# mjevans26/Satellite_ComputerVision

Measured on AMD Instinct MI355X. Metric: tiles/sec (train) 256x256x4 U-Net, higher is better.
Workload: dtype bf16; 1 GPU; U-Net 256x256x4 bfloat16 training, batch 64 per GPU (BASELINE configs[1]); global_batch=64, parallelism=dp1, loss=weighted_categorical_crossentropy, optimizer=adam(9e-4)

## Files before the change

include/satcv.h:

```cpp
#ifndef SATCV_H
#define SATCV_H
#include <stdint.h>
#ifdef __cplusplus
extern "C" {
#endif

typedef double satcv_stat_t;

enum { SATCV_OK = 0, SATCV_ERR_INVALID = -1, SATCV_ERR_HIP = -2, SATCV_ERR_UNSUPPORTED = -3 };
enum { SATCV_F32 = 0, SATCV_BF16 = 1,
       SATCV_FP8 = 2 ,
       SATCV_FP8X = 3 ,
       SATCV_F64 = 4  };
#define SATCV_STAT_ROWS 32

const char* satcv_version(void);
const char* satcv_last_error(void);
int satcv_device_info(int32_t* out4);

int satcv_ingest_nhwc(const float* src, void* dst, int64_t npix, int32_t c, int32_t cpad,
                      int32_t dtype, void* stream);
int satcv_ingest_nhwc_scaled(const float* src, void* dst, int64_t npix, int32_t c, int32_t cpad, float mul, int32_t dtype, void* stream);
int satcv_ingest_chw(const void* src, int32_t src_kind, float scale, void* dst, int32_t n,
                     int32_t c, int32_t h, int32_t w, int32_t cpad, int32_t dtype, void* stream);

int satcv_pack_weights(const float* src, void* dst_fwd, void* dst_dgrad, int32_t kh, int32_t kw,
                       int32_t cin, int32_t cout, int32_t cin_pad, int32_t transposed,
                       int32_t dtype, void* stream);
typedef struct { const float* src; void* dst; int32_t mode, taps, cin, cout, kpad, npad; } satcv_pack_job;
int64_t satcv_pack_job_items(const satcv_pack_job* job);
int satcv_pack_weights_batched(const satcv_pack_job* jobs_dev, const int64_t* prefix_dev, int32_t njobs, int64_t total_items, int32_t dtype,
                               void* stream);

typedef struct satcv_conv_desc {
  const void* x0;
  const void* x1;
  int32_t c0, c1;
  const float* in_scale;
  const float* in_shift;
  int32_t in_relu;
  const void* w;
  const float* bias;
  void* y;
  int32_t ldy;
  satcv_stat_t* stats;
  int32_t stats_ld;
  int32_t n, h, w_;
  int32_t cout;
  int32_t cout_pad;
  int32_t kh, kw, dil;
  int32_t mode_in;
  int32_t mode_out;
  int32_t f;
  int32_t cstat;
  int32_t out_relu;
  int32_t dtype;
  int32_t accumulate;
  int32_t stride, hin, win;
  const float* out_scale;
  void* pool_y; int32_t pool_ld, pool_f;
  const void* bst_y; const void* bst_y1; int32_t bst_ld, bst_ld1, bst_split;
  const float* bst_scale; const float* bst_shift; const float* bst_mean; const float* bst_rstd; int32_t bst_relu;
  int32_t tile_policy;
  int32_t pair_n, pair_c0, pair_c1;
} satcv_conv_desc;
int satcv_conv2d_igemm(const satcv_conv_desc* d, void* stream);
int satcv_conv2d_igemm_pipelined(const satcv_conv_desc* d);

typedef struct satcv_wgrad_desc {
  const void* x0; const void* x1; int32_t c0, c1;
  const float* in_scale; const float* in_shift; int32_t in_relu;
  const void* dy; int32_t lddy;
  float* dw;
  int32_t cin, cout;
  int32_t n, h, w_;
  int32_t kh, kw, dil;
  int32_t mode_dy;
  int32_t f;
  int32_t transposed;
  float* workspace; int64_t workspace_bytes;
  int32_t dtype;
  int32_t accumulate;
  int32_t whole_chip;
  int32_t defer_reduce;
} satcv_wgrad_desc;
int64_t satcv_conv2d_wgrad_workspace(const satcv_wgrad_desc* d);
int satcv_conv2d_wgrad(const satcv_wgrad_desc* d, void* stream);

typedef struct satcv_reduce_job {
  const float* ws; float* dw;
  int32_t nslab, taps, kpad, npad, cin, nvalid, transposed, accumulate, lanes, pad_;
} satcv_reduce_job;
int satcv_conv2d_wgrad_reduce_job(const satcv_wgrad_desc* d, satcv_reduce_job* job);
int64_t satcv_reduce_job_items(const satcv_reduce_job* job);
int satcv_reduce_slabs_batched(const satcv_reduce_job* jobs_dev, const int64_t* prefix_dev, int32_t njobs, int64_t total_items, void* stream);

typedef struct satcv_bwdf_desc {
  const void* g; const void* yraw; int32_t ldg;
  const float* bn_scale; const float* bn_shift; const float* bn_mean; const float* bn_rstd;
  const float* bn_coef;
  int32_t linear;
  const void* x0; const void* x1; int32_t c0, c1;
  const float* in_scale; const float* in_shift; int32_t in_relu;
  const void* w_dgrad;
  void* dx; int32_t lddx;
  float* dw; int32_t cin, cout;
  int32_t n, h, w_;
  int32_t kh, kw, dil;
  float* workspace; int64_t workspace_bytes;
  int32_t dtype;
  int32_t accumulate;
  satcv_stat_t* bst_sums; int32_t bst_sums_ld;
  const float* bst_mean; const float* bst_rstd;
  int32_t bst_act_form;
  const void* dpool; int32_t lddp; const void* amax;
// ... 243 lines not shown
```

satellite_computervision_amd/_lib.py:

```python
import ctypes as C
import os

import torch

_HERE = os.path.dirname(os.path.abspath(__file__))
LIB_PATH = os.environ.get('SATCV_LIB') or os.path.join(_HERE, 'libsatcv.so')

F32, BF16, FP8, FP8X, F64 = 0, 1, 2, 3, 4
STAT_ROWS = 32
COMPOSITE_MAX_T = 256

c_i32, c_i64, c_f32, c_vp = C.c_int32, C.c_int64, C.c_float, C.c_void_p


class ConvDesc(C.Structure):
    _fields_ = [('x0', c_vp), ('x1', c_vp), ('c0', c_i32), ('c1', c_i32),
                ('in_scale', c_vp), ('in_shift', c_vp), ('in_relu', c_i32),
                ('w', c_vp), ('bias', c_vp), ('y', c_vp), ('ldy', c_i32),
                ('stats', c_vp), ('stats_ld', c_i32),
                ('n', c_i32), ('h', c_i32), ('w_', c_i32),
                ('cout', c_i32), ('cout_pad', c_i32),
                ('kh', c_i32), ('kw', c_i32), ('dil', c_i32),
                ('mode_in', c_i32), ('mode_out', c_i32), ('f', c_i32),
                ('cstat', c_i32), ('out_relu', c_i32), ('dtype', c_i32), ('accumulate', c_i32),
                ('stride', c_i32), ('hin', c_i32), ('win', c_i32), ('out_scale', c_vp), ('pool_y', c_vp), ('pool_ld', c_i32), ('pool_f', c_i32),
                ('bst_y', c_vp), ('bst_y1', c_vp), ('bst_ld', c_i32), ('bst_ld1', c_i32), ('bst_split', c_i32),
                ('bst_scale', c_vp), ('bst_shift', c_vp), ('bst_mean', c_vp), ('bst_rstd', c_vp), ('bst_relu', c_i32), ('tile_policy', c_i32),
                ('pair_n', c_i32), ('pair_c0', c_i32), ('pair_c1', c_i32)]


class PackJob(C.Structure):
    _fields_ = [('src', c_vp), ('dst', c_vp), ('mode', c_i32), ('taps', c_i32), ('cin', c_i32), ('cout', c_i32), ('kpad', c_i32), ('npad', c_i32)]


class TileDesc(C.Structure):
    _fields_ = [('src', c_vp), ('src_kind', c_i32), ('n', c_i32), ('c', c_i32), ('hin', c_i32), ('win', c_i32), ('h', c_i32), ('w_', c_i32),
                ('rescale', C.c_double), ('nan_mask', c_i32), ('replace', c_i32), ('seed', C.c_uint64), ('ch_mean', c_vp),
                ('contra_mul', C.c_double), ('bright_mul', C.c_double), ('flip_v', c_i32), ('flip_h', c_i32), ('rot', c_i32),
                ('dst', c_vp), ('ldc', c_i32), ('coff', c_i32)]


class SceneGatherDesc(C.Structure):
    _fields_ = [('src', c_vp), ('src_kind', c_i32), ('h', c_i32), ('w_', c_i32), ('c', c_i32), ('rescale', C.c_double),
                ('origins', c_vp), ('total', c_i32), ('first', c_i32), ('n', c_i32), ('off', c_i32), ('side', c_i32),
                ('dst', c_vp), ('ldc', c_i32), ('coff', c_i32)]


class SceneScatterDesc(C.Structure):
    _fields_ = [('src', c_vp), ('src_kind', c_i32), ('n', c_i32), ('sh', c_i32), ('sw', c_i32), ('lds', c_i32), ('c0', c_i32), ('nc', c_i32),
                ('crop_y', c_i32), ('crop_x', c_i32), ('crop_h', c_i32), ('crop_w', c_i32),
                ('origins', c_vp), ('total', c_i32), ('first', c_i32), ('dst', c_vp), ('dst_kind', c_i32),
                ('h', c_i32), ('w_', c_i32), ('ldd', c_i32), ('doff', c_i32), ('accumulate', c_i32)]


class CompositeDesc(C.Structure):
    _fields_ = [('src', c_vp), ('src_kind', c_i32), ('t', c_i32), ('c', c_i32), ('h', c_i32), ('w_', c_i32), ('offsets', c_vp),
                ('median', c_vp), ('ld_med', c_i32), ('coff_med', c_i32), ('norm', c_vp), ('ld_norm', c_i32), ('coff_norm', c_i32),
                ('use_fill', c_i32), ('fill', c_f32)]


class WgradDesc(C.Structure):
    _fields_ = [('x0', c_vp), ('x1', c_vp), ('c0', c_i32), ('c1', c_i32),
                ('in_scale', c_vp), ('in_shift', c_vp), ('in_relu', c_i32),
                ('dy', c_vp), ('lddy', c_i32), ('dw', c_vp),
                ('cin', c_i32), ('cout', c_i32),
                ('n', c_i32), ('h', c_i32), ('w_', c_i32),
                ('kh', c_i32), ('kw', c_i32), ('dil', c_i32),
                ('mode_dy', c_i32), ('f', c_i32), ('transposed', c_i32),
                ('workspace', c_vp), ('workspace_bytes', c_i64), ('dtype', c_i32), ('accumulate', c_i32), ('whole_chip', c_i32), ('defer_reduce', c_i32)]


class BwdfDesc(C.Structure):
    _fields_ = [('g', c_vp), ('yraw', c_vp), ('ldg', c_i32),
                ('bn_scale', c_vp), ('bn_shift', c_vp), ('bn_mean', c_vp), ('bn_rstd', c_vp), ('bn_coef', c_vp), ('linear', c_i32),
                ('x0', c_vp), ('x1', c_vp), ('c0', c_i32), ('c1', c_i32),
                ('in_scale', c_vp), ('in_shift', c_vp), ('in_relu', c_i32),
                ('w_dgrad', c_vp), ('dx', c_vp), ('lddx', c_i32),
                ('dw', c_vp), ('cin', c_i32), ('cout', c_i32),
                ('n', c_i32), ('h', c_i32), ('w_', c_i32), ('kh', c_i32), ('kw', c_i32), ('dil', c_i32),
                ('workspace', c_vp), ('workspace_bytes', c_i64), ('dtype', c_i32), ('accumulate', c_i32),
                ('bst_sums', c_vp), ('bst_sums_ld', c_i32), ('bst_mean', c_vp), ('bst_rstd', c_vp), ('bst_act_form', c_i32),
# ... 179 lines not shown
```

satellite_computervision_amd/csrc/common.hpp:

```cpp
#pragma once
#include <hip/hip_runtime.h>
#include <hip/hip_fp8.h>
#include <stdint.h>
#include <type_traits>
#include "../../include/satcv.h"

typedef __bf16 bf16;
typedef __hip_fp8_e4m3 fp8;
struct fp8s : public __hip_fp8_e4m3 { using __hip_fp8_e4m3::__hip_fp8_e4m3; };
using i32x8 = __attribute__((ext_vector_type(8))) int;
using i32x4 = __attribute__((ext_vector_type(4))) int;

template <typename T> struct KTraits { static constexpr int EL = 8, SUB = 1; };
template <> struct KTraits<fp8s> { static constexpr int EL = 16, SUB = 2; };
using bf16x8 = __attribute__((ext_vector_type(8))) __bf16;
using bf16x4 = __attribute__((ext_vector_type(4))) __bf16;
using short4v = __attribute__((ext_vector_type(4))) short;
using f32x16 = __attribute__((ext_vector_type(16))) float;
using f32x4 = __attribute__((ext_vector_type(4))) float;

void satcv_set_error(const char* fmt, ...);
#define SATCV_CHECK(cond, ...)                        \
  do {                                                \
    if (!(cond)) {                                    \
// ... 199 lines not shown
  } else if constexpr (std::is_same<T, float>::value) {
    const float* f = reinterpret_cast<const float*>(&r.q[0]);
#pragma unroll
    for (int i = 0; i < 8; ++i) out[i] = f[i];
  } else {
    const fp8* b = reinterpret_cast<const fp8*>(&r.q);
#pragma unroll
    for (int i = 0; i < 8; ++i) out[i] = (float)b[i];
  }
}
template <typename T>
__device__ __forceinline__ void keep8(const Raw8<T>& r) {
  if constexpr (std::is_same<T, fp8>::value) { asm volatile("" :: "v"(r.q.x), "v"(r.q.y)); }
  else {
#pragma unroll
    for (int i = 0; i < Raw8<T>::NQ; ++i) asm volatile("" :: "v"(r.q[i].x), "v"(r.q[i].y), "v"(r.q[i].z), "v"(r.q[i].w));
  }
}
template <typename T>
__device__ __forceinline__ Raw8<T> select8(bool keep, const Raw8<T>& r) {
  Raw8<T> o;
  if constexpr (std::is_same<T, fp8>::value) {
    o.q = make_uint2(keep ? r.q.x : 0u, keep ? r.q.y : 0u);
  } else {
#pragma unroll
    for (int i = 0; i < Raw8<T>::NQ; ++i) o.q[i] = make_uint4(keep ? r.q[i].x : 0u, keep ? r.q[i].y : 0u, keep ? r.q[i].z : 0u, keep ? r.q[i].w : 0u);
  }
  return o;
}

template <typename T>
__device__ __forceinline__ float round_to(float x) {
  if constexpr (std::is_same<T, bf16>::value) return (float)(bf16)x;
  else if constexpr (std::is_same<T, fp8>::value) return (float)(fp8)x;
  else return x;
}

__device__ __forceinline__ float wave_sum(float v) {
#pragma unroll
  for (int o = 32; o > 0; o >>= 1) v += __shfl_xor(v, o, 64);
  return v;
}

typedef __attribute__((address_space(3))) char satcv_lds_char;
__device__ __forceinline__ unsigned lds_addr_of(const void* p) { return (unsigned)(uintptr_t)(satcv_lds_char*)p; }
__device__ __forceinline__ void lds_dma16(const void* gbase, unsigned voff, unsigned lds_dst) {
  unsigned keep;
  asm volatile("s_mov_b32 %0, m0\n\ts_mov_b32 m0, %3\n\ts_nop 0\n\tglobal_load_lds_dwordx4 %2, %1\n\ts_mov_b32 m0, %0"
               : "=&s"(keep) : "s"(gbase), "v"(voff), "s"(lds_dst) : "memory");
}
__device__ __forceinline__ void dma_wait_all() { asm volatile("s_waitcnt vmcnt(0)" ::: "memory"); }

#define SATCV_STAT_REPL 32
```

satellite_computervision_amd/csrc/conv_igemm.hip:

```cpp
#include "igemm_common.hpp"
#include <cstdlib>

template <typename T, int TW, int WM, int WN, int MT, int NT, int KS>
__global__ __launch_bounds__(WM* WN * 64) void igemm_kernel(const IgemmArgs a) {
  constexpr int NTHREADS = WM * WN * 64;
  constexpr int BM = WM * MT * 32;
  constexpr int BN = WN * NT * 32;
  constexpr int TH = BM / TW;
  constexpr int KC = KS * 16;
  constexpr int SLOTS = KC / 8;
  extern __shared__ __attribute__((aligned(16))) unsigned char smem_raw[];
  T* ldsA = reinterpret_cast<T*>(smem_raw);
  const int a_elems = SLOTS * a.rl * a.pitch * 8;
  T* ldsB = ldsA + a_elems;

  const int tid = threadIdx.x;
  const int lane = tid & 63;
  const int wave = tid >> 6;
  const int wm = wave / WN, wn = wave % WN;
  const int r = lane & 31, hh = lane >> 5;

  int bid = blockIdx.x;
  const int nt = bid % a.n_tiles;
  int mt = bid / a.n_tiles;
// ... 226 lines not shown

template <typename T>
static int launch_t(IgemmArgs& a, hipStream_t st) {
  switch (igemm_pick_tw(a.w_)) {
    case 32: return launch_tw<T, 32>(a, st);
    case 16: return launch_tw<T, 16>(a, st);
    default: return launch_tw<T, 8>(a, st);
  }
}

void satcv_prof_begin(int kind, double flops, hipStream_t st);
void satcv_prof_end(int kind, hipStream_t st);

static int igemm_fill_args(const satcv_conv_desc* d, IgemmArgs& a) {
  SATCV_CHECK(d && d->x0 && d->w && d->y, "igemm: null pointer");
  SATCV_CHECK(d->c0 > 0 && d->c0 % 16 == 0 && d->c1 % 16 == 0, "igemm: channels must be multiples of 16 (c0=%d c1=%d)", d->c0, d->c1);
  SATCV_CHECK(d->dtype != SATCV_FP8X || (d->c0 % 64 == 0 && d->c1 % 64 == 0 && !d->in_scale), "igemm: the scaled fp8 path needs channels %% 64 == 0 and no input transform");
  SATCV_CHECK((d->c1 == 0) == (d->x1 == nullptr), "igemm: x1/c1 mismatch");
  SATCV_CHECK(d->kh >= 1 && d->kw >= 1 && (d->kh & 1) && (d->kw & 1) && d->dil >= 1, "igemm: bad taps");
  SATCV_CHECK(d->n > 0 && d->h > 0 && d->w_ > 0 && d->cout > 0, "igemm: bad dims");
  SATCV_CHECK(satcv_pixels_ok(d->n, d->h, d->w_, d->f) && d->cout <= (1 << 20) && d->c0 <= (1 << 20) && d->c1 <= (1 << 20) &&
              d->kh <= 15 && d->kw <= 15 && d->dil <= (1 << 15) && d->f <= 16 && d->stride <= 16,
              "igemm: extents out of range (n*h*w must stay below 2^31 pixels, channels below 2^20)");
  SATCV_CHECK(d->cstat > 0, "igemm: cstat");
  SATCV_CHECK((!d->mode_in && !d->mode_out) || (d->f >= 2 && d->kh == 1 && d->kw == 1), "igemm: s2d/d2s need 1x1 taps and f>=2");
  SATCV_CHECK(!(d->accumulate && d->stats), "igemm: accumulate with statistics");
  SATCV_CHECK(!(d->mode_in && d->in_scale), "igemm: s2d source cannot carry an input transform");
  a.x0 = d->x0; a.x1 = d->x1; a.c0 = d->c0; a.c1 = d->c1;
  a.in_scale = d->in_scale; a.in_shift = d->in_shift; a.in_relu = d->in_relu;
  a.w = d->w; a.bias = d->bias; a.out_scale = d->out_scale; a.y = d->y; a.ldy = d->ldy;
  a.pool_y = d->pool_y; a.pool_ld = d->pool_ld; a.pool_f = d->pool_f;
  SATCV_CHECK(!d->pool_y || (d->pool_f >= 2 && !d->mode_out && !d->accumulate && d->h % d->pool_f == 0 && d->w_ % d->pool_f == 0 && d->pool_ld >= d->cout &&
                             d->cout % (d->dtype == SATCV_F32 ? 4 : (d->dtype == SATCV_BF16 ? 8 : 16)) == 0),
              "igemm: fused max-pool needs pool_f >= 2 dividing h and w_, plain output mode, whole 16-byte channel vectors");
  a.stats = d->stats; a.stats_ld = d->stats_ld;
  a.n = d->n; a.h = d->h; a.w_ = d->w_;
  a.hs = d->mode_in ? d->h * d->f : d->h; a.ws = d->mode_in ? d->w_ * d->f : d->w_;
  a.cout = d->cout; a.cout_pad = d->cout_pad;
  a.kh = d->kh; a.kw = d->kw; a.dil = d->dil;
  a.mode_in = d->mode_in; a.mode_out = d->mode_out; a.f = d->f;
  a.cstat = d->cstat; a.out_relu = d->out_relu; a.accumulate = d->accumulate;
  a.stride = d->stride > 1 ? d->stride : 1;
  if (a.stride > 1) {
    SATCV_CHECK(!d->mode_in && !d->mode_out && d->hin > 0 && d->win > 0 && d->h == (d->hin - 1) / a.stride + 1 && d->w_ == (d->win - 1) / a.stride + 1,
                "igemm: strided conv needs hin/win with h=(hin-1)/stride+1");
    a.hs = d->hin; a.ws = d->win;
  }
  a.dbg = 0;
  a.ksplit = 1; a.kslab = nullptr;
  a.bst_y = d->bst_y; a.bst_y1 = d->bst_y1; a.bst_ld = d->bst_ld; a.bst_ld1 = d->bst_ld1; a.bst_split = d->bst_y1 ? d->bst_split : 0;
  a.bst_scale = d->bst_scale; a.bst_shift = d->bst_shift; a.bst_mean = d->bst_mean; a.bst_rstd = d->bst_rstd; a.bst_relu = d->bst_relu;
  a.tile_policy = d->tile_policy;
  a.pair_n = d->pair_n; a.pair_c0 = d->pair_c0; a.pair_c1 = d->pair_c1;
  if (d->pair_n || d->pair_c0 || d->pair_c1) {
    const int epv = d->dtype == SATCV_F32 ? 4 : (d->dtype == SATCV_BF16 ? 8 : 16);
    SATCV_CHECK(d->pair_n > 0 && d->n == 2 * d->pair_n, "igemm: pair store needs n == 2 * pair_n (n=%d pair_n=%d)", d->n, d->pair_n);
    SATCV_CHECK(!d->mode_out && !d->accumulate && !d->stats && !d->bst_y, "igemm: pair store needs a plain store (no mode_out / accumulate / stats / bst_y)");
    SATCV_CHECK(d->pair_c0 >= 0 && d->pair_c1 >= 0 && d->pair_c0 + d->cout <= d->ldy && d->pair_c1 + d->cout <= d->ldy,
                "igemm: pair channel offsets %d / %d + cout %d exceed ldy %d", d->pair_c0, d->pair_c1, d->cout, d->ldy);
    SATCV_CHECK(d->pair_c0 % epv == 0 && d->pair_c1 % epv == 0, "igemm: pair channel offsets must be multiples of %d", epv);
  }
  if (d->bst_y) {
    SATCV_CHECK(d->stats && d->bst_scale && d->bst_shift && d->bst_mean && d->bst_rstd, "igemm: bst_y needs stats and the four BatchNorm vectors");
    SATCV_CHECK(!d->accumulate && !d->mode_out && !d->out_relu && !d->pool_y && d->cstat == d->cout, "igemm: bst_y needs a plain, non-accumulating store");
    SATCV_CHECK(d->bst_ld >= (d->bst_y1 ? d->bst_split : d->cout) && (!d->bst_y1 || (d->bst_split > 0 && d->bst_split < d->cout && d->bst_ld1 >= d->cout - d->bst_split)),
                "igemm: bst_y channel strides");
  }
  if (a.mode_in == 1) {
    SATCV_CHECK(!d->x1, "igemm: s2d with dual source");
    a.c1 = a.c0 * (d->f * d->f - 1);
  }
  return SATCV_OK;
}

static bool igemm_force_generic() {
  static const bool v = [] { const char* e = getenv("SATCV_IGEMM"); return e && e[0] == 'g'; }();
  return v;
}

extern "C" int satcv_conv2d_igemm_pipelined(const satcv_conv_desc* d) {
  IgemmArgs a;
  if (!d || igemm_fill_args(d, a) != SATCV_OK || igemm_force_generic()) return 0;
  if (a.kh == 3 && a.kw == 3 && a.stride == 1 && a.dil >= a.h && a.dil >= a.w_) { a.kh = a.kw = 1; a.dil = 1; }
  if (d->bst_y && a.dil == 3) {
    IgemmArgs b = a;
    b.bst_y = nullptr; b.bst_y1 = nullptr;
    if (igemm_ws_launch(b, d->dtype, nullptr, true) == SATCV_OK) return 0;
  }
  return igemm_fast_launch(a, d->dtype, nullptr, true) == SATCV_OK ? 1 : 0;
}

extern "C" int satcv_conv2d_igemm(const satcv_conv_desc* d, void* stream) {
  IgemmArgs a;
  int rc = igemm_fill_args(d, a);
  if (rc) return rc;
  hipStream_t st = reinterpret_cast<hipStream_t>(stream);
  const double flops = 2.0 * d->n * d->h * d->w_ * (double)d->cout * (double)(a.c0 + a.c1) * d->kh * d->kw;
  if (a.kh == 3 && a.kw == 3 && a.stride == 1 && a.dil >= a.h && a.dil >= a.w_) {
    const size_t esz = d->dtype == SATCV_BF16 ? 2 : 4;
    a.w = reinterpret_cast<const unsigned char*>(a.w) + (size_t)4 * ((a.c0 + a.c1) / 8) * a.cout_pad * 8 * esz;
    a.kh = a.kw = 1; a.dil = 1;
  }
  satcv_prof_begin(d->kh * d->kw > 1 ? 0 : 1, flops, st);
  rc = SATCV_ERR_UNSUPPORTED;
  if (!igemm_force_generic()) {
    rc = convt_thin_launch(a, d->dtype, st);
    if (rc == SATCV_ERR_UNSUPPORTED) rc = convt_thin_dgrad_launch(a, d->dtype, st);
    if (rc == SATCV_ERR_UNSUPPORTED) rc = igemm_tr_launch(a, d->dtype, st, false);
    if (rc == SATCV_ERR_UNSUPPORTED) rc = igemm_ws_launch(a, d->dtype, st, false);
    if (rc == SATCV_ERR_UNSUPPORTED) rc = igemm_fast_launch(a, d->dtype, st);
  }
  if (rc != SATCV_ERR_UNSUPPORTED) {  }
  else if (d->dtype == SATCV_FP8 || d->dtype == SATCV_FP8X) { satcv_set_error("igemm: this fp8 shape is outside the pipelined kernel's limits"); rc = SATCV_ERR_UNSUPPORTED; }
  else if (d->out_scale || d->pool_y || d->bst_y || d->pair_n) { satcv_set_error("igemm: out_scale / pool_y / bst_y / pair store need the pipelined kernel"); rc = SATCV_ERR_UNSUPPORTED; }
  else if (d->dtype == SATCV_BF16) rc = launch_t<bf16>(a, st);
  else if (d->dtype == SATCV_F32) rc = launch_t<float>(a, st);
  else { satcv_set_error("igemm: bad dtype %d", d->dtype); rc = SATCV_ERR_INVALID; }
  satcv_prof_end(d->kh * d->kw > 1 ? 0 : 1, st);
  return rc;
}
```

satellite_computervision_amd/csrc/conv_igemm_fast.hip:

```cpp
#include "igemm_common.hpp"
#include <cstdlib>
extern int g_opt_igemm_db, g_opt_igemm_thin, g_opt_igemm_sched, g_opt_splitk, g_opt_igemm_m16;

#ifndef SATCV_ABLATE
#define SATCV_ABLATE 0
#endif
#define ABL(bit) ((SATCV_ABLATE & (bit)) != 0)
#ifdef SATCV_STAMP
__device__ unsigned long long g_stamp[8][8][8];
#define STAMP(t) do { __builtin_amdgcn_sched_barrier(0); asm volatile("s_memtime %0\n\ts_waitcnt lgkmcnt(0)" : "=s"(t) :: "memory"); __builtin_amdgcn_sched_barrier(0); } while (0)
extern "C" int satcv_debug_read_stamps(unsigned long long* out) {
  return hipMemcpyFromSymbol(out, HIP_SYMBOL(g_stamp), sizeof(g_stamp)) == hipSuccess ? 0 : -1;
}
#endif
template <typename T, int TW, int WM, int WN, int MT, int NT, int KS, int TAPS, bool DYN, bool TL = false, bool DB = false, int WPS = 0, bool WDMA = false, bool SK = false, bool M16 = false>
__global__ __launch_bounds__(WM* WN * 64, (WPS ? WPS : (MT * NT <= 2 ? (KTraits<T>::SUB == 2 ? 2 : 4) : 1))) void igemm_fast_kernel(const IgemmArgs a) {
  constexpr int NTHREADS = WM * WN * 64;
  constexpr int BM = WM * MT * 32;
  constexpr int BN = WN * NT * 32;
  constexpr int TH = BM / TW;
  constexpr int EL = KTraits<T>::EL, SUB = KTraits<T>::SUB;
  constexpr int CLc = TW + (TAPS == 9 ? 2 : 0);
  constexpr int PITCHc = igemm_pitch(TW, CLc, M16);
  static_assert(!M16 || (std::is_same<T, bf16>::value && DB && !SK && !DYN && KS % 2 == 0 && TW >= 16), "16x16x32 form: double-buffered bf16 tiles, chunks of 32 k channels, tiles at least 16 pixels wide");
// ... 440 lines not shown
#ifdef SATCV_STAMP
      STAMP(t2);
#endif
      __syncthreads();
#ifdef SATCV_STAMP
      STAMP(t3);
#endif
      if (more) {
        store_lds(chunk + 1);
#ifdef SATCV_STAMP
        STAMP(t4);
#endif
        __syncthreads();
      }
#ifdef SATCV_STAMP
      else { STAMP(t4); }
      STAMP(t5);
      s_issue += t1 - t0; s_comp += t2 - t1; s_bar1 += t3 - t2; s_store += t4 - t3; s_bar2 += t5 - t4;
#endif
    }
#ifdef SATCV_STAMP
    if (blockIdx.x < 8 && lane == 0) {
      g_stamp[blockIdx.x][wave][0] = s_issue; g_stamp[blockIdx.x][wave][1] = s_comp; g_stamp[blockIdx.x][wave][2] = s_bar1;
      g_stamp[blockIdx.x][wave][3] = s_store; g_stamp[blockIdx.x][wave][7] = s_bar2;
    }
#endif
    }
#ifdef SATCV_STAMP
    STAMP(k3);
#endif

    if constexpr (SK) {
      const size_t mtot = (size_t)a.n * a.h * a.w_;
      float* slab = a.kslab + (size_t)split * mtot * a.cout;
#pragma unroll
      for (int m = 0; m < MT; ++m)
#pragma unroll
        for (int i = 0; i < 16; ++i) {
          const int q = (wm * MT + m) * 32 + (i & 3) + 8 * (i >> 2) + 4 * hh;
          const int t = q / TW, cx = q % TW;
          const int k = (a.imgs == 1) ? 0 : t / a.rpi;
          const int nimg = n0 + k, y = y0 + (t - k * a.rpi), x = x0 + cx;
          if (!((k < a.imgs) && (nimg < a.n) && (y < a.h) && (x < a.w_))) continue;
          float* row = slab + ((size_t)(nimg * a.h + y) * a.w_ + x) * a.cout;
#pragma unroll
          for (int n = 0; n < NT; ++n) {
            const int cn = nbase + (wn * NT + n) * 32 + r;
            if (cn < a.cout) row[cn] = acc[m][n][i];
          }
        }
      return;
    } else
    igemm_epilogue<T, TW, WM, WN, MT, NT, ABL(1), !DYN, true, M16, !DYN && !std::is_same<T, float>::value>(a, acc, n0, y0, x0, nbase, smem_raw);
#ifdef SATCV_STAMP
    {
      unsigned long long k4;
      STAMP(k4);
      if (blockIdx.x < 8 && lane == 0) {
        g_stamp[blockIdx.x][wave][4] = k1 - k0; g_stamp[blockIdx.x][wave][5] = k2 - k1; g_stamp[blockIdx.x][wave][6] = k4 - k3;
      }
    }
#endif
  }
}


#include <mutex>
static float* igemm_splitk_workspace(hipStream_t st, size_t bytes) {
  struct Slot { hipStream_t st; int dev; void* p; size_t n; bool captured; };
  static Slot slots[16];
  static int nslots = 0;
  static std::mutex mu;
  std::lock_guard<std::mutex> lk(mu);
  int dev = 0;
  (void)hipGetDevice(&dev);
  Slot* s = nullptr;
  for (int i = 0; i < nslots; ++i) if (slots[i].st == st && slots[i].dev == dev) s = &slots[i];
  if (!s) {
    if (nslots == 16) return nullptr;
    s = &slots[nslots++];
    *s = Slot{st, dev, nullptr, 0, false};
  }
  hipStreamCaptureStatus cs = hipStreamCaptureStatusNone;
  const bool capturing = hipStreamIsCapturing(st, &cs) == hipSuccess && cs != hipStreamCaptureStatusNone;
  if (s->n < bytes) {
    if (capturing) return nullptr;
    if (s->p && !s->captured) { (void)hipStreamSynchronize(st); (void)hipFree(s->p); }
    s->p = nullptr; s->n = 0; s->captured = false;
    const size_t want = bytes + (bytes >> 2);
    if (hipMalloc(&s->p, want) != hipSuccess) { (void)hipGetLastError(); s->p = nullptr; return nullptr; }
    s->n = want;
  }
  if (capturing) s->captured = true;
  return reinterpret_cast<float*>(s->p);
}

template <typename T>
__global__ __launch_bounds__(256) void igemm_splitk_finish_kernel(const IgemmArgs a, long long mtot) {
  __shared__ float ssum[2][1024];
  const int G = a.cout / 8;
  const long long total = mtot * G;
  const bool st = a.stats != nullptr && a.cout <= 1024 && 256 % G == 0;
  if (st) { for (int i = threadIdx.x; i < 2 * 1024; i += blockDim.x) (&ssum[0][0])[i] = 0.f; __syncthreads(); }
  float s1[8], s2[8];
#pragma unroll
  for (int e = 0; e < 8; ++e) { s1[e] = 0.f; s2[e] = 0.f; }
// ... 84 lines not shown
  if (M16) {
    const size_t plane_b = (((size_t)a.rl * a.pitch * EL * sizeof(T) + 255) / 256) * 256;
    const size_t a_st = (size_t)(KC / EL) * plane_b, b_sl = (size_t)TAPS * KC * BN * sizeof(T);
    lds_stage = WDMA ? 2 * a_st + 3 * b_sl : 2 * (a_st + b_sl);
  }
  if (WDMA && (((uintptr_t)a.w % 16) != 0 || a.cout_pad % 64 != 0)) return SATCV_ERR_UNSUPPORTED;
  if (DB && ((TL && TAPS != 1) || a.mode_in != 0)) return SATCV_ERR_UNSUPPORTED;
  size_t lds_out = (size_t)BM * (BN + 16 / sizeof(T)) * sizeof(T) + (size_t)(WM + 1) * 2 * BN * sizeof(float);
  if (a.bst_y) {
    if (sizeof(T) != 2 || (TAPS == 9 && a.dil != 1 && !TL) || a.imgs != 1 || a.h % TH != 0 || a.w_ % TW != 0 || a.cout % BN != 0 || a.cout % 8 != 0 || a.bst_ld % 8 != 0 ||
        ((uintptr_t)a.bst_y % 16) != 0 || (a.bst_y1 && (a.bst_split % 8 != 0 || a.bst_ld1 % 8 != 0 || ((uintptr_t)a.bst_y1 % 16) != 0)))
      return SATCV_ERR_UNSUPPORTED;
    lds_out += (size_t)BM * (BN + 16 / sizeof(T)) * sizeof(T);
  }
  const size_t lds_tab = a.in_scale ? (size_t)2 * cin * sizeof(float) : 0;
  const size_t lds = lds_stage + lds_tab > lds_out ? lds_stage + lds_tab : lds_out;
  if (lds > 160 * 1024) return SATCV_ERR_UNSUPPORTED;
  const bool dyn = TAPS == 9 && a.dil != 1;
  if (a.pair_n && (dyn || std::is_same<T, float>::value)) return SATCV_ERR_UNSUPPORTED;
  long long blocks = (long long)a.ngroups * a.tiles_y * a.tiles_x * a.n_tiles;
  if (blocks <= 0 || blocks > 0x7fffffffLL) return SATCV_ERR_UNSUPPORTED;
  a.ksplit = 1; a.kslab = nullptr;
  int ks = 1;
  if constexpr (SK) {
    const int splitk = g_opt_splitk;
    static const int splitk_tl = [] { const char* e = getenv("SATCV_SPLITK_TL"); return e ? atoi(e) : 1; }();
    if ((TL ? splitk_tl : splitk) && !dyn && sizeof(T) == 2 && a.mode_out == 0 && !a.pool_y && !a.accumulate && !a.bst_y && !a.pair_n && a.cout % 8 == 0 && a.ldy % 8 == 0 &&
        a.stride == 1 && (!a.stats || (a.cout <= 1024 && 256 % (a.cout / 8) == 0))) {
      constexpr bool DEEP1X1 = TAPS == 1 && !TL && KS == 4;
      const bool small_only = !TL && (DEEP1X1 || splitk == 2);
      while (ks < (TL ? 16 : 4) && blocks * ks * 2 <= 256 && a.nchunks / (ks * 2) >= (DEEP1X1 ? 4 : 8) && !(small_only && blocks >= 64)) ks *= 2;
    }
    if (ks == 1) return SATCV_ERR_UNSUPPORTED;
  }
  if (dry) return SATCV_OK;
  if (!dyn) {
    constexpr int CLc = TW + (TAPS == 9 ? 2 : 0);
    constexpr int PITCHc = igemm_pitch(TW, CLc, M16);
    if (a.cl != CLc || a.pitch != PITCHc) { satcv_set_error("igemm_fast: internal pitch mismatch (%d/%d vs %d/%d)", a.cl, a.pitch, CLc, PITCHc); return SATCV_ERR_INVALID; }
  }
  auto kern = igemm_fast_kernel<T, TW, WM, WN, MT, NT, KS, TAPS, false, TL, DB, WPS, WDMA, SK, M16>;
  if constexpr (TAPS == 9 && !DB && WPS == 0 && !SK) { if (dyn) kern = igemm_fast_kernel<T, TW, WM, WN, MT, NT, KS, TAPS, true>; }
  if ((DB || WPS || SK) && dyn) return SATCV_ERR_UNSUPPORTED;
  { const int rc = satcv_ensure_dynamic_lds(reinterpret_cast<const void*>(kern), lds); if (rc) return rc; }
  if constexpr (SK) {
    float* ws = igemm_splitk_workspace(st, (size_t)ks * a.n * a.h * a.w_ * a.cout * sizeof(float));
    if (!ws) return SATCV_ERR_UNSUPPORTED;
    a.ksplit = ks; a.kslab = ws; blocks *= ks;
  }
  hipLaunchKernelGGL(kern, dim3((unsigned)blocks), dim3(NTHREADS), lds, st, a);
  hipError_t e = hipGetLastError();
  if (e != hipSuccess) { satcv_set_error("igemm_fast launch: %s", hipGetErrorString(e)); return SATCV_ERR_HIP; }
  if (a.ksplit > 1) return igemm_splitk_finish<T>(a, st);
  return SATCV_OK;
}

template <typename T, int TW, int TAPS>
static int fast_tw(IgemmArgs& a, hipStream_t st, bool dry) {
  const int cin = a.c0 + a.c1;
  static const bool convt_wide = !(getenv("SATCV_CONVT_WIDE") && atoi(getenv("SATCV_CONVT_WIDE")) == 0);
  const int nspace = (a.mode_out && !convt_wide) ? a.cstat : a.cout;
  if constexpr (TAPS == 9 && std::is_same<T, bf16>::value) {
    const int db_mode = g_opt_igemm_db;
    a.dbg = g_opt_igemm_sched;
    const int m16 = (g_opt_igemm_m16 > 0 && a.tile_policy > g_opt_igemm_m16) ? a.tile_policy : g_opt_igemm_m16;
    if (TW == 32 && a.dil == 1 && (m16 >= 2 || (m16 == 1 && (a.stats || a.bst_y)))) {
      const int rc = igemm_m16p_launch(a, SATCV_BF16, st, dry);
      if (rc != SATCV_ERR_UNSUPPORTED) return rc;
    }
    if (db_mode && a.dil == 1 && a.mode_in == 0 && a.mode_out == 0 && !a.pool_y && nspace % 128 == 0 && (cin >= 128 || db_mode >= 2)) {
      const long long tiles256 = (long long)cdiv(a.n * a.h * a.w_, 256) * (nspace / 128);
      if (db_mode >= 2 || tiles256 >= 192) {
        static const int wdma = [] { const char* e = getenv("SATCV_WDMA"); return e ? atoi(e) : 1; }();
        if (m16 >= 2 || (m16 == 1 && (a.stats || a.bst_y))) {
          const int rc = igemm_m16_launch(a, SATCV_BF16, st, dry);
          if (rc != SATCV_ERR_UNSUPPORTED) return rc;
        }
        if (wdma) {
          const int rc = fast_cfg<T, TW, 4, 2, 2, 2, 1, TAPS, false, true, 0, true>(a, st, dry);
          if (rc != SATCV_ERR_UNSUPPORTED) return rc;
        }
        const int rc = fast_cfg<T, TW, 4, 2, 2, 2, 1, TAPS, false, true>(a, st, dry);
        if (rc != SATCV_ERR_UNSUPPORTED) return rc;
      }
    }
    static const int db64 = [] { const char* e = getenv("SATCV_DB64"); return e ? atoi(e) : 1; }();
    if (db_mode && db64 && a.dil == 1 && a.mode_in == 0 && a.mode_out == 0 && !a.pool_y && nspace % 64 == 0 && (nspace == 64 || db64 >= 2) && (cin >= 128 || db64 >= 3) &&
        (long long)cdiv(a.n * a.h * a.w_, 512) * (nspace / 64) >= 192) {
      const int rc = fast_cfg<T, TW, 8, 1, 2, 2, 1, TAPS, false, true>(a, st, dry);
      if (rc != SATCV_ERR_UNSUPPORTED) return rc;
    }
  }
  if constexpr (KTraits<T>::SUB == 2) {
    if (nspace >= 64 && nspace % 64 == 0) return fast_cfg<T, TW, 2, 2, 2, 1, 1, TAPS>(a, st, dry);
    return fast_cfg<T, TW, 4, 1, 2, 1, 1, TAPS>(a, st, dry);
  }
  if constexpr (TAPS == 1 && KTraits<T>::SUB == 1) {
    const bool ks2 = (cin % 32 == 0) && (!a.x1 || a.c0 % 32 == 0) && (a.mode_in != 1 || a.c0 % 32 == 0);
    if (a.taploop) {
      if (!ks2) {
        if (nspace >= 64 && nspace % 64 == 0) return fast_cfg<T, TW, 2, 2, 2, 1, 1, TAPS, true>(a, st, dry);
        return fast_cfg<T, TW, 4, 1, 2, 1, 1, TAPS, true>(a, st, dry);
      }
      if (nspace >= 128 && nspace % 128 == 0) {
        if constexpr (std::is_same<T, bf16>::value) {
          const int rc = fast_cfg<T, TW, 2, 2, 2, 2, 2, TAPS, true, false, 0, false, true>(a, st, dry);
// ... 90 lines not shown
```

satellite_computervision_amd/csrc/conv_igemm_m16.hip:

```cpp
#include "igemm_common.hpp"
#include <cstdlib>

#ifndef SATCV_M16_ABL
#define SATCV_M16_ABL 0
#endif
#define MABL(bit) ((SATCV_M16_ABL & (bit)) != 0)

template <int TW>
struct M16Geom {
  static constexpr int BM = 256, BN = 128, TH = BM / TW, CL = TW + 2, RL = TH + 2;
  static constexpr int NPIX = ((RL * CL + 7) / 8) * 8;
  static constexpr int PLANE_E = (((NPIX * 16 + 255) / 256) * 256) / 2;
  static constexpr int A_STAGE_E = 4 * PLANE_E;
  static constexpr int UNIT_E = 3 * 4 * BN * 8;
  static constexpr int WBUF_E = 2 * UNIT_E;
  static constexpr int A_ITEMS = NPIX * 4;
  static constexpr int AI = (A_ITEMS + 511) / 512;
  static constexpr size_t LDS_OPERANDS = (size_t)(2 * A_STAGE_E + 2 * WBUF_E) * 2;
};

template <int TW>
__global__ __launch_bounds__(512, 1) void igemm_m16sym_kernel(const IgemmArgs a) {
  using T = bf16;
  using G = M16Geom<TW>;
// ... 128 lines not shown
#pragma unroll
        for (int j = 0; j < AI; ++j) {
          if (MABL(128)) { asm volatile("" :: "v"(ra[j].q[0].x), "v"(ra[j].q[0].y), "v"(ra[j].q[0].z), "v"(ra[j].q[0].w)); continue; }
          if (P == 0) store_a(1, j);
          if (P == 2) { if (c + 2 < nch) store_a(0, j); }
        }
      }
      if (t >= 0 && t < 3) {
        if (t < AI && !MABL(64)) {
          if (P == 1) load_a(c + 2 < nch ? c + 2 : nch - 1, t);
          if (P == 2) load_a(c + 3 < nch ? c + 3 : nch - 1, t);
        }
        if (more && !MABL(32)) {
          dma_piece(2 * (k + 1) + (2 * t) / 3, (2 * t) % 3, (k + 1) & 1, (2 * t) / 3);
          dma_piece(2 * (k + 1) + (2 * t + 1) / 3, (2 * t + 1) % 3, (k + 1) & 1, (2 * t + 1) / 3);
        }
      }
      __builtin_amdgcn_sched_barrier(0);
      if (!MABL(8)) mma16_step<MT, NT>(acc, af[MABL(1) ? 0 : (s & 1)], bf[MABL(1) ? 0 : (s & 1)]);
      else { for (int m = 0; m < 2 * MT; ++m) asm volatile("" :: "v"(af[s & 1][m].v)); for (int n = 0; n < 2 * NT; ++n) asm volatile("" :: "v"(bf[s & 1][n].v)); }
    }
#pragma unroll
    for (int m = 0; m < MT; ++m)
#pragma unroll
      for (int n = 0; n < NT; ++n) asm volatile("" : "+v"(acc[m][n]));
    if (!MABL(4)) {
      dma_wait_all();
      __syncthreads();
    }
  };
  static_assert(AI <= 3, "one activation load per staging slot");
  auto k_loop = [&](auto LATEC) {
    for (int k = 0, c = 0; k < nint; k += 3, c += 2) {
      interval(std::integral_constant<int, 0>{}, LATEC, k, c);
      interval(std::integral_constant<int, 1>{}, LATEC, k + 1, c);
      interval(std::integral_constant<int, 2>{}, LATEC, k + 2, c);
    }
  };
#ifdef SATCV_M16_NOSTAGGER
  k_loop(std::false_type{});
#else
  if (wave >= 4) k_loop(std::true_type{});
  else k_loop(std::false_type{});
#endif
  if (MABL(4)) { dma_wait_all(); __syncthreads(); }
  if (MABL(16)) {
#pragma unroll
    for (int m = 0; m < MT; ++m)
#pragma unroll
      for (int n = 0; n < NT; ++n) asm volatile("" :: "v"(acc[m][n]));
    return;
  }
  igemm_epilogue<T, TW, WM, WN, MT, NT, false, true, true, true>(a, acc, n0, y0, x0, nbase, smem_raw);
}

template <int TW>
__global__ __launch_bounds__(768, 1) void igemm_m16_kernel(const IgemmArgs a) {
  using T = bf16;
  using G = M16Geom<TW>;
  constexpr int WM = 4, WN = 2, MT = 2, NT = 2, BN = G::BN, TH = G::TH, CL = G::CL;
  extern __shared__ __attribute__((aligned(16))) unsigned char smem_raw[];
  T* ldsA = reinterpret_cast<T*>(smem_raw);
  T* ldsW = ldsA + 2 * G::A_STAGE_E;
  float* ldsT = reinterpret_cast<float*>(ldsW + 2 * G::WBUF_E);
  const int tid = threadIdx.x, lane = tid & 63;
  const int wave = __builtin_amdgcn_readfirstlane(tid >> 6);
  const int cin = a.c0 + a.c1, nch = cin / 32, nint = (3 * nch) / 2;
  int bid;
  {
    const int G_ = gridDim.x, orig = blockIdx.x;
    const int xcd = orig & 7, q = G_ >> 3, rem = G_ & 7;
    bid = (xcd < rem ? xcd * (q + 1) : rem * (q + 1) + (xcd - rem) * q) + (orig >> 3);
  }
  const int nbase = (bid % a.n_tiles) * BN;
  int n0, y0, x0;
  {
    int mt = bid / a.n_tiles;
    const int tx = mt % a.tiles_x; mt /= a.tiles_x;
    const int ty = mt % a.tiles_y;
    n0 = mt / a.tiles_y; y0 = ty * TH; x0 = tx * TW;
  }
  if (a.in_scale) {
    for (int i = tid; i < cin; i += 768) { ldsT[i] = a.in_scale[i]; ldsT[cin + i] = a.in_shift[i]; }
  }

  if (wave >= 8) {
    constexpr int NS = 256, AI = (G::A_ITEMS + NS - 1) / NS;
    const int sid = tid - 512, ws = wave - 8;
#ifndef SATCV_M16_PRIO
#define SATCV_M16_PRIO 2
#endif
    if (SATCV_M16_PRIO) __builtin_amdgcn_s_setprio(SATCV_M16_PRIO);
    const int slot_t = ((sid >> 3) + sid) & 3;
    int a_l[AI], a_p[AI];
#pragma unroll
    for (int j = 0; j < AI; ++j) {
      const int it = sid + j * NS;
      const int pix = ((it >> 5) << 3) | (it & 7);
      const int L = pix / CL, c = pix - L * CL;
      const int y = y0 + L - 1, x = x0 + c - 1;
      a_l[j] = (it < G::A_ITEMS) ? slot_t * G::PLANE_E + pix * 8 : -1;
      a_p[j] = (it < G::A_ITEMS && L < G::RL && y >= 0 && y < a.h && x >= 0 && x < a.w_) ? (n0 * a.h + y) * a.w_ + x : -1;
    }
    auto chunk_ptr = [&](int x, int& cs) -> const T* {
      const int cg0 = x * 32;
      if (cg0 < a.c0) { cs = a.c0; return reinterpret_cast<const T*>(a.x0) + cg0 + slot_t * 8; }
// ... 72 lines not shown
  }

  const int wm = wave / WN, wn = wave % WN, g4 = lane >> 4, l16 = lane & 15;
  int a_off[2 * MT];
#pragma unroll
  for (int m = 0; m < 2 * MT; ++m) {
    const int q = wm * MT * 32 + m * 16 + l16;
    a_off[m] = g4 * G::PLANE_E + ((q / TW) * CL + q % TW) * 8;
  }
  const int b_lane = (g4 * BN + wn * NT * 32 + l16) * 8;
  f32x16 acc[MT][NT];
#pragma unroll
  for (int m = 0; m < MT; ++m)
#pragma unroll
    for (int n = 0; n < NT; ++n)
#pragma unroll
      for (int i = 0; i < 16; ++i) acc[m][n][i] = 0.f;
  __syncthreads();
  __syncthreads();
  auto interval = [&](auto PC, int k) {
    constexpr int P = decltype(PC)::value;
    const int wb = (k & 1) * G::WBUF_E;
    FragT<T> af[2][2 * MT], bf[2][2 * NT];
    auto read_step = [&](int s, int buf) {
      const int ub = s / 3, kx = s % 3;
      const int ky = P == 0 ? ub : (P == 1 ? (ub == 0 ? 2 : 0) : ub + 1);
      const int stage = P == 0 ? 0 : (P == 1 ? ub : 1);
      const int aoff = stage * G::A_STAGE_E + (ky * CL + kx) * 8;
#pragma unroll
      for (int m = 0; m < 2 * MT; ++m) af[buf][m] = lds_frag<T>(ldsA + a_off[m] + aoff);
#pragma unroll
      for (int n = 0; n < 2 * NT; ++n) bf[buf][n] = lds_frag<T>(ldsW + wb + b_lane + ub * G::UNIT_E + (kx * 4 * BN + n * 16) * 8);
    };
    read_step(0, 0);
#pragma unroll
    for (int s = 0; s < 6; ++s) {
      asm volatile("" ::: "memory");
      if (s + 1 < 6) read_step(s + 1, (s + 1) & 1);
      __builtin_amdgcn_sched_barrier(0);
      mma16_step<MT, NT>(acc, af[s & 1], bf[s & 1]);
    }
#pragma unroll
    for (int m = 0; m < MT; ++m)
#pragma unroll
      for (int n = 0; n < NT; ++n) asm volatile("" : "+v"(acc[m][n]));
    __syncthreads();
  };
  for (int k = 0; k < nint; k += 3) {
    interval(std::integral_constant<int, 0>{}, k);
    interval(std::integral_constant<int, 1>{}, k + 1);
    interval(std::integral_constant<int, 2>{}, k + 2);
  }
  igemm_epilogue<T, TW, WM, WN, MT, NT, false, true, true, true>(a, acc, n0, y0, x0, nbase, smem_raw);
}

template <int TW>
static int m16_cfg(IgemmArgs& a, hipStream_t st, bool dry) {
  using G = M16Geom<TW>;
  const int cin = a.c0 + a.c1;
  if (a.h < G::TH) return SATCV_ERR_UNSUPPORTED;
  if (cin % 64 != 0 || (a.x1 && a.c0 % 32 != 0) || a.cout % 128 != 0 || a.cout_pad % 64 != 0 || a.cout_pad < a.cout) return SATCV_ERR_UNSUPPORTED;
  if (((uintptr_t)a.w % 16) != 0 || a.ldy % 8 != 0 || ((uintptr_t)a.y % 16) != 0) return SATCV_ERR_UNSUPPORTED;
  a.halh = a.halw = 1;
  a.tiles_x = cdiv(a.w_, TW); a.tiles_y = cdiv(a.h, G::TH);
  a.rpi = G::TH; a.imgs = 1; a.ngroups = a.n;
  a.seg = G::RL; a.rl = G::RL; a.cl = G::CL; a.pitch = G::CL;
  a.n_tiles = a.cout / 128;
  a.cpt = cin / 32; a.nchunks = a.cpt; a.taploop = 0; a.halh_tl = a.halw_tl = 1;
  a.ksplit = 1; a.kslab = nullptr;
  size_t lds_out = (size_t)G::BM * (G::BN + 8) * 2 + (size_t)(4 + 1) * 2 * G::BN * sizeof(float);
  if (a.bst_y) {
    if (a.h % G::TH != 0 || a.w_ % TW != 0 || a.cout % 8 != 0 || a.bst_ld % 8 != 0 || ((uintptr_t)a.bst_y % 16) != 0 ||
        (a.bst_y1 && (a.bst_split % 8 != 0 || a.bst_ld1 % 8 != 0 || ((uintptr_t)a.bst_y1 % 16) != 0)))
      return SATCV_ERR_UNSUPPORTED;
    lds_out += (size_t)G::BM * (G::BN + 8) * 2;
  }
  const size_t lds_op = G::LDS_OPERANDS + (a.in_scale ? (size_t)2 * cin * sizeof(float) : 0);
  const size_t lds = lds_op > lds_out ? lds_op : lds_out;
  if (lds > 160 * 1024) return SATCV_ERR_UNSUPPORTED;
  const long long blocks = (long long)a.n * a.tiles_y * a.tiles_x * a.n_tiles;
  if (blocks <= 0 || blocks > 0x7fffffffLL) return SATCV_ERR_UNSUPPORTED;
  if (dry) return SATCV_OK;
  static const int roles_opt = [] { const char* e = getenv("SATCV_M16_WS"); return e ? atoi(e) : 1; }();
  const bool roles = roles_opt >= 2 || (roles_opt == 1 && cin >= 256);
  auto kern = roles ? igemm_m16_kernel<TW> : igemm_m16sym_kernel<TW>;
  { const int rc = satcv_ensure_dynamic_lds(reinterpret_cast<const void*>(kern), lds); if (rc) return rc; }
  hipLaunchKernelGGL(kern, dim3((unsigned)blocks), dim3(roles ? 768 : 512), lds, st, a);
  hipError_t e = hipGetLastError();
  if (e != hipSuccess) { satcv_set_error("igemm_m16 launch: %s", hipGetErrorString(e)); return SATCV_ERR_HIP; }
  return SATCV_OK;
}

int igemm_m16_launch(IgemmArgs& a, int dtype, hipStream_t st, bool dry) {
  if (dtype != SATCV_BF16) return SATCV_ERR_UNSUPPORTED;
  if (!(a.kh == 3 && a.kw == 3 && a.dil == 1 && a.stride == 1 && a.mode_in == 0 && a.mode_out == 0 && !a.pool_y && !a.out_scale)) return SATCV_ERR_UNSUPPORTED;
  switch (igemm_pick_tw(a.w_)) {
    case 32: return m16_cfg<32>(a, st, dry);
    case 16: return m16_cfg<16>(a, st, dry);
    default: return SATCV_ERR_UNSUPPORTED;
  }
}
```

satellite_computervision_amd/csrc/conv_igemm_m16p.hip:

```cpp
#include "igemm_common.hpp"
#include <cstdlib>

#ifndef SATCV_M16P_ABL
#define SATCV_M16P_ABL 0
#endif
#define PABL(bit) ((SATCV_M16P_ABL & (bit)) != 0)

#ifdef SATCV_STAMP_M16P
__device__ unsigned long long g_stamp_m16p[8][12][4];
extern "C" int satcv_debug_read_stamps_m16p(unsigned long long* out) { return hipMemcpyFromSymbol(out, HIP_SYMBOL(g_stamp_m16p), sizeof(g_stamp_m16p)) == hipSuccess ? 0 : -1; }
#define PSTAMP(t) do { __builtin_amdgcn_sched_barrier(0); asm volatile("s_memtime %0\n\ts_waitcnt lgkmcnt(0)" : "=s"(t) :: "memory"); __builtin_amdgcn_sched_barrier(0); } while (0)
#else
#define PSTAMP(t) do { } while (0)
#endif

__device__ __forceinline__ bf16x4 m16p_tr_read(const bf16* p) {
  typedef short short4v_ __attribute__((ext_vector_type(4)));
  short4v_ v = __builtin_amdgcn_ds_read_tr16_b64_v4i16((__attribute__((address_space(3))) short4v_*)(p));
  return __builtin_bit_cast(bf16x4, v);
}

extern int g_opt_m16p_prio;
extern int g_opt_m16p;
int g_m16p_launches = 0;

template <int BN_>
struct M16PGeom {
  static constexpr int TW = 32, TH = 8, BM = 256, BN = BN_, CL = TW + 2, RL = TH + 2;
  static constexpr int NPIX = ((RL * CL + 7) / 8) * 8;
  static constexpr int PLANE_E = (((NPIX * 16 + 255) / 256) * 256) / 2;
  static constexpr int A_STAGE_E = 4 * PLANE_E;
  static constexpr int UNIT_E = 3 * 4 * BN * 8;
  static constexpr int A_ITEMS = NPIX * 4;
  static constexpr int NS = 256, AI = (A_ITEMS + NS - 1) / NS;
  static constexpr int VPR = BN / 8, PPR = NS / VPR;
  static constexpr int ROUNDS = BM * (BN / 8) / NS;
  static constexpr int NBW = BN / 32;
  static constexpr int SWM = BN == 128 ? 15 : 7;
  static constexpr size_t FIXED_BYTES = (size_t)(2 * A_STAGE_E + 2 * UNIT_E + BM * BN) * 2 + BN * sizeof(float);
};

template <bool BST, int BN_ = 128>
__global__ __launch_bounds__(768, 1) void igemm_m16p_kernel(const IgemmArgs a, const int m_total) {
  using T = bf16;
  using G = M16PGeom<BN_>;
  constexpr int BN = G::BN, CL = G::CL, TH = G::TH, TW = G::TW;
  extern __shared__ __attribute__((aligned(16))) unsigned char smem_raw[];
  T* ldsA = reinterpret_cast<T*>(smem_raw);
  T* ldsW = ldsA + 2 * G::A_STAGE_E;
  T* ldsO = ldsW + 2 * G::UNIT_E;
  float* ldsB = reinterpret_cast<float*>(ldsO + G::BM * BN);
  float* ldsT = ldsB + BN;
  const int tid = threadIdx.x, lane = tid & 63;
  const int wave = __builtin_amdgcn_readfirstlane(tid >> 6);
  const int cin = a.c0 + a.c1, nch = cin / 32, upt = 3 * nch;

  int bid;
  {
    const int G_ = gridDim.x, orig = blockIdx.x;
    const int xcd = orig & 7, q = G_ >> 3, rem = G_ & 7;
    bid = (xcd < rem ? xcd * (q + 1) : rem * (q + 1) + (xcd - rem) * q) + (orig >> 3);
  }
  const int nbase = (bid % a.n_tiles) * BN;
  int m_lo, ntl;
  {
    const int rr = bid / a.n_tiles, R = gridDim.x / a.n_tiles;
    const int per = m_total / R, extra = m_total % R;
    m_lo = rr * per + (rr < extra ? rr : extra);
    ntl = per + (rr < extra ? 1 : 0);
  }
  if (ntl <= 0) return;
  for (int i = tid; i < BN; i += 768) ldsB[i] = a.bias ? a.bias[nbase + i] : 0.f;
  const bool xaff = !BST && a.in_scale != nullptr;
  if (xaff) {
    for (int i = tid; i < cin; i += 768) { ldsT[i] = a.in_scale[i]; ldsT[cin + i] = a.in_shift[i]; }
  }
  if constexpr (BST) {
    for (int i = tid; i < BN; i += 768) { ldsT[i] = a.bst_scale[nbase + i]; ldsT[BN + i] = a.bst_shift[nbase + i]; }
  }
  auto tile_origin = [&](int v, int& n0, int& y0, int& x0) __attribute__((always_inline)) {
    const int tx = v % a.tiles_x; v /= a.tiles_x;
    const int ty = v % a.tiles_y;
    n0 = v / a.tiles_y; y0 = ty * TH; x0 = tx * TW;
  };

  if (wave >= 8) {
    constexpr int NS = G::NS, AI = G::AI;
    const int sid = tid - 512;
    if (a.dbg == 1) __builtin_amdgcn_s_setprio(1);
    else if (a.dbg == 2) __builtin_amdgcn_s_setprio(2);
    else if (a.dbg == 3) __builtin_amdgcn_s_setprio(3);
    const int nc = ntl * nch;
    const int slot_t = ((sid >> 3) + sid) & 3;
    auto item_lc = [&](int j, int& L, int& c) __attribute__((always_inline)) -> bool {
      int it = sid + j * NS;
      asm volatile("" : "+v"(it));
      const int pix = ((it >> 5) << 3) | (it & 7);
      L = pix / CL; c = pix - L * CL;
      return it < G::A_ITEMS && L < G::RL;
    };
    Raw8<T> ra[2][AI];
    unsigned vmask[2] = {0u, 0u};
    int l_v = m_lo, l_x = 0;
    unsigned l_pix[AI], l_vm = 0;
    long long l_pb = 0;
    auto load_setup = [&]() __attribute__((always_inline)) {
      int n0, y0, x0; tile_origin(l_v, n0, y0, x0);
      const int ylo = 1 - y0, yhi = a.h - y0 + 1, xlo = 1 - x0, xhi = a.w_ - x0 + 1;
      l_pb = (long long)(n0 * a.h + y0 - 1) * a.w_ + (x0 - 1);
      unsigned vm = 0;
#pragma unroll
      for (int j = 0; j < AI; ++j) {
        int L, c;
        const bool ok = item_lc(j, L, c) && L >= ylo && L < yhi && c >= xlo && c < xhi;
        vm |= (ok ? 1u : 0u) << j;
        l_pix[j] = ok ? (unsigned)(__mul24(L, a.w_) + c) : (unsigned)(a.w_ + 1);
      }
      l_vm = vm;
    };
    auto load_items = [&](auto SET, auto J0C, auto NJC) __attribute__((always_inline)) {
      constexpr int S = decltype(SET)::value, J0 = decltype(J0C)::value, NJ = decltype(NJC)::value;
      const int cg0 = l_x * 32;
      const bool second = cg0 >= a.c0;
      const int cs = second ? a.c1 : a.c0;
// ... 305 lines not shown
            asm volatile("" ::: "memory");
            if (kx + 1 < 3 && (!PABL(2) || gu == 0)) read_step(kx + 1, (kx + 1) & 1);
            __builtin_amdgcn_sched_barrier(0);
#pragma unroll
            for (int m = 0; m < 4; ++m)
#pragma unroll
              for (int n = 0; n < NBW; ++n) {
                if constexpr (!PABL(1)) acc[m][n] = __builtin_amdgcn_mfma_f32_16x16x32_bf16(bf[kx & 1][n].v, af[kx & 1][m].v, acc[m][n], 0, 0, 0);
                else asm volatile("" : "+v"(acc[m][n]) : "v"(bf[kx & 1][n].v), "v"(af[kx & 1][m].v));
              }
          }
        }
        if (ky == 2 && x + 1 == nch && !PABL(32)) {
#pragma unroll
          for (int m = 0; m < 4; ++m) {
            const int px = wm * 64 + m * 16 + l16;
#pragma unroll
            for (int n = 0; n < NBW; ++n) {
              const int gr = (wn * (BN / 8) + n * 4 + g4) ^ (2 * (l16 & G::SWM));
              bf16x4 o;
#pragma unroll
              for (int j = 0; j < 4; ++j) o[j] = (bf16)acc[m][n][j];
              *reinterpret_cast<bf16x4*>(ldsO + px * BN + gr * 4) = o;
            }
          }
          acc_init();
        }
        PSTAMP(y1);
        if (!PABL(128)) dma_wait_all();
        PSTAMP(y2);
        __syncthreads();
        PSTAMP(y3);
#ifdef SATCV_STAMP_M16P
        ys[0] += y1 - y0; ys[1] += y2 - y1; ys[2] += y3 - y2; ys[3] += 1; y0 = y3;
#endif
        ++gu;
      }
    }
  }
#ifdef SATCV_STAMP_M16P
  if (blockIdx.x < 8 && lane == 0) for (int i = 0; i < 4; ++i) g_stamp_m16p[blockIdx.x][wave][i] = ys[i];
#endif
  if (mstats) {
    stats_mfma();
    if ((l16 >> 2) == g4) {
      const int r = l16 & 3;
      const float s2 = r == 0 ? g_sq[0] : r == 1 ? g_sq[1] : r == 2 ? g_sq[2] : g_sq[3];
      const float s1 = r == 0 ? g_sm[0] : r == 1 ? g_sm[1] : r == 2 ? g_sm[2] : g_sm[3];
      satcv_stat_t* rowp = a.stats + (size_t)(blockIdx.x % SATCV_STAT_ROWS) * 2 * a.stats_ld;
      atomicAdd(rowp + nbase + wave * 16 + l16, (satcv_stat_t)s1);
      atomicAdd(rowp + a.stats_ld + nbase + wave * 16 + l16, (satcv_stat_t)s2);
    }
  }
}

template <int BN>
static int m16p_launch_bn(IgemmArgs& a, hipStream_t st, bool dry) {
  using G = M16PGeom<BN>;
  if (!(a.kh == 3 && a.kw == 3 && a.dil == 1 && a.stride == 1 && a.mode_in == 0 && a.mode_out == 0 && !a.pool_y && !a.out_scale && !a.out_relu && !a.accumulate))
    return SATCV_ERR_UNSUPPORTED;
  const int cin = a.c0 + a.c1;
  if (a.h % G::TH != 0 || a.w_ % G::TW != 0) return SATCV_ERR_UNSUPPORTED;
  if (cin % 64 != 0 || (a.x1 && a.c0 % 32 != 0) || a.cout % BN != 0 || a.cout_pad % 64 != 0 || a.cout_pad < a.cout || a.cstat != a.cout) return SATCV_ERR_UNSUPPORTED;
  if (((uintptr_t)a.w % 16) != 0 || a.ldy % 8 != 0 || ((uintptr_t)a.y % 16) != 0 || ((uintptr_t)a.x0 % 16) != 0 || (a.x1 && ((uintptr_t)a.x1 % 16) != 0)) return SATCV_ERR_UNSUPPORTED;
  if (a.c0 % 8 != 0 || a.c1 % 8 != 0) return SATCV_ERR_UNSUPPORTED;
  if (a.bst_y) {
    if (a.bst_ld % 8 != 0 || ((uintptr_t)a.bst_y % 16) != 0 || (a.bst_y1 && (a.bst_split % 8 != 0 || a.bst_ld1 % 8 != 0 || ((uintptr_t)a.bst_y1 % 16) != 0))) return SATCV_ERR_UNSUPPORTED;
    if ((long long)G::TH * a.w_ * (a.bst_ld > a.bst_ld1 ? a.bst_ld : a.bst_ld1) >= (1LL << 31)) return SATCV_ERR_UNSUPPORTED;
  }
  if ((long long)(G::TH + 2) * a.w_ * (a.c0 > a.c1 ? a.c0 : a.c1) >= (1LL << 23)) return SATCV_ERR_UNSUPPORTED;
  if ((long long)G::TH * a.w_ * a.ldy >= (1LL << 31)) return SATCV_ERR_UNSUPPORTED;
  if (a.bst_y && a.in_scale) return SATCV_ERR_UNSUPPORTED;
  const size_t lds = G::FIXED_BYTES + (a.bst_y ? (size_t)2 * G::BN * sizeof(float) : a.in_scale ? (size_t)2 * cin * sizeof(float) : 0);
  if (lds > 160 * 1024) return SATCV_ERR_UNSUPPORTED;
  static int ncu = 0;
  if (!ncu) {
    int dev = 0; hipDeviceProp_t p;
    if (hipGetDevice(&dev) != hipSuccess || hipGetDeviceProperties(&p, dev) != hipSuccess) { satcv_set_error("igemm_m16p: device query failed"); return SATCV_ERR_HIP; }
    ncu = p.multiProcessorCount;
  }
  a.halh = a.halw = 1;
  a.tiles_x = a.w_ / G::TW; a.tiles_y = a.h / G::TH;
  a.rpi = G::TH; a.imgs = 1; a.ngroups = a.n;
  a.seg = G::RL; a.rl = G::RL; a.cl = G::CL; a.pitch = G::CL;
  a.n_tiles = a.cout / BN;
  a.cpt = cin / 32; a.nchunks = a.cpt; a.taploop = 0; a.halh_tl = a.halw_tl = 1;
  a.ksplit = 1; a.kslab = nullptr;
  a.dbg = a.bst_y ? g_opt_m16p_prio % 10 : a.in_scale ? (g_opt_m16p_prio / 10) % 10 : (g_opt_m16p_prio / 100) % 10;
  if (BN == 64) {
    static const int p64 = [] { const char* e = getenv("SATCV_M16P_PRIO64"); return e ? atoi(e) : -1; }();
    if (p64 >= 0) a.dbg = a.bst_y ? p64 % 10 : a.in_scale ? (p64 / 10) % 10 : (p64 / 100) % 10;
  }
  const long long m_total = (long long)a.n * a.tiles_y * a.tiles_x;
  if (m_total <= 0 || m_total > 0x7fffffffLL || a.n_tiles > ncu) return SATCV_ERR_UNSUPPORTED;
  long long ranges = ncu / a.n_tiles;
  if (ranges > m_total) ranges = m_total;
  if (g_opt_m16p < 2 && m_total < 2 * ranges) return SATCV_ERR_UNSUPPORTED;
  if (dry) return SATCV_OK;
  auto kern = a.bst_y ? igemm_m16p_kernel<true, BN> : igemm_m16p_kernel<false, BN>;
  { const int rc = satcv_ensure_dynamic_lds(reinterpret_cast<const void*>(kern), lds); if (rc) return rc; }
  hipLaunchKernelGGL(kern, dim3((unsigned)(ranges * a.n_tiles)), dim3(768), lds, st, a, (int)m_total);
  ++g_m16p_launches;
  hipError_t e = hipGetLastError();
  if (e != hipSuccess) { satcv_set_error("igemm_m16p launch: %s", hipGetErrorString(e)); return SATCV_ERR_HIP; }
  return SATCV_OK;
}

int igemm_m16p_launch(IgemmArgs& a, int dtype, hipStream_t st, bool dry) {
  if (dtype != SATCV_BF16 || a.pair_n) return SATCV_ERR_UNSUPPORTED;
  if (!g_opt_m16p) return SATCV_ERR_UNSUPPORTED;
  if (a.cout % 128 == 0) return m16p_launch_bn<128>(a, st, dry);
  static const int bn64 = [] { const char* e = getenv("SATCV_M16P_BN64"); return e ? atoi(e) : 1; }();
  if (bn64 && a.cout % 64 == 0) return m16p_launch_bn<64>(a, st, dry);
  return SATCV_ERR_UNSUPPORTED;
}
```

satellite_computervision_amd/csrc/conv_igemm_ws.hip:

```cpp
#include "igemm_common.hpp"
#include <cstdlib>
extern int g_opt_igemm_thin;
int g_ws_launches = 0;

#ifndef SATCV_ABLATE
#define SATCV_ABLATE 0
#endif
#define WABL(bit) ((SATCV_ABLATE & (bit)) != 0)
#ifdef SATCV_STAMP
__device__ unsigned long long g_stamp_ws[8][8][8];
extern "C" int satcv_debug_read_stamps_ws(unsigned long long* out) { return hipMemcpyFromSymbol(out, HIP_SYMBOL(g_stamp_ws), sizeof(g_stamp_ws)) == hipSuccess ? 0 : -1; }
#define STAMP(t) do { __builtin_amdgcn_sched_barrier(0); asm volatile("s_memtime %0\n\ts_waitcnt lgkmcnt(0)" : "=s"(t) :: "memory"); __builtin_amdgcn_sched_barrier(0); } while (0)
#define STAMP_V(t) do { __builtin_amdgcn_sched_barrier(0); asm volatile("s_waitcnt vmcnt(0)\n\ts_memtime %0\n\ts_waitcnt lgkmcnt(0)" : "=s"(t) :: "memory"); __builtin_amdgcn_sched_barrier(0); } while (0)
#endif

template <typename T, int CIN, int NT, int WPS, int WN = 1, int DIL = 1>
__global__ __launch_bounds__(256 * WN, WPS) void igemm_ws_kernel(const IgemmArgs a, const int total_tiles) {
  constexpr int TW = 32, TH = 8, WM = 4, MT = 2, BM = 256, BN = WN * NT * 32, NTHREADS = 256 * WN, EL = 8;
  constexpr int SLOTS = CIN / EL, CL = TW + 2 * DIL, PITCH = CL, RL = TH + 2 * DIL;
  constexpr int PLANE = RL * PITCH * EL;
  constexpr int WANT = (SLOTS >= 8 ? 16 : 128 / SLOTS) / (int)sizeof(T), BANKSPAN = 128 / (int)sizeof(T);
  constexpr int SPAD = ((WANT - PLANE % BANKSPAN) % BANKSPAN + BANKSPAN) % BANKSPAN;
  constexpr int SLOT_STRIDE = PLANE + SPAD;
  constexpr int A_ITEMS = RL * CL * SLOTS, AI = (A_ITEMS + NTHREADS - 1) / NTHREADS;
  constexpr int W_ITEMS = 9 * SLOTS * BN;
  constexpr int OPITCH = BN + 16 / (int)sizeof(T);
  constexpr size_t A_BYTES = (size_t)SLOTS * SLOT_STRIDE * sizeof(T);
  constexpr size_t O_BYTES = (size_t)BM * OPITCH * sizeof(T) + (size_t)(WM + 1) * 2 * BN * sizeof(float);
  constexpr size_t R0_BYTES = ((A_BYTES > O_BYTES ? A_BYTES : O_BYTES) + 127) / 128 * 128;
  extern __shared__ __attribute__((aligned(16))) unsigned char smem_raw[];
  T* ldsA = reinterpret_cast<T*>(smem_raw);
  T* ldsW = reinterpret_cast<T*>(smem_raw + R0_BYTES);

  const int tid = threadIdx.x, lane = tid & 63, wave = tid >> 6;
  const int wm = wave / WN, wn = wave % WN;
  const int r = lane & 31, hh = lane >> 5;
  const int slot_t = tid % SLOTS;
  const T* wp = reinterpret_cast<const T*>(a.w);

  for (int it = tid; it < W_ITEMS; it += NTHREADS) {
    const int co = it % BN, run = it / BN;
    const Raw8<T> v = gload8<T>(wp + ((size_t)run * a.cout_pad + co) * EL);
    lstore8<T>(ldsW + (size_t)it * EL, v);
  }
  const int ch0 = slot_t * EL;
  const bool second = ch0 >= a.c0;
  const T* src = second ? reinterpret_cast<const T*>(a.x1) + (ch0 - a.c0) : reinterpret_cast<const T*>(a.x0) + ch0;
  const int cs = second ? a.c1 : a.c0;
  float sc[8], sh[8];
#pragma unroll
  for (int e = 0; e < 8; ++e) { sc[e] = a.in_scale ? a.in_scale[ch0 + e] : 1.f; sh[e] = a.in_scale ? a.in_shift[ch0 + e] : 0.f; }
  const bool aff = a.in_scale != nullptr;
  const unsigned relu_lim = a.in_relu != 0 ? 0u : 0x80008000u;

  int a_l[AI], a_yx[AI], a_eoff[AI];
#pragma unroll
  for (int j = 0; j < AI; ++j) {
    const int it = tid + j * NTHREADS;
    const int pix = it / SLOTS, c = pix % CL, L = pix / CL;
    a_l[j] = it < A_ITEMS ? slot_t * SLOT_STRIDE + (L * PITCH + c) * EL : -1;
    a_yx[j] = ((L - DIL) << 16) | ((c - DIL) & 0xffff);
    a_eoff[j] = ((L - DIL) * a.w_ + (c - DIL)) * cs;
  }
  int a_off[MT];
#pragma unroll
  for (int m = 0; m < MT; ++m) {
    const int q = (wm * MT + m) * 32 + r;
// ... 68 lines not shown
    f32x16 acc[MT][NT];
#pragma unroll
    for (int m = 0; m < MT; ++m)
#pragma unroll
      for (int n = 0; n < NT; ++n)
#pragma unroll
        for (int i = 0; i < 16; ++i) acc[m][n][i] = 0.f;
    {
      constexpr int KS = CIN / 16, STEPS = 9 * KS;
      FragT<T> af[2][MT], bf[2][NT];
      auto read_step = [&](int st, int buf) {
        const int tap = st / KS, ks = st % KS;
        const int tap_off = ((tap / 3) * DIL * PITCH + (tap % 3) * DIL) * EL;
        const int slot = ks * 2 + hh;
#pragma unroll
        for (int m = 0; m < MT; ++m) af[buf][m] = lds_frag<T>(ldsA + slot * SLOT_STRIDE + a_off[m] + tap_off);
#pragma unroll
        for (int n = 0; n < NT; ++n) bf[buf][n] = lds_frag<T>(ldsW + ((tap * SLOTS + slot) * BN + (wn * NT + n) * 32 + r) * EL);
      };
      read_step(0, 0);
#pragma unroll
      for (int st = 0; st < STEPS; ++st) {
        asm volatile("" ::: "memory");
        if (st + 1 < STEPS) read_step(st + 1, (st + 1) & 1);
        __builtin_amdgcn_sched_barrier(0);
#pragma unroll
        for (int m = 0; m < MT; ++m)
#pragma unroll
          for (int n = 0; n < NT; ++n) { if (!WABL(2)) mma32<T>(acc[m][n], af[st & 1][m], bf[st & 1][n]); }
      }
    }
#ifdef SATCV_STAMP
    STAMP(q5);
#endif
    __syncthreads();
#ifdef SATCV_STAMP
    STAMP(q6);
#endif
    igemm_epilogue<T, TW, WM, WN, MT, NT, WABL(1), true, false, false, DIL == 1>(a, acc, tn0, ty0, tx0, 0, smem_raw, carry);
#ifdef SATCV_STAMP
    STAMP(q7);
#endif
    __syncthreads();
#ifdef SATCV_STAMP
    STAMP(q8);
    z[0] += q1 - q0; z[1] += q2 - q1; z[2] += q3 - q2; z[3] += q4 - q3; z[4] += q5 - q4; z[5] += q6 - q5; z[6] += q7 - q6; z[7] += q8 - q7;
#endif
  }
  if (a.stats && tid < BN && tid < a.cout && t_lo < t_hi) {
    satcv_stat_t* rowp = a.stats + (size_t)(blockIdx.x % SATCV_STAT_ROWS) * 2 * a.stats_ld;
    atomicAdd(rowp + tid, (satcv_stat_t)carry[0]);
    atomicAdd(rowp + a.stats_ld + tid, (satcv_stat_t)carry[1]);
  }
#ifdef SATCV_STAMP
  if (blockIdx.x < 8 && lane == 0)
    for (int i = 0; i < 8; ++i) g_stamp_ws[blockIdx.x][wave][i] = z[i] / (unsigned long long)max(t_hi - t_lo, 1);
#endif
}

template <typename T, int CIN, int NT, int WPS, int WN = 1, int DIL = 1>
static int ws_cfg(IgemmArgs& a, hipStream_t st, bool dry) {
  constexpr int TW = 32, TH = 8, BN = WN * NT * 32, SLOTS = CIN / 8, RL = TH + 2 * DIL, PITCH = TW + 2 * DIL;
  constexpr int ES = (int)sizeof(T);
  constexpr int PLANE = RL * PITCH * 8;
  constexpr int WANT = (SLOTS >= 8 ? 16 : 128 / SLOTS) / ES, BANKSPAN = 128 / ES;
  constexpr int SPAD = ((WANT - PLANE % BANKSPAN) % BANKSPAN + BANKSPAN) % BANKSPAN;
  constexpr size_t A_BYTES = (size_t)SLOTS * (PLANE + SPAD) * ES;
  constexpr size_t O_BYTES = (size_t)256 * (BN + 16 / ES) * ES + (size_t)5 * 2 * BN * 4;
  constexpr size_t R0 = ((A_BYTES > O_BYTES ? A_BYTES : O_BYTES) + 127) / 128 * 128;
  constexpr size_t LDS = R0 + (size_t)9 * SLOTS * BN * 8 * ES;
  static_assert(LDS <= 160 * 1024, "weights + tile exceed the LDS");
  a.halh = a.halw = DIL;
  a.tiles_x = cdiv(a.w_, TW); a.tiles_y = cdiv(a.h, TH);
  a.rpi = TH; a.imgs = 1; a.ngroups = a.n; a.seg = RL; a.rl = RL; a.cl = PITCH; a.pitch = PITCH; a.n_tiles = 1;
  const long long total = (long long)a.n * a.tiles_y * a.tiles_x;
  if (total <= 0 || total > 0x7fffffffLL) return SATCV_ERR_UNSUPPORTED;
  if (dry) return SATCV_OK;
  auto kern = igemm_ws_kernel<T, CIN, NT, WPS, WN, DIL>;
  { const int rc = satcv_ensure_dynamic_lds(reinterpret_cast<const void*>(kern), LDS); if (rc) return rc; }
  static int ncu = 0;
  if (!ncu) {
    int dev = 0; hipDeviceProp_t p;
    if (hipGetDevice(&dev) != hipSuccess || hipGetDeviceProperties(&p, dev) != hipSuccess) { satcv_set_error("ws: device query failed"); return SATCV_ERR_HIP; }
    ncu = p.multiProcessorCount;
  }
  int per_cu = (int)((160 * 1024) / LDS);
  if (per_cu > WPS) per_cu = WPS;
  if (per_cu < 1) per_cu = 1;
  long long grid = (long long)ncu * per_cu;
  if (grid > total) grid = total;
  hipLaunchKernelGGL(kern, dim3((unsigned)grid), dim3(256 * WN), LDS, st, a, (int)total);
  ++g_ws_launches;
  hipError_t e = hipGetLastError();
  if (e != hipSuccess) { satcv_set_error("igemm_ws launch: %s", hipGetErrorString(e)); return SATCV_ERR_HIP; }
  return SATCV_OK;
}

int igemm_ws_launch(IgemmArgs& a, int dtype, hipStream_t st, bool dry) {
  if (!g_opt_igemm_thin || (dtype != SATCV_BF16 && dtype != SATCV_FP8)) return SATCV_ERR_UNSUPPORTED;
  const int cin = a.c0 + a.c1;
  if (a.kh != 3 || a.kw != 3 || (a.dil != 1 && a.dil != 3) || a.stride != 1 || a.mode_in || a.mode_out || a.bst_y) return SATCV_ERR_UNSUPPORTED;
  if (a.accumulate && (a.accumulate != 1 || dtype != SATCV_BF16 || a.stats || a.pool_y || a.out_relu || a.out_scale)) return SATCV_ERR_UNSUPPORTED;
  if (a.pool_y && (8 % a.pool_f != 0 || 32 % a.pool_f != 0)) return SATCV_ERR_UNSUPPORTED;
  if (a.dil == 3) {
    if (dtype != SATCV_BF16 || a.pool_y || a.pair_n || !(cin == 16 || cin == 32) || !(a.cout == 16 || a.cout == 32) || a.cout_pad != 32 || a.cstat != a.cout) return SATCV_ERR_UNSUPPORTED;
    if (a.x1 && (a.c0 % 8 != 0)) return SATCV_ERR_UNSUPPORTED;
    if (a.h % 8 != 0 || a.w_ % 32 != 0 || a.ldy % 8 != 0 || ((uintptr_t)a.y % 16) != 0) return SATCV_ERR_UNSUPPORTED;
    return cin == 16 ? ws_cfg<bf16, 16, 1, 2, 1, 3>(a, st, dry) : ws_cfg<bf16, 32, 1, 2, 1, 3>(a, st, dry);
  }
  if (a.cout == 16 && dtype == SATCV_BF16 && !a.pool_y && (cin == 16 || cin == 32) && a.cout_pad == 32 && a.cstat == 16 && !(a.x1 && (a.c0 % 8 != 0)) &&
      a.h % 8 == 0 && a.w_ % 32 == 0 && a.ldy % 8 == 0 && ((uintptr_t)a.y % 16) == 0) {
    return cin == 16 ? ws_cfg<bf16, 16, 1, 3>(a, st, dry) : ws_cfg<bf16, 32, 1, 3>(a, st, dry);
  }
  if (!(cin == 16 || cin == 32 || cin == 64) || !(a.cout == 32 || a.cout == 64) || a.cout_pad != a.cout || a.cstat != a.cout) return SATCV_ERR_UNSUPPORTED;
  if (a.x1 && (a.c0 % 8 != 0)) return SATCV_ERR_UNSUPPORTED;
  const int epv = dtype == SATCV_FP8 ? 16 : 8;
  if (a.h % 8 != 0 || a.w_ % 32 != 0 || a.ldy % epv != 0 || ((uintptr_t)a.y % 16) != 0) return SATCV_ERR_UNSUPPORTED;
  if (dtype == SATCV_FP8) {
    if (a.stats || cin == 16 || (a.pool_y && a.pool_ld % 16 != 0)) return SATCV_ERR_UNSUPPORTED;
    if (a.cout == 32) return cin == 32 ? ws_cfg<fp8, 32, 1, 3>(a, st, dry) : ws_cfg<fp8, 64, 1, 2>(a, st, dry);
    return cin == 32 ? ws_cfg<fp8, 32, 2, 2>(a, st, dry) : ws_cfg<fp8, 64, 1, 1, 2>(a, st, dry);
  }
  if (a.cout == 32) {
    if (cin == 16) return ws_cfg<bf16, 16, 1, 3>(a, st, dry);
    if (cin == 32) return ws_cfg<bf16, 32, 1, 3>(a, st, dry);
    return ws_cfg<bf16, 64, 1, 2>(a, st, dry);
  }
  if (cin == 16) return ws_cfg<bf16, 16, 2, 2>(a, st, dry);
  if (cin == 32) return ws_cfg<bf16, 32, 2, 2>(a, st, dry);
  return ws_cfg<bf16, 64, 1, 1, 2>(a, st, dry);
}
```

satellite_computervision_amd/csrc/conv_thin_roles.hip:

```cpp
#include "igemm_common.hpp"
#include <cstdlib>
extern int g_opt_igemm_thin, g_opt_thin_roles;
extern int g_ws_launches, g_tr_launches;

template <int CINS, int COUT, int TH>
struct TrGeom {
  static constexpr int CINP = CINS < 32 ? 32 : CINS;
  static constexpr int SX = CINP / 8, SXR = CINS / 8, PX = TH * 32, RL = TH + 2, CL = 34, NPIX = RL * CL, NPIXP = (NPIX + 7) / 8 * 8;
  static constexpr int PLANE_E = ((NPIXP * 16 + 255) / 256 * 256) / 2;
  static constexpr int ABUF_E = SX * PLANE_E;
  static constexpr int W_E = 9 * CINP * COUT;
  static constexpr int OPITCH = COUT + 8, O_E = PX * OPITCH;
  static constexpr size_t LDS = (size_t)(2 * ABUF_E + W_E + 2 * O_E) * 2;
  static constexpr int A_ITEMS = NPIXP * SXR, AI = (A_ITEMS + 255) / 256;
  static_assert(LDS >= 16 * 256 * sizeof(float), "end-of-kernel reduction of the statistics");
};

template <int CINS, int COUT, int TH>
__global__ __launch_bounds__(768, 1) void igemm_tr_kernel(const IgemmArgs a, const int total_tiles) {
  typedef bf16 T;
  using G = TrGeom<CINS, COUT, TH>;
  constexpr int CINP = G::CINP, SX = G::SX, SXR = G::SXR, PX = G::PX, CL = G::CL, OPITCH = G::OPITCH, AI = G::AI;
  constexpr int NS = 256, VQ = COUT / 8, OI = PX * VQ / NS, OQS = NS / VQ;
  static_assert((PX * VQ) % NS == 0 && NS % VQ == 0 && NS % (8 * SXR) == 0, "item -> thread mapping");
// ... 116 lines not shown
          for (int e = 0; e < 8; ++e) mx[e] = -INFINITY;
          for (int i = 0; i < f; ++i)
            for (int jj = 0; jj < f; ++jj) {
              const bf16x8 s8 = *reinterpret_cast<const bf16x8*>(so + ((t0 + i) * 32 + c0 + jj) * OPITCH);
#pragma unroll
              for (int e = 0; e < 8; ++e) mx[e] = fmaxf(mx[e], (float)s8[e]);
            }
          bf16x8 o;
#pragma unroll
          for (int e = 0; e < 8; ++e) o[e] = (bf16)mx[e];
          *reinterpret_cast<bf16x8*>(pp + ((size_t)(n0 * hp + (y0 + t0) / f) * wp + (x0 + c0) / f) * a.pool_ld) = o;
        }
      }
    };
    const std::integral_constant<int, 0> S0{};
    const std::integral_constant<int, 1> S1{};
    if (t_lo < t_hi) issue(t_lo, S0);
    if (t_lo + 1 < t_hi) issue(t_lo + 1, S1);
    __syncthreads();
    if (t_lo < t_hi) {
      store_tile(0, S0);
      if (t_lo + 2 < t_hi) issue(t_lo + 2, S0);
    }
    __syncthreads();
    auto iteration = [&](int t, auto KC) __attribute__((always_inline)) {
      constexpr int K = decltype(KC)::value;
      if (t > t_lo) epilogue(t - 1, K ^ 1);
      if (t + 1 < t_hi) {
        store_tile(K ^ 1, std::integral_constant<int, K ^ 1>{});
        if (t + 3 < t_hi) issue(t + 3, std::integral_constant<int, K ^ 1>{});
      }
      __syncthreads();
    };
    for (int t = t_lo; t < t_hi; t += 2) {
      iteration(t, S0);
      if (t + 1 < t_hi) iteration(t + 1, S1);
    }
    if (t_lo < t_hi) epilogue(t_hi - 1, (t_hi - 1 - t_lo) & 1);
    __syncthreads();
    if (a.stats && t_lo < t_hi) {
      float* r2 = reinterpret_cast<float*>(smem_raw);
#pragma unroll
      for (int e = 0; e < 8; ++e) { r2[e * NS + sid] = st1[e]; r2[(8 + e) * NS + sid] = st2[e]; }
      __syncthreads();
      if (sid < COUT) {
        const int gq = sid >> 3, e = sid & 7;
        double t1 = 0.0, t2 = 0.0;
        for (int k = 0; k < NS / VQ; ++k) { t1 += (double)r2[e * NS + k * VQ + gq]; t2 += (double)r2[(8 + e) * NS + k * VQ + gq]; }
        satcv_stat_t* rowp = a.stats + (size_t)(blockIdx.x % SATCV_STAT_ROWS) * 2 * a.stats_ld;
        atomicAdd(rowp + sid, (satcv_stat_t)t1);
        atomicAdd(rowp + a.stats_ld + sid, (satcv_stat_t)t2);
      }
    }
    return;
  }

  const int g4 = lane >> 4, l16 = lane & 15;
  constexpr int NPB = PX / 16, PBW = NPB / 8, NB = COUT / 16, KS = CINP / 32;
  static_assert(PBW * 8 == NPB, "pixel blocks per wave");
  int a_off[PBW];
#pragma unroll
  for (int p = 0; p < PBW; ++p) {
    const int q = (wave * PBW + p) * 16 + l16;
    a_off[p] = g4 * G::PLANE_E + ((q >> 5) * CL + (q & 31)) * 8;
  }
  const int b_off = (g4 * COUT + l16) * 8;
  float bia[NB], osc[NB];
#pragma unroll
  for (int n = 0; n < NB; ++n) { bia[n] = a.bias ? a.bias[n * 16 + l16] : 0.f; osc[n] = a.out_scale ? a.out_scale[n * 16 + l16] : 1.f; }
  const bool orelu = a.out_relu != 0;
  __syncthreads();
  __syncthreads();
  for (int t = t_lo; t < t_hi; ++t) {
    const int b = (t - t_lo) & 1;
    const T* A = ldsA + b * G::ABUF_E;
    f32x4 acc[PBW][NB];
#pragma unroll
    for (int p = 0; p < PBW; ++p)
#pragma unroll
      for (int n = 0; n < NB; ++n) acc[p][n] = f32x4{0.f, 0.f, 0.f, 0.f};
    {
      constexpr int STEPS = 9 * KS;
      FragT<T> af[2][PBW], bf[2][NB];
      auto read_step = [&](int st, int buf) __attribute__((always_inline)) {
        const int tap = st / KS, ks = st % KS;
        const int toff = ((tap / 3) * CL + (tap % 3)) * 8 + ks * 4 * G::PLANE_E;
#pragma unroll
        for (int p = 0; p < PBW; ++p) af[buf][p] = lds_frag<T>(A + a_off[p] + toff);
#pragma unroll
        for (int n = 0; n < NB; ++n) bf[buf][n] = lds_frag<T>(ldsW + ((tap * SX + ks * 4) * COUT + n * 16) * 8 + b_off);
      };
      read_step(0, 0);
      auto tap_row = [&](auto GC) __attribute__((always_inline)) {
        constexpr int S0_ = decltype(GC)::value * 3 * KS;
#pragma unroll
        for (int s_ = 0; s_ < 3 * KS; ++s_) {
          const int st = S0_ + s_;
          asm volatile("" ::: "memory");
          if (st + 1 < STEPS) read_step(st + 1, (st + 1) & 1);
          __builtin_amdgcn_sched_barrier(0);
#pragma unroll
          for (int p = 0; p < PBW; ++p)
#pragma unroll
            for (int n = 0; n < NB; ++n) acc[p][n] = __builtin_amdgcn_mfma_f32_16x16x32_bf16(af[st & 1][p].v, bf[st & 1][n].v, acc[p][n], 0, 0, 0);
        }
      };
      tap_row(std::integral_constant<int, 0>{});
      tap_row(std::integral_constant<int, 1>{});
      tap_row(std::integral_constant<int, 2>{});
    }
#pragma unroll
    for (int p = 0; p < PBW; ++p) {
      T* op = ldsO + b * G::O_E + ((wave * PBW + p) * 16 + 4 * g4) * OPITCH + l16;
#pragma unroll
      for (int n = 0; n < NB; ++n)
#pragma unroll
        for (int j = 0; j < 4; ++j) {
          float v = acc[p][n][j] * osc[n] + bia[n];
          if (orelu) v = fmaxf(v, 0.f);
          op[j * OPITCH + n * 16] = (T)v;
        }
    }
    __syncthreads();
  }
  __syncthreads();
}

template <int CINS, int COUT, int TH>
static int tr_cfg(IgemmArgs& a, hipStream_t st, bool dry) {
  using G = TrGeom<CINS, COUT, TH>;
  static_assert(G::LDS <= 160 * 1024, "buffers + weights exceed the LDS");
  if (a.h % TH != 0) return SATCV_ERR_UNSUPPORTED;
  if (a.pool_y && (TH % a.pool_f != 0 || 32 % a.pool_f != 0)) return SATCV_ERR_UNSUPPORTED;
  a.halh = a.halw = 1;
  a.tiles_x = a.w_ / 32; a.tiles_y = a.h / TH;
  a.rpi = TH; a.imgs = 1; a.ngroups = a.n; a.seg = TH + 2; a.rl = TH + 2; a.cl = 34; a.pitch = 34; a.n_tiles = 1;
  const long long total = (long long)a.n * a.tiles_y * a.tiles_x;
  if (total <= 0 || total > 0x7fffffffLL) return SATCV_ERR_UNSUPPORTED;
  if ((long long)(TH + 2) * a.w_ * (a.c0 > a.c1 ? a.c0 : a.c1) >= (1LL << 23)) return SATCV_ERR_UNSUPPORTED;
  if (dry) return SATCV_OK;
  auto kern = igemm_tr_kernel<CINS, COUT, TH>;
  { const int rc = satcv_ensure_dynamic_lds(reinterpret_cast<const void*>(kern), G::LDS); if (rc) return rc; }
  static int ncu = 0;
  if (!ncu) {
    int dev = 0; hipDeviceProp_t p;
    if (hipGetDevice(&dev) != hipSuccess || hipGetDeviceProperties(&p, dev) != hipSuccess) { satcv_set_error("igemm_tr: device query failed"); return SATCV_ERR_HIP; }
    ncu = p.multiProcessorCount;
  }
  long long grid = ncu;
  if (grid > total) grid = total;
  hipLaunchKernelGGL(kern, dim3((unsigned)grid), dim3(768), G::LDS, st, a, (int)total);
  ++g_ws_launches; ++g_tr_launches;
  hipError_t e = hipGetLastError();
  if (e != hipSuccess) { satcv_set_error("igemm_tr launch: %s", hipGetErrorString(e)); return SATCV_ERR_HIP; }
  return SATCV_OK;
}

int igemm_tr_launch(IgemmArgs& a, int dtype, hipStream_t st, bool dry) {
  const int on = g_opt_thin_roles;
  if (!on || !g_opt_igemm_thin || dtype != SATCV_BF16) return SATCV_ERR_UNSUPPORTED;
  const int cin = a.c0 + a.c1;
  if (a.kh != 3 || a.kw != 3 || a.dil != 1 || a.stride != 1 || a.mode_in || a.mode_out || a.accumulate || a.bst_y || a.pair_n) return SATCV_ERR_UNSUPPORTED;
  if (!(cin == 16 || cin == 32 || cin == 64) || !(a.cout == 32 || a.cout == 64) || a.cout_pad != a.cout || a.cstat != a.cout) return SATCV_ERR_UNSUPPORTED;
  if (a.x1 && (a.c0 % 8 != 0)) return SATCV_ERR_UNSUPPORTED;
  if (a.w_ % 32 != 0 || a.ldy % 8 != 0 || ((uintptr_t)a.y % 16) != 0 || ((uintptr_t)a.w % 16) != 0) return SATCV_ERR_UNSUPPORTED;
  if (a.pool_y && (a.pool_ld % 8 != 0 || ((uintptr_t)a.pool_y % 16) != 0)) return SATCV_ERR_UNSUPPORTED;
  if (on < 2 && cin != 32) return SATCV_ERR_UNSUPPORTED;
  if (a.cout == 32) {
    if (cin == 16) return tr_cfg<16, 32, 8>(a, st, dry);
    if (cin == 32) return tr_cfg<32, 32, 8>(a, st, dry);
    return tr_cfg<64, 32, 4>(a, st, dry);
  }
  if (cin == 16) return tr_cfg<16, 64, 8>(a, st, dry);
  if (cin == 32) return tr_cfg<32, 64, 8>(a, st, dry);
  return SATCV_ERR_UNSUPPORTED;
}
```

satellite_computervision_amd/csrc/conv_transpose_thin.hip:

```cpp
#include "igemm_common.hpp"
#include <cstdlib>

struct ConvtArgs {
  const void* x; const float* in_scale; const float* in_shift; int in_relu;
  const void* w; const float* bias;
  const float* out_scale; int out_relu;
  void* y; int ldy;
  satcv_stat_t* stats; int stats_ld;
  int h, w_;
  int total_strips;
};

__device__ __forceinline__ unsigned pk_bf16(float a, float b) {
  typedef __bf16 bf16x2 __attribute__((ext_vector_type(2)));
  bf16x2 v;
  v[0] = (bf16)a; v[1] = (bf16)b;
  return __builtin_bit_cast(unsigned, v);
}

template <int CIN, int COUT, int NW, int WPS, int NSPLIT = 1>
__global__ __launch_bounds__(NW * 64, WPS) void convt_thin_kernel(const ConvtArgs a) {
  typedef bf16 T;
  constexpr int KS = CIN / 16, NCOL = 4 * COUT, NTW = NCOL / 32 / NSPLIT, NT = NTW, NCOLW = NTW * 32, NTHREADS = NW * 64;
  static_assert(NTW % 2 == 0 && (NTW * 32) % 64 == 0 && (NSPLIT == 1 || (NTW * 32) % COUT == 0 || COUT % (NTW * 32) == 0), "column blocks of whole 64-channel pairs");
  constexpr size_t W_BYTES = (size_t)CIN * NCOLW * sizeof(T);
  extern __shared__ __attribute__((aligned(16))) unsigned char smem_raw[];
  T* ldsW = reinterpret_cast<T*>(smem_raw);
  float* tab = reinterpret_cast<float*>(smem_raw + W_BYTES);
  constexpr int OPITCH = 144, TAB_FLOATS = (2 * CIN + 2 * COUT > 2 * NW * COUT ? 2 * CIN + 2 * COUT : 2 * NW * COUT);
  unsigned char* ldsO = smem_raw + W_BYTES + (size_t)TAB_FLOATS * sizeof(float) + (size_t)(threadIdx.x >> 6) * (32 * OPITCH);
  const int tid = threadIdx.x, lane = tid & 63, wave = tid >> 6;
  const int r = lane & 31, hh = lane >> 5;

  {
    const T* wp = reinterpret_cast<const T*>(a.w);
    const int col0 = (int)((blockIdx.x >> 3) % NSPLIT) * NCOLW;
    for (int it = tid; it < (CIN / 8) * NCOLW; it += NTHREADS) lstore8<T>(ldsW + (size_t)it * 8, gload8<T>(wp + ((size_t)(it / NCOLW) * NCOL + col0 + it % NCOLW) * 8));
    for (int ch = tid; ch < CIN; ch += NTHREADS) {
      tab[ch] = a.in_scale ? a.in_scale[ch] : 1.f;
      tab[CIN + ch] = a.in_scale ? a.in_shift[ch] : 0.f;
    }
    for (int ch = tid; ch < COUT; ch += NTHREADS) { tab[2 * CIN + ch] = a.bias ? a.bias[ch] : 0.f; tab[2 * CIN + COUT + ch] = a.out_scale ? a.out_scale[ch] : 1.f; }
  }
  __syncthreads();
  const bool xaff = a.in_scale != nullptr;
  const unsigned relu_lim = a.in_relu != 0 ? 0u : 0x80008000u;
  const unsigned orelu_lim = a.out_relu != 0 ? 0u : 0x80008000u;
  const bool want_stats = a.stats != nullptr;

  const int G = gridDim.x / NSPLIT;
  const int xcd = blockIdx.x & 7, jx = blockIdx.x >> 3, by = jx % NSPLIT, gj = jx / NSPLIT;
  const int gnt0 = __builtin_amdgcn_readfirstlane(by * NTW);
  const int nx = G >> 3, remx = G & 7;
  const int bid = (xcd < remx ? xcd * (nx + 1) : remx * (nx + 1) + (xcd - remx) * nx) + gj;
  const int gw = __builtin_amdgcn_readfirstlane(bid * NW + wave), GW = G * NW;
  const int per = a.total_strips / GW, extra = a.total_strips % GW;
  const int t_lo = gw * per + (gw < extra ? gw : extra), t_hi = t_lo + per + (gw < extra ? 1 : 0);

  const T* xlane = reinterpret_cast<const T*>(a.x) + (size_t)r * CIN + hh * 8;
  const T* wlane = ldsW + (size_t)(hh * NCOLW + r) * 8;
  const int wo = 2 * a.w_;
  float st1[NT], st2[NT];
#pragma unroll
// ... 66 lines not shown
      {
        const int ij = ((gnt0 + 2 * np) * 32) / COUT, cbp = ((gnt0 + 2 * np) * 32) % COUT;
        T* yrow = reinterpret_cast<T*>(a.y) + ((size_t)(2 * row + (ij >> 1)) * wo + 2 * x0 + (COUT == 32 ? 0 : (ij & 1))) * a.ldy + (COUT == 32 ? 0 : cbp);
#pragma unroll
        for (int m = 0; m < 4; ++m) {
          const int c = lane + 64 * m, q = c >> 3, piece = c & 7;
          const uint4 v = *reinterpret_cast<const uint4*>(ldsO + q * OPITCH + piece * 16);
          const int eoff = COUT == 32 ? (2 * q + (piece >> 2)) * a.ldy + (piece & 3) * 8 : 2 * q * a.ldy + piece * 8;
          *reinterpret_cast<uint4*>(yrow + eoff) = v;
        }
      }
      if (want_stats) {
#pragma unroll
        for (int u = 0; u < 2; ++u) {
          const int cb = ((gnt0 + 2 * np + u) * 32) % COUT;
          const float bv = tab[2 * CIN + cb + r];
          float s1 = 0.f, s2 = 0.f;
#pragma unroll
          for (int i = 0; i < 16; ++i) {
            const float fv = (float)(T)(accD[u][i] + bv);
            s1 += fv; s2 += fv * fv;
          }
          st1[2 * np + u] += s1; st2[2 * np + u] += s2;
        }
      }
    }
  }
  if (want_stats) {
    float c1[COUT / 32], c2[COUT / 32];
#pragma unroll
    for (int u = 0; u < COUT / 32; ++u) { c1[u] = 0.f; c2[u] = 0.f; }
#pragma unroll
    for (int nt = 0; nt < NT; ++nt) {
      const int grp = (gnt0 + nt) % (COUT / 32);
#pragma unroll
      for (int u = 0; u < COUT / 32; ++u) { c1[u] += u == grp ? st1[nt] : 0.f; c2[u] += u == grp ? st2[nt] : 0.f; }
    }
    __syncthreads();
    float* red = tab;
#pragma unroll
    for (int u = 0; u < COUT / 32; ++u) {
      const float s1 = c1[u] + __shfl_xor(c1[u], 32, 64), s2 = c2[u] + __shfl_xor(c2[u], 32, 64);
      if (hh == 0) { red[(wave * 2 + 0) * COUT + u * 32 + r] = s1; red[(wave * 2 + 1) * COUT + u * 32 + r] = s2; }
    }
    __syncthreads();
    if (tid < COUT) {
      float t1 = 0.f, t2 = 0.f;
#pragma unroll
      for (int w = 0; w < NW; ++w) { t1 += red[(w * 2 + 0) * COUT + tid]; t2 += red[(w * 2 + 1) * COUT + tid]; }
      satcv_stat_t* rowp = a.stats + (size_t)(blockIdx.x % SATCV_STAT_ROWS) * 2 * a.stats_ld;
      atomicAdd(rowp + tid, (satcv_stat_t)t1);
      atomicAdd(rowp + a.stats_ld + tid, (satcv_stat_t)t2);
    }
  }
}

template <int CIN, int COUT, int NW, int WPS, int NSPLIT = 1>
static int convt_thin_cfg(const ConvtArgs& ca, hipStream_t st) {
  constexpr size_t lds = (size_t)CIN * 4 * COUT / NSPLIT * sizeof(bf16) + (size_t)(2 * CIN + 2 * COUT > 2 * NW * COUT ? 2 * CIN + 2 * COUT : 2 * NW * COUT) * sizeof(float) + (size_t)NW * 32 * 144;
  auto kern = convt_thin_kernel<CIN, COUT, NW, WPS, NSPLIT>;
  { const int rc = satcv_ensure_dynamic_lds(reinterpret_cast<const void*>(kern), lds); if (rc) return rc; }
  static const int cus = [] {
    int dev = 0, v = 256;
    hipDeviceProp_t p;
    if (hipGetDevice(&dev) == hipSuccess && hipGetDeviceProperties(&p, dev) == hipSuccess && p.multiProcessorCount > 0) v = p.multiProcessorCount;
    return v;
  }();
  int per_cu = WPS * 4 / NW;
  while (per_cu > 1 && (size_t)per_cu * lds > 150 * 1024) --per_cu;
  if (per_cu < 1) per_cu = 1;
  long long grid = (long long)cus * per_cu;
  const long long need = (ca.total_strips + NW - 1) / NW * NSPLIT;
  if (grid > need) grid = need;
  if (NSPLIT > 1) { grid -= grid % (8 * NSPLIT); if (grid < 8 * NSPLIT) grid = 8 * NSPLIT; }
  if (grid < 1) grid = 1;
  hipLaunchKernelGGL(kern, dim3((unsigned)grid), dim3(NW * 64), lds, st, ca);
  hipError_t e = hipGetLastError();
  if (e != hipSuccess) { satcv_set_error("convt_thin launch: %s", hipGetErrorString(e)); return SATCV_ERR_HIP; }
  return SATCV_OK;
}

struct ConvtDgradArgs {
  const void* dy; int lddy;
  const void* w;
  void* dx; int lddx;
  satcv_stat_t* stats; int stats_ld;
  const void* bst_y; int bst_ld;
  const float* bst_scale; const float* bst_shift; const float* bst_mean; const float* bst_rstd; int bst_relu;
  int h, w_, total_strips;
};

template <int CIN, int COUT, int NW, int WPS>
__global__ __launch_bounds__(NW * 64, WPS) void convt_thin_dgrad_kernel(const ConvtDgradArgs a) {
  typedef bf16 T;
  constexpr int K = 4 * COUT, KS = K / 16, NT = CIN / 32, NP = NT / 2, NTHREADS = NW * 64, KPP = COUT / 16;
  constexpr size_t W_BYTES = (size_t)K * CIN * sizeof(T);
  constexpr int OPITCH = 144, TAB_FLOATS = (4 * CIN > 2 * NW * CIN ? 4 * CIN : 2 * NW * CIN);
  extern __shared__ __attribute__((aligned(16))) unsigned char smem_raw[];
  T* ldsW = reinterpret_cast<T*>(smem_raw);
  float* tab = reinterpret_cast<float*>(smem_raw + W_BYTES);
  unsigned char* ldsO = smem_raw + W_BYTES + (size_t)TAB_FLOATS * sizeof(float) + (size_t)(threadIdx.x >> 6) * (32 * OPITCH);
  const int tid = threadIdx.x, lane = tid & 63, wave = tid >> 6;
  const int r = lane & 31, hh = lane >> 5;
  const bool bst = a.bst_y != nullptr;
  {
    const T* wp = reinterpret_cast<const T*>(a.w);
// ... 134 lines not shown
      atomicAdd(rowp + tid, (satcv_stat_t)t1);
      atomicAdd(rowp + a.stats_ld + tid, (satcv_stat_t)(((double)t2 - (double)a.bst_mean[tid] * (double)t1) * (double)a.bst_rstd[tid]));
    }
  }
}

template <int CIN, int COUT, int NW, int WPS>
static int convt_thin_dgrad_cfg(const ConvtDgradArgs& ca, hipStream_t st) {
  constexpr size_t lds = (size_t)4 * COUT * CIN * sizeof(bf16) + (size_t)(4 * CIN > 2 * NW * CIN ? 4 * CIN : 2 * NW * CIN) * sizeof(float) + (size_t)NW * 32 * 144;
  auto kern = convt_thin_dgrad_kernel<CIN, COUT, NW, WPS>;
  { const int rc = satcv_ensure_dynamic_lds(reinterpret_cast<const void*>(kern), lds); if (rc) return rc; }
  static const int cus = [] {
    int dev = 0, v = 256;
    hipDeviceProp_t p;
    if (hipGetDevice(&dev) == hipSuccess && hipGetDeviceProperties(&p, dev) == hipSuccess && p.multiProcessorCount > 0) v = p.multiProcessorCount;
    return v;
  }();
  int per_cu = WPS * 4 / NW;
  while (per_cu > 1 && (size_t)per_cu * lds > 150 * 1024) --per_cu;
  if (per_cu < 1) per_cu = 1;
  long long grid = (long long)cus * per_cu;
  const long long need = (ca.total_strips + NW - 1) / NW;
  if (grid > need) grid = need;
  if (grid < 1) grid = 1;
  hipLaunchKernelGGL(kern, dim3((unsigned)grid), dim3(NW * 64), lds, st, ca);
  hipError_t e = hipGetLastError();
  if (e != hipSuccess) { satcv_set_error("convt_thin_dgrad launch: %s", hipGetErrorString(e)); return SATCV_ERR_HIP; }
  return SATCV_OK;
}

int convt_thin_dgrad_launch(const IgemmArgs& a, int dtype, hipStream_t st) {
  static const bool on = [] { const char* e = getenv("SATCV_CONVT_THIN"); return !e || atoi(e) != 0; }();
  if (!on || dtype != SATCV_BF16 || a.pair_n) return SATCV_ERR_UNSUPPORTED;
  if (a.kh != 1 || a.kw != 1 || a.mode_in != 1 || a.mode_out != 0 || a.f != 2 || a.x1 || a.stride != 1) return SATCV_ERR_UNSUPPORTED;
  if (a.out_scale || a.pool_y || a.accumulate || a.out_relu || a.in_scale || a.bias || a.bst_y1) return SATCV_ERR_UNSUPPORTED;
  if ((a.stats != nullptr) != (a.bst_y != nullptr)) return SATCV_ERR_UNSUPPORTED;
  const int cout_t = a.c0, cin = a.cout;
  if (a.cout_pad != cin || a.w_ % 32 != 0 || a.ldy % 8 != 0 || a.ldy < cin) return SATCV_ERR_UNSUPPORTED;
  if (((uintptr_t)a.y % 16) != 0 || ((uintptr_t)a.x0 % 16) != 0 || ((uintptr_t)a.w % 16) != 0) return SATCV_ERR_UNSUPPORTED;
  if (a.bst_y && (a.bst_ld % 8 != 0 || a.bst_ld < cin || ((uintptr_t)a.bst_y % 16) != 0 || a.stats_ld < cin || a.cstat != cin)) return SATCV_ERR_UNSUPPORTED;
  const long long strips = (long long)a.n * a.h * a.w_ / 32;
  if (strips < 8 || strips > 0x3ffffff) return SATCV_ERR_UNSUPPORTED;
  ConvtDgradArgs ca;
  ca.dy = a.x0; ca.lddy = a.c0; ca.w = a.w; ca.dx = a.y; ca.lddx = a.ldy; ca.stats = a.stats; ca.stats_ld = a.stats_ld;
  ca.bst_y = a.bst_y; ca.bst_ld = a.bst_ld; ca.bst_scale = a.bst_scale; ca.bst_shift = a.bst_shift; ca.bst_mean = a.bst_mean; ca.bst_rstd = a.bst_rstd;
  ca.bst_relu = a.bst_relu;
  ca.h = a.h; ca.w_ = a.w_; ca.total_strips = (int)strips;
  static const bool all = [] { const char* e = getenv("SATCV_CONVT_THIN"); return e && atoi(e) >= 2; }();
  if (cin == 64 && cout_t == 32 && all) return convt_thin_dgrad_cfg<64, 32, 4, 3>(ca, st);
  if (cin == 128 && cout_t == 64) return convt_thin_dgrad_cfg<128, 64, 8, 2>(ca, st);
  return SATCV_ERR_UNSUPPORTED;
}

int convt_thin_launch(const IgemmArgs& a, int dtype, hipStream_t st) {
  static const bool on = [] { const char* e = getenv("SATCV_CONVT_THIN"); return !e || atoi(e) != 0; }();
  if (!on || dtype != SATCV_BF16 || a.pair_n) return SATCV_ERR_UNSUPPORTED;
  if (a.kh != 1 || a.kw != 1 || a.mode_out != 1 || a.mode_in != 0 || a.f != 2 || a.x1 || a.stride != 1) return SATCV_ERR_UNSUPPORTED;
  if (a.pool_y || a.accumulate || a.bst_y || ((a.out_scale || a.out_relu) && a.stats)) return SATCV_ERR_UNSUPPORTED;
  const int cin = a.c0, cout_t = a.cstat;
  if (a.cout != 4 * cout_t || a.cout_pad != 4 * cout_t) return SATCV_ERR_UNSUPPORTED;
  if (a.w_ % 32 != 0 || a.ldy % 8 != 0 || a.ldy < cout_t || ((uintptr_t)a.y % 16) != 0 || ((uintptr_t)a.x0 % 16) != 0 || ((uintptr_t)a.w % 16) != 0) return SATCV_ERR_UNSUPPORTED;
  const long long strips = (long long)a.n * a.h * a.w_ / 32;
  if (strips < 8 || strips > 0x3ffffff) return SATCV_ERR_UNSUPPORTED;
  if (a.stats && a.stats_ld < cout_t) return SATCV_ERR_UNSUPPORTED;
  ConvtArgs ca;
  ca.x = a.x0; ca.in_scale = a.in_scale; ca.in_shift = a.in_shift; ca.in_relu = a.in_relu;
  ca.w = a.w; ca.bias = a.bias; ca.out_scale = a.out_scale; ca.out_relu = a.out_relu; ca.y = a.y; ca.ldy = a.ldy; ca.stats = a.stats; ca.stats_ld = a.stats_ld;
  ca.h = a.h; ca.w_ = a.w_; ca.total_strips = (int)strips;
  static const int wps = [] { const char* e = getenv("SATCV_CONVT_WPS"); return e ? atoi(e) : 3; }();
  if (cin == 64 && cout_t == 32) {
    if (wps == 2) return convt_thin_cfg<64, 32, 4, 2>(ca, st);
    return convt_thin_cfg<64, 32, 4, 3>(ca, st);
  }
  if (cin == 128 && cout_t == 64) return convt_thin_cfg<128, 64, 8, 2>(ca, st);
  static const bool mid = [] { const char* e = getenv("SATCV_CONVT_MID"); return !e || atoi(e) != 0; }();
  if (cin == 256 && cout_t == 128 && mid) return convt_thin_cfg<256, 128, 8, 2, 4>(ca, st);
  return SATCV_ERR_UNSUPPORTED;
}
```

satellite_computervision_amd/csrc/elementwise.hip:

```cpp
#include "common.hpp"
#include <cstdlib>

#define EW_BLOCK 256
static inline int ew_grid(long long items, int cap = 0) {
  static const int dflt = [] { const char* e = getenv("SATCV_EW_PER_CU"); const int v = e ? atoi(e) : 6; return 256 * (v >= 1 ? v : 6); }();
  if (cap <= 0) cap = dflt;
  long long b = (items + EW_BLOCK - 1) / EW_BLOCK;
  if (b < 1) b = 1;
  if (b > cap) b = cap;
  return (int)b;
}
#define LAUNCH_OK(name)                                                          \
  do {                                                                           \
    hipError_t e__ = hipGetLastError();                                          \
    if (e__ != hipSuccess) {                                                     \
      satcv_set_error(name " launch: %s", hipGetErrorString(e__));               \
      return SATCV_ERR_HIP;                                                      \
    }                                                                            \
  } while (0)
#define DISPATCH_T(dtype, ...)                                                   \
  do {                                                                           \
    if ((dtype) == SATCV_BF16) { using T = bf16; __VA_ARGS__; }                  \
    else if ((dtype) == SATCV_F32) { using T = float; __VA_ARGS__; }             \
    else { satcv_set_error("bad dtype %d", (int)(dtype)); return SATCV_ERR_INVALID; } \
// ... 126 lines not shown
      else { if (k < j.taps * j.cout && nn < j.cin) x = j.src[(size_t)k * j.cin + nn]; }
      v[e] = x;
    }
    store8<T>(reinterpret_cast<T*>(j.dst) + it * 8, v);
  }
}
extern "C" int64_t satcv_pack_job_items(const satcv_pack_job* j) {
  if (!j || j->kpad <= 0 || j->kpad % 8 || j->npad <= 0 || j->mode < 0 || j->mode > 3) return -1;
  const int64_t real = (int64_t)(j->mode >= 2 ? 1 : j->taps) * (j->kpad / 8) * j->npad;
  return (real + EW_BLOCK - 1) / EW_BLOCK * EW_BLOCK;
}
extern "C" int satcv_pack_weights_batched(const satcv_pack_job* jobs_dev, const int64_t* prefix_dev, int32_t njobs, int64_t total_items, int32_t dtype,
                                          void* stream) {
  SATCV_CHECK(jobs_dev && prefix_dev && njobs > 0 && total_items > 0, "pack_weights_batched: bad args");
  SATCV_CHECK(total_items % EW_BLOCK == 0, "pack_weights_batched: the prefix table must be built from satcv_pack_job_items (multiples of 256)");
  DISPATCH_T8(dtype, hipLaunchKernelGGL(pack_batched_kernel<T>, dim3(ew_grid(total_items)), dim3(EW_BLOCK), 0, (hipStream_t)stream, jobs_dev,
                                        (const long long*)prefix_dev, njobs, (long long)total_items));
  LAUNCH_OK("pack_weights_batched");
  return SATCV_OK;
}

extern "C" int satcv_pack_weights(const float* src, void* dst_fwd, void* dst_dgrad, int32_t kh, int32_t kw, int32_t cin, int32_t cout, int32_t cin_pad, int32_t transposed, int32_t dtype, void* stream) {
  SATCV_CHECK(src && cin > 0 && cout > 0 && cin_pad >= cin && cin_pad % 16 == 0, "pack_weights: bad args");
  const int taps = kh * kw;
  hipStream_t st = (hipStream_t)stream;
  if (dtype == SATCV_FP8X) {
    SATCV_CHECK(dst_fwd && !dst_dgrad && cin_pad % 16 == 0, "pack_weights: the scaled fp8 image is forward-only, cin_pad %% 16 == 0");
    const int kp = cin_pad, np = rup(transposed ? taps * cout : cout, 32);
    const long long items = (long long)(transposed ? 1 : taps) * (kp / 16) * np;
    hipLaunchKernelGGL((pack_kernel<fp8, 16>), dim3(ew_grid(items)), dim3(EW_BLOCK), 0, st, src, (fp8*)dst_fwd, transposed ? 2 : 0, taps, cin, cout, kp, np);
    LAUNCH_OK("pack_weights");
    return SATCV_OK;
  }
  DISPATCH_T8(dtype, {
    if (!transposed) {
      if (dst_fwd) { const int kp = cin_pad, np = rup(cout, 32);
        hipLaunchKernelGGL(pack_kernel<T>, dim3(ew_grid((long long)taps * (kp / 8) * np)), dim3(EW_BLOCK), 0, st, src, (T*)dst_fwd, 0, taps, cin, cout, kp, np); }
      if (dst_dgrad) { const int kp = rup(cout, 16), np = rup(cin, 32);
        hipLaunchKernelGGL(pack_kernel<T>, dim3(ew_grid((long long)taps * (kp / 8) * np)), dim3(EW_BLOCK), 0, st, src, (T*)dst_dgrad, 1, taps, cin, cout, kp, np); }
    } else {
      if (dst_fwd) { const int kp = cin_pad, np = rup(taps * cout, 32);
        hipLaunchKernelGGL(pack_kernel<T>, dim3(ew_grid((long long)(kp / 8) * np)), dim3(EW_BLOCK), 0, st, src, (T*)dst_fwd, 2, taps, cin, cout, kp, np); }
      if (dst_dgrad) { const int kp = rup(taps * cout, 16), np = rup(cin, 32);
        hipLaunchKernelGGL(pack_kernel<T>, dim3(ew_grid((long long)(kp / 8) * np)), dim3(EW_BLOCK), 0, st, src, (T*)dst_dgrad, 3, taps, cin, cout, kp, np); }
    }
  });
  LAUNCH_OK("pack_weights");
  return SATCV_OK;
}

__global__ void bn_finalize_train_kernel(satcv_stat_t* stats, int ld, int c, float count, const float* gamma, const float* beta,
                                         float eps, float momentum, int updates, int bessel, float* mm, float* mv,
                                         float* scale, float* shift, float* mean_o, float* rstd_o) {
  static_assert(SATCV_STAT_ROWS == 32, "one lane per replica row");
  const int ch = blockIdx.x * (blockDim.x / 32) + threadIdx.x / 32, r = threadIdx.x & 31;
  double s1 = 0.0, s2 = 0.0;
  float gam = 0.f, bet = 0.f, mm0 = 0.f, mv0 = 0.f;
  if (ch < c) {
    satcv_stat_t* row = stats + (size_t)r * 2 * ld;
    s1 = row[ch]; s2 = row[ld + ch];
    if (r == 0) { gam = gamma[ch]; bet = beta[ch]; if (mm) { mm0 = mm[ch]; mv0 = mv[ch]; } }
    row[ch] = 0.0; row[ld + ch] = 0.0;
  }
#pragma unroll
  for (int o = 16; o > 0; o >>= 1) { s1 += __shfl_xor(s1, o, 64); s2 += __shfl_xor(s2, o, 64); }
  if (ch >= c || r != 0) return;
  const double mean_d = s1 / (double)count;
  const float mean = (float)mean_d;
  float var = (float)(s2 / (double)count - mean_d * mean_d);
  var = fmaxf(var, 0.f);
  const float rstd = rsqrtf(var + eps);
  const float sc = gam * rstd;
  scale[ch] = sc; shift[ch] = bet - mean * sc;
  mean_o[ch] = mean; rstd_o[ch] = rstd;
  if (mm) {
    const float vv = bessel ? var * (count / fmaxf(count - 1.f, 1.f)) : var;
    float a = mm0, b = mv0;
    for (int u = 0; u < updates; ++u) { a = a * momentum + mean * (1.f - momentum); b = b * momentum + vv * (1.f - momentum); }
    mm[ch] = a; mv[ch] = b;
  }
}
extern "C" int satcv_bn_finalize_train(satcv_stat_t* stats, int32_t stats_ld, int32_t c, float count, const float* gamma, const float* beta,
                                       float eps, float momentum, int32_t updates, int32_t bessel, float* moving_mean, float* moving_var,
                                       float* scale, float* shift, float* mean, float* rstd, void* stream) {
  SATCV_CHECK(stats && gamma && beta && scale && shift && mean && rstd && c > 0 && stats_ld >= c && count > 0, "bn_finalize_train: bad args");
  hipLaunchKernelGGL(bn_finalize_train_kernel, dim3(cdiv(c, 8)), dim3(256), 0, (hipStream_t)stream, stats, stats_ld, c, count, gamma, beta,
                     eps, momentum, updates, bessel, moving_mean, moving_var, scale, shift, mean, rstd);
  LAUNCH_OK("bn_finalize_train");
  return SATCV_OK;
}
__global__ void bn_affine_infer_kernel(const float* gamma, const float* beta, const float* mm, const float* mv, float eps, int c, float* scale, float* shift) {
  const int ch = blockIdx.x * blockDim.x + threadIdx.x;
  if (ch >= c) return;
  const float sc = gamma[ch] / sqrtf(mv[ch] + eps);
  scale[ch] = sc; shift[ch] = beta[ch] - mm[ch] * sc;
}
extern "C" int satcv_bn_affine_infer(const float* gamma, const float* beta, const float* moving_mean, const float* moving_var, float eps, int32_t c, float* scale, float* shift, void* stream) {
  SATCV_CHECK(gamma && beta && moving_mean && moving_var && scale && shift && c > 0, "bn_affine_infer: bad args");
  hipLaunchKernelGGL(bn_affine_infer_kernel, dim3(cdiv(c, 128)), dim3(128), 0, (hipStream_t)stream, gamma, beta, moving_mean, moving_var, eps, c, scale, shift);
  LAUNCH_OK("bn_affine_infer");
  return SATCV_OK;
}

__global__ void bn_affine_infer_batched_kernel(const satcv_bn_affine_job* __restrict__ jobs, float eps) {
  const satcv_bn_affine_job j = jobs[blockIdx.x];
  for (int ch = threadIdx.x; ch < j.c; ch += blockDim.x) {
    const float sc = j.gamma[ch] / sqrtf(j.moving_var[ch] + eps);
    const float sh = j.beta[ch] - j.moving_mean[ch] * sc;
    j.scale[ch] = sc; j.shift[ch] = sh;
    if (j.bias_eff) j.bias_eff[ch] = sh + (j.conv_bias ? j.conv_bias[ch] * sc : 0.f);
  }
}
extern "C" int satcv_bn_affine_infer_batched(const satcv_bn_affine_job* jobs_device, int32_t njobs, float eps, void* stream) {
  SATCV_CHECK(jobs_device && njobs > 0, "bn_affine_infer_batched: bad args");
  hipLaunchKernelGGL(bn_affine_infer_batched_kernel, dim3(njobs), dim3(256), 0, (hipStream_t)stream, jobs_device, eps);
  LAUNCH_OK("bn_affine_infer_batched");
  return SATCV_OK;
}

__device__ __forceinline__ void block_channel_reduce(float* lds, const float (&a)[8], const float (&b)[8], int g, bool active,
                                                     int c, satcv_stat_t* out, int out_ld, int c_out = -1) {
  const int G = c / 8;
  if (c_out < 0) c_out = c;
  const int pitch = blockDim.x + 8;
#pragma unroll
  for (int e = 0; e < 8; ++e) { lds[e * pitch + threadIdx.x] = active ? a[e] : 0.f; lds[(8 + e) * pitch + threadIdx.x] = active ? b[e] : 0.f; }
  __syncthreads();
  const int g0 = (int)((blockIdx.x * (long long)blockDim.x) % G);
  satcv_stat_t* row = out + (size_t)(blockIdx.x % SATCV_STAT_ROWS) * 2 * out_ld;
  for (int i = threadIdx.x; i < 2 * c_out; i += blockDim.x) {
    const int which = i / c_out, ch = i - which * c_out, gg = ch / 8, e = ch % 8;
    float s = 0.f;
    for (int t = (gg - g0 + G) % G; t < (int)blockDim.x; t += G) s += lds[(which * 8 + e) * pitch + t];
// ... 392 lines not shown
}
static int bnbwd_check(const satcv_bnbwd_desc* d, bool apply) {
  SATCV_CHECK(d && d->yraw && d->scale && d->shift && d->mean && d->rstd, "bn_bwd: null pointer");
  SATCV_CHECK(d->da || d->dpool, "bn_bwd: no incoming gradient");
  SATCV_CHECK(d->c > 0 && d->c % 8 == 0 && d->c <= 2048 && d->n > 0 && d->h > 0 && d->w_ > 0, "bn_bwd: bad dims");
  SATCV_CHECK(!d->dpool || d->f >= 1, "bn_bwd: pool factor");
  SATCV_CHECK(!apply || !d->sk_sums || (d->c_split > 0 && !d->dbias && d->sk_sums_ld >= d->c_split), "bn_bwd_apply: sk_sums needs the two-source form");
  if (apply) SATCV_CHECK(d->coef && d->dy, "bn_bwd_apply: coef/dy missing");
  else SATCV_CHECK(d->sums && d->sums_ld >= d->c, "bn_bwd_reduce: sums missing");
  if (d->c_split > 0) {
    SATCV_CHECK(d->c_split % 8 == 0 && d->c_split < d->c && d->yraw1 && d->ldy1 >= d->c - d->c_split && !d->dpool && d->da && !d->dbias &&
                (long long)d->n * d->h * d->w_ < 0x7fffffffLL, "bn_bwd: second source needs the dense form (da, no dpool / dbias), c_split %% 8 == 0");
    if (apply) SATCV_CHECK(!d->dy1 || d->lddy1 >= d->c - d->c_split, "bn_bwd_apply: dy1 channel stride");
  }
  return SATCV_OK;
}
extern "C" int satcv_bn_bwd_reduce(const satcv_bnbwd_desc* d, void* stream) {
  int rc = bnbwd_check(d, false); if (rc) return rc;
  const int f = d->dpool ? d->f : 1;
  const long long items = (long long)d->n * cdiv(d->h, f) * cdiv(d->w_, f) * (d->c / 8);
  const int grid = ew_grid((items + 7) / 8);
  if (!d->dpool && d->da && (long long)d->n * d->h * d->w_ < 0x7fffffffLL) {
    DISPATCH_T(d->dtype, hipLaunchKernelGGL((bn_bwd_dense_kernel<T, false>), dim3(grid), dim3(EW_BLOCK), (EW_BLOCK + 8) * 16 * sizeof(float), (hipStream_t)stream, *d, 0, d->c));
  } else {
    DISPATCH_T(d->dtype, hipLaunchKernelGGL((bn_bwd_kernel<T, false>), dim3(grid), dim3(EW_BLOCK), (EW_BLOCK + 8) * 16 * sizeof(float), (hipStream_t)stream, *d));
  }
  LAUNCH_OK("bn_bwd_reduce");
  return SATCV_OK;
}
extern "C" int satcv_bn_bwd_apply(const satcv_bnbwd_desc* d, void* stream) {
  static const int rev = getenv("SATCV_BN_REV") ? atoi(getenv("SATCV_BN_REV")) : 1;
  int rc = bnbwd_check(d, true); if (rc) return rc;
  const int f = d->dpool ? d->f : 1;
  if (d->c_split > 0 && !d->dy1) {
    satcv_bnbwd_desc e = *d;
    e.c = d->c_split; e.c_split = 0; e.yraw1 = nullptr;
    const long long it1 = (long long)d->n * d->h * d->w_ * (e.c / 8);
    const size_t lds_1 = d->sk_sums ? (EW_BLOCK + 8) * 16 * sizeof(float) : e.c * sizeof(float);
    DISPATCH_T(d->dtype, bn_bwd_apply_dense_launch<T>(e, it1, lds_1, rev, d->c, (hipStream_t)stream));
    LAUNCH_OK("bn_bwd_apply");
    return SATCV_OK;
  }
  const long long items = (long long)d->n * cdiv(d->h, f) * cdiv(d->w_, f) * (d->c / 8);
  if (!d->dpool && d->da && (long long)d->n * d->h * d->w_ < 0x7fffffffLL) {
    const size_t lds_b = d->sk_sums ? (EW_BLOCK + 8) * 16 * sizeof(float) : d->c * sizeof(float);
    DISPATCH_T(d->dtype, bn_bwd_apply_dense_launch<T>(*d, items, lds_b, rev, d->c, (hipStream_t)stream));
  } else {
    DISPATCH_T(d->dtype, hipLaunchKernelGGL((bn_bwd_kernel<T, true>), dim3(ew_grid(items)), dim3(EW_BLOCK), d->c * sizeof(float), (hipStream_t)stream, *d));
  }
  LAUNCH_OK("bn_bwd_apply");
  return SATCV_OK;
}
__global__ void bn_bwd_finalize_kernel(satcv_stat_t* sums, int ld, int c, float count, float* dgamma, float* dbeta, float* coef, int accumulate) {
  const int ch = blockIdx.x * (blockDim.x / 32) + threadIdx.x / 32, r = threadIdx.x & 31;
  double d1 = 0.0, d2 = 0.0;
  if (ch < c) {
    satcv_stat_t* row = sums + (size_t)r * 2 * ld;
    d1 = row[ch]; d2 = row[ld + ch];
    row[ch] = 0.0; row[ld + ch] = 0.0;
  }
#pragma unroll
  for (int o = 16; o > 0; o >>= 1) { d1 += __shfl_xor(d1, o, 64); d2 += __shfl_xor(d2, o, 64); }
  if (ch >= c || r != 0) return;
  const float s1 = (float)d1, s2 = (float)d2;
  if (dbeta) dbeta[ch] = accumulate ? dbeta[ch] + s1 : s1;
  if (dgamma) dgamma[ch] = accumulate ? dgamma[ch] + s2 : s2;
  coef[ch] = s1 / count; coef[c + ch] = s2 / count;
}
__global__ void bn_bwd_finalize2_kernel(satcv_stat_t* sums, int ld, satcv_stat_t* asums, int ald, int c, float count, const float* scale, const float* shift,
                                        const float* mean, const float* rstd, float* dgamma, float* dbeta, float* coef, int accumulate) {
  const int ch = blockIdx.x * (blockDim.x / 32) + threadIdx.x / 32, r = threadIdx.x & 31;
  double d1 = 0.0, d2 = 0.0, a1 = 0.0, a2 = 0.0;
  if (ch < c) {
    if (sums) { satcv_stat_t* row = sums + (size_t)r * 2 * ld; d1 = row[ch]; d2 = row[ld + ch]; row[ch] = 0.0; row[ld + ch] = 0.0; }
    satcv_stat_t* arow = asums + (size_t)r * 2 * ald;
    a1 = arow[ch]; a2 = arow[ald + ch]; arow[ch] = 0.0; arow[ald + ch] = 0.0;
  }
#pragma unroll
  for (int o = 16; o > 0; o >>= 1) {
    d1 += __shfl_xor(d1, o, 64); d2 += __shfl_xor(d2, o, 64); a1 += __shfl_xor(a1, o, 64); a2 += __shfl_xor(a2, o, 64);
  }
  if (ch >= c || r != 0) return;
  const double sc = (double)scale[ch], sh = (double)shift[ch], mu = (double)mean[ch], rs = (double)rstd[ch];
  const double a2x = sc != 0.0 ? (a2 - (sh + sc * mu) * a1) * (rs / sc) : 0.0;
  const float s1 = (float)(d1 + a1), s2 = (float)(d2 + a2x);
  if (dbeta) dbeta[ch] = accumulate ? dbeta[ch] + s1 : s1;
  if (dgamma) dgamma[ch] = accumulate ? dgamma[ch] + s2 : s2;
  coef[ch] = s1 / count; coef[c + ch] = s2 / count;
}
extern "C" int satcv_bn_bwd_finalize2(satcv_stat_t* sums, int32_t sums_ld, satcv_stat_t* act_sums, int32_t act_sums_ld, int32_t c, float count,
                                      const float* scale, const float* shift, const float* mean, const float* rstd, float* dgamma, float* dbeta,
                                      float* coef, int32_t accumulate, void* stream) {
  SATCV_CHECK(act_sums && coef && scale && shift && mean && rstd && c > 0 && act_sums_ld >= c && (!sums || sums_ld >= c) && count > 0, "bn_bwd_finalize2: bad args");
  hipLaunchKernelGGL(bn_bwd_finalize2_kernel, dim3(cdiv(c, 8)), dim3(256), 0, (hipStream_t)stream, sums, sums_ld, act_sums, act_sums_ld, c, count, scale, shift,
                     mean, rstd, dgamma, dbeta, coef, accumulate);
  LAUNCH_OK("bn_bwd_finalize2");
  return SATCV_OK;
}
extern "C" int satcv_bn_bwd_finalize(satcv_stat_t* sums, int32_t sums_ld, int32_t c, float count, float* dgamma, float* dbeta, float* coef, int32_t accumulate,
                                     void* stream) {
  SATCV_CHECK(sums && coef && c > 0 && sums_ld >= c && count > 0, "bn_bwd_finalize: bad args");
  hipLaunchKernelGGL(bn_bwd_finalize_kernel, dim3(cdiv(c, 8)), dim3(256), 0, (hipStream_t)stream, sums, sums_ld, c, count, dgamma, dbeta, coef, accumulate);
  LAUNCH_OK("bn_bwd_finalize");
  return SATCV_OK;
}

#define HEAD_NCMAX 8
template <typename T>
__global__ void head_fwd_kernel(const satcv_head_desc d) {
  extern __shared__ float lds[];
  const int cin = d.cin, nc = d.ncls;
  float* lw = lds; float* lb = lw + cin * nc; float* lsc = lb + nc; float* lsh = lsc + cin;
  for (int i = threadIdx.x; i < cin * nc; i += blockDim.x) lw[i] = d.w[i];
  for (int i = threadIdx.x; i < nc; i += blockDim.x) lb[i] = d.b[i];
  for (int i = threadIdx.x; i < cin; i += blockDim.x) { lsc[i] = d.in_scale ? d.in_scale[i] : 1.f; lsh[i] = d.in_shift ? d.in_shift[i] : 0.f; }
  __syncthreads();
  const T* x = (const T*)d.x;
  const bool tr = d.in_scale != nullptr;
  for (long long p = blockIdx.x * (long long)blockDim.x + threadIdx.x; p < d.npix; p += (long long)gridDim.x * blockDim.x) {
    float z[HEAD_NCMAX];
#pragma unroll
    for (int k = 0; k < HEAD_NCMAX; ++k) z[k] = k < nc ? lb[k] : -INFINITY;
    for (int g = 0; g < cin / 8; ++g) {
      float v[8];
      load8<T>(x + p * d.ldx + g * 8, v);
#pragma unroll
      for (int e = 0; e < 8; ++e) {
        const int ch = g * 8 + e;
        const float a = tr ? fmaxf(v[e] * lsc[ch] + lsh[ch], 0.f) : v[e];
#pragma unroll
        for (int k = 0; k < HEAD_NCMAX; ++k) if (k < nc) z[k] += a * lw[ch * nc + k];
      }
    }
    if (d.activation == 2) {
#pragma unroll
      for (int k = 0; k < HEAD_NCMAX; ++k) if (k < nc) d.probs[p * nc + k] = z[k];
    } else if (d.activation == 0) {
      float mx = z[0]; int am = 0;
#pragma unroll
      for (int k = 1; k < HEAD_NCMAX; ++k) if (k < nc && z[k] > mx) { mx = z[k]; }
      float s = 0.f, ex[HEAD_NCMAX];
// ... 885 lines not shown
```

satellite_computervision_amd/csrc/igemm_common.hpp:

```cpp
#pragma once
#include "common.hpp"

struct IgemmArgs {
  const void* x0; const void* x1;
  int c0, c1;
  const float* in_scale; const float* in_shift; int in_relu;
  const void* w; const float* bias; const float* out_scale;
  void* pool_y; int pool_ld, pool_f;
  void* y; int ldy;
  satcv_stat_t* stats; int stats_ld;
  int n, h, w_;
  int hs, ws;
  int cout, cout_pad;
  int kh, kw, dil;
  int mode_in, mode_out, f;
  int cstat, out_relu, accumulate, stride;
  int tiles_x, tiles_y, ngroups;
  int rpi, imgs, seg, rl, cl, pitch, halh, halw;
  int n_tiles;
  int nchunks;
  int halh_tl, halw_tl;
  int taploop, cpt;
  const void* bst_y; const void* bst_y1; int bst_ld, bst_ld1, bst_split;
  const float* bst_scale; const float* bst_shift; const float* bst_mean; const float* bst_rstd; int bst_relu;
  int dbg;
  int ksplit; float* kslab;
  int tile_policy;
  int pair_n, pair_c0, pair_c1;
};

template <typename T>
struct FragT;
template <>
struct FragT<bf16> { bf16x8 v; };
template <>
struct FragT<float> { float4 lo, hi; };
template <>
struct FragT<fp8> { long v; };
template <>
struct FragT<fp8s> { i32x4 lo, hi; };

template <typename T>
__device__ __forceinline__ FragT<T> lds_frag(const T* p, int sub_stride = 0) {
  FragT<T> f;
  if constexpr (std::is_same<T, fp8s>::value) {
    f.lo = *reinterpret_cast<const i32x4*>(p);
    f.hi = *reinterpret_cast<const i32x4*>(p + sub_stride);
  } else if constexpr (std::is_same<T, bf16>::value) {
    f.v = *reinterpret_cast<const bf16x8*>(p);
  } else if constexpr (std::is_same<T, fp8>::value) {
    f.v = *reinterpret_cast<const long*>(p);
  } else {
    f.lo = reinterpret_cast<const float4*>(p)[0];
    f.hi = reinterpret_cast<const float4*>(p)[1];
  }
  return f;
}

template <typename T>
__device__ __forceinline__ void mma32(f32x16& acc, const FragT<T>& a, const FragT<T>& b) {
  if constexpr (std::is_same<T, bf16>::value) {
#ifdef SATCV_EXP_M16
    typedef float f32x4_ __attribute__((ext_vector_type(4)));
    f32x4_ c0 = {acc[0], acc[1], acc[2], acc[3]}, c1 = {acc[8], acc[9], acc[10], acc[11]};
    c0 = __builtin_amdgcn_mfma_f32_16x16x32_bf16(a.v, b.v, c0, 0, 0, 0);
    c1 = __builtin_amdgcn_mfma_f32_16x16x32_bf16(a.v, b.v, c1, 0, 0, 0);
    acc[0] = c0[0]; acc[1] = c0[1]; acc[2] = c0[2]; acc[3] = c0[3];
    acc[8] = c1[0]; acc[9] = c1[1]; acc[10] = c1[2]; acc[11] = c1[3];
#else
    acc = __builtin_amdgcn_mfma_f32_32x32x16_bf16(a.v, b.v, acc, 0, 0, 0);
#endif
  } else if constexpr (std::is_same<T, fp8>::value) {
    acc = __builtin_amdgcn_mfma_f32_32x32x16_fp8_fp8(a.v, b.v, acc, 0, 0, 0);
  } else if constexpr (std::is_same<T, fp8s>::value) {
    const i32x8 av = __builtin_shufflevector(a.lo, a.hi, 0, 1, 2, 3, 4, 5, 6, 7);
    const i32x8 bv = __builtin_shufflevector(b.lo, b.hi, 0, 1, 2, 3, 4, 5, 6, 7);
    acc = __builtin_amdgcn_mfma_scale_f32_32x32x64_f8f6f4(av, bv, acc, 0, 0, 0, 0x7f7f7f7f, 0, 0x7f7f7f7f);
  } else {
    acc = __builtin_amdgcn_mfma_f32_32x32x2f32(a.lo.x, b.lo.x, acc, 0, 0, 0);
    acc = __builtin_amdgcn_mfma_f32_32x32x2f32(a.lo.y, b.lo.y, acc, 0, 0, 0);
    acc = __builtin_amdgcn_mfma_f32_32x32x2f32(a.lo.z, b.lo.z, acc, 0, 0, 0);
// ... 357 lines not shown
    } else if (ncols - vq * EPV >= EPV) {
      *reinterpret_cast<uint4*>(yp + off) = *reinterpret_cast<const uint4*>(sp);
    } else {
      for (int e = 0; e < ncols - vq * EPV; ++e) yp[off + e] = sp[e];
    }
  }
  if (a.pool_y) {
    const int f = a.pool_f, pw = TW / f, ph = (BM / TW) / f;
    const int hp = a.h / f, wp = a.w_ / f;
    T* pp = reinterpret_cast<T*>(a.pool_y);
    for (int it = tid; it < ph * pw * VPR; it += NTHREADS) {
      const int vq = it % VPR, pq = it / VPR;
      if (vq * EPV + EPV > ncols) continue;
      const int t0 = (pq / pw) * f, c0 = (pq % pw) * f;
      const int k = (a.imgs == 1) ? 0 : t0 / a.rpi;
      const int nimg = n0 + k, y = y0 + (t0 - k * a.rpi), x = x0 + c0;
      if (!((k < a.imgs) && (nimg < a.n) && (y + f <= a.h) && (x + f <= a.w_))) continue;
      float mx[EPV];
#pragma unroll
      for (int e = 0; e < EPV; ++e) mx[e] = -INFINITY;
      for (int i = 0; i < f; ++i)
        for (int j = 0; j < f; ++j) {
          const T* sp = ldsO + ((t0 + i) * TW + c0 + j) * OPITCH + vq * EPV;
#pragma unroll
          for (int e = 0; e < EPV; ++e) mx[e] = fmaxf(mx[e], (float)sp[e]);
        }
      T o[EPV];
#pragma unroll
      for (int e = 0; e < EPV; ++e) o[e] = (T)mx[e];
      *reinterpret_cast<uint4*>(pp + ((size_t)(nimg * hp + y / f) * wp + x / f) * a.pool_ld + cbase + vq * EPV) = *reinterpret_cast<const uint4*>(o);
    }
  }
}

__host__ __device__ constexpr int igemm_pitch(int tw, int cl, bool m16) {
  return (tw == 32 || (m16 && tw == 16)) ? cl : (tw == 16 ? ((cl + 15) / 16) * 16 : (cl <= 8 ? 8 : ((cl - 8 + 15) / 16) * 16 + 8));
}

static inline int igemm_pick_tw(int w) {
  int best = 8, bestpad = cdiv(w, 8) * 8;
  const int cands[2] = {16, 32};
  for (int i = 0; i < 2; ++i) {
    int p = cdiv(w, cands[i]) * cands[i];
    if (p <= bestpad) { best = cands[i]; bestpad = p; }
  }
  return best;
}

int igemm_fast_launch(IgemmArgs& a, int dtype, hipStream_t st, bool dry_run = false);
int igemm_m16_launch(IgemmArgs& a, int dtype, hipStream_t st, bool dry);
int igemm_m16p_launch(IgemmArgs& a, int dtype, hipStream_t st, bool dry);
int igemm_ws_launch(IgemmArgs& a, int dtype, hipStream_t st, bool dry_run);
int igemm_tr_launch(IgemmArgs& a, int dtype, hipStream_t st, bool dry);
int convt_thin_launch(const IgemmArgs& a, int dtype, hipStream_t st);
int convt_thin_dgrad_launch(const IgemmArgs& a, int dtype, hipStream_t st);
```

satellite_computervision_amd/engine.py:

```python
import ctypes as C
import os
import itertools
from collections import defaultdict
from fractions import Fraction

import numpy as np
import torch

from . import ops, parallel
from ._lib import lib, check, F32, BF16, STAT_ROWS

_M16_DEFAULT = int(os.environ.get('SATCV_M16', '1'))

BN_EPS = 1e-3
BN_MOMENTUM = 0.99


class KTensor:
    _ids = itertools.count()

    def __init__(self, node, channels, down=Fraction(1), name=None):
        self.id = next(KTensor._ids)
        self.node, self.channels, self.down, self.name = node, channels, down, name

# ... 205 lines not shown
    def plan(self, n, h, w, training):
        frozen = tuple(sorted(l.name for l in self.model.layers if not l.trainable)) if training else ()
        raw_bn = tuple(sorted(self.zero_gamma)) if training else ()
        key = (n, h, w, bool(training), frozen, raw_bn)
        if key not in self.plans:
            self.plans[key] = Plan(self, n, h, w, training, frozen, raw_bn)
        return self.plans[key]


class Plan:

    def __init__(self, rt, n, h, w, training, frozen=(), raw_bn=()):
        self.rt, self.n, self.h, self.w, self.training = rt, n, h, w, training
        self.frozen = set(frozen)
        self.raw_bn = set(raw_bn)
        self.tile_policy = 2 if (training and _M16_DEFAULT == 1) else 0
        self.eo_lo, self.early_opt, self.eo_done = None, None, False
        self.fwd, self.bwd = [], []
        self.keep = []
        self.dropouts = []
        self.x_inputs = []
        self.x_by_tid = {}
        self.x_src = {}
        _sp = os.environ.get('SATCV_SIDE_PRIORITY')
        self.side = (torch.cuda.Stream(priority=int(_sp)) if _sp is not None else torch.cuda.Stream()) if (training and rt.model.wgrad_side_stream) else None
        self.step_count = 0
        self.outputs = {}
        self.sync_bn = bool(training and getattr(rt.model, 'sync_bn', False) and parallel.active())
        self.amax_of = {}
        self._bn_jobs = []
        self._build()
        if self._bn_jobs:
            tab = torch.tensor([[int(v or 0) for v in j] for j in self._bn_jobs], dtype=torch.int64).to(rt.dev)
            self.keep.append(tab)
            nj = len(self._bn_jobs)
            self.fwd.insert(0, lambda st: check(lib.satcv_bn_affine_infer_batched(tab.data_ptr(), nj, BN_EPS, st)))

    def _z(self, *shape, dtype=None):
        t = torch.zeros(*shape, dtype=dtype or self.rt.tdtype, device=self.rt.dev)
        self.keep.append(t)
        return t

    def _dims(self, t):
        hh, ww = self.h * t.down, self.w * t.down
        if hh.denominator != 1 or ww.denominator != 1:
            raise ValueError(f'input {self.h}x{self.w} is not divisible by the model downsampling ({1 / t.down})')
        return int(hh), int(ww)

    def _conv_step(self, role='fwd', **kw):
        kw.setdefault('tile_policy', self.tile_policy)
        d = ops.make_conv_desc(**kw)
        self.keep.append(d)
        fn = lambda st, d=d: check(lib.satcv_conv2d_igemm(C.byref(d), st))
        k, cin, cout = kw.get('kh', 1) * kw.get('kw', 1), kw.get('c0', 0) + (kw.get('c1', 0) or 0), kw['cout']
        px = kw['n'] * kw['h'] * kw['w_']
        fn.label = (f"conv_{role} k{kw.get('kh', 1)} d{kw.get('dil', 1)} n{kw['n']} {kw['h']}x{kw['w_']} {kw.get('c0', 0)}+{kw.get('c1', 0) or 0}->{cout}"
                    f"{' d2s' if kw.get('mode_out') else ''}{' s2d' if kw.get('mode_in') else ''}")
        fn.work = dict(kind='conv', role=role, taps=k, px=px, cin=cin, cout=cout, esize=self.rt.esize)
        return fn

    def _src_args(self, r):
        (x0, c0) = r.srcs[0]
        x1, c1 = (r.srcs[1] if len(r.srcs) > 1 else (None, 0))
        a = r.affine
        return dict(x0=x0.data_ptr(), c0=c0, x1=x1.data_ptr() if x1 is not None else None, c1=c1,
                    in_scale=_fp(a['scale']) if a else None, in_shift=_fp(a['shift']) if a else None,
                    in_relu=1 if (a and r.relu) else 0)

    def _bn_forward(self, bnname, stats, ld, off, c, count, updates, aff=None, aoff=0, conv_bias=None, bias_eff=None):
        rt = self.rt
        a = aff or dict(scale=self._z(c, dtype=torch.float32), shift=self._z(c, dtype=torch.float32),
                        mean=self._z(c, dtype=torch.float32), rstd=self._z(c, dtype=torch.float32))
        g, b = rt.pptr(bnname + '/gamma'), rt.pptr(bnname + '/beta')
        mm, mv = rt.sptr(bnname + '/moving_mean'), rt.sptr(bnname + '/moving_var')
        if self.training:
            bessel = 1 if rt.model.bn_bessel else 0
            if self.sync_bn:
                self.fwd.append(lambda st: parallel.allreduce_mean_(stats))
            if bnname in self.frozen:
                ts, tt = self._z(c, dtype=torch.float32), self._z(c, dtype=torch.float32)
                self.fwd.append(lambda st: check(lib.satcv_bn_finalize_train(
                    _fp(stats, off), ld, c, float(count), g, b, BN_EPS, BN_MOMENTUM, updates, bessel, None, None,
                    _fp(ts), _fp(tt), _fp(a['mean'], aoff), _fp(a['rstd'], aoff), st)))
                self.fwd.append(lambda st: check(lib.satcv_bn_affine_infer(g, b, mm, mv, BN_EPS, c, _fp(a['scale'], aoff), _fp(a['shift'], aoff), st)))
                return a
            self.fwd.append(lambda st: check(lib.satcv_bn_finalize_train(
                _fp(stats, off), ld, c, float(count), g, b, BN_EPS, BN_MOMENTUM, updates, bessel, mm, mv,
                _fp(a['scale'], aoff), _fp(a['shift'], aoff), _fp(a['mean'], aoff), _fp(a['rstd'], aoff), st)))
        else:
            self._bn_jobs.append((g, b, mm, mv, _fp(a['scale'], aoff), _fp(a['shift'], aoff), c, conv_bias, bias_eff))
        return a

    def _materialize(self, t, r, f=1, pooled=None, sink=None, actslot=None):
        if not r.relu:
            raise NotImplementedError('materialising a linear (no-ReLU) BatchNorm output')
        (y, c) = r.srcs[0]
        hh, ww = r.h, r.w
        if actslot is None:
            act = self._z(self.n, hh, ww, c)
            act_ptr, act_ld = act.data_ptr(), c
        else:
            act = actslot[0]
            act_ptr, act_ld = actslot[0].data_ptr() + actslot[1] * self.rt.esize, actslot[2]
        st_ptr, ld = (None, 0)
        if sink is not None and self.training:
            st_ptr, ld = _fp(sink[0], sink[1]), sink[2]
        a = r.affine
        dt = self.rt.dtype
        if (self.training and pooled is not None and f == 2 and dt == BF16 and getattr(self.rt.model, 'fuse_pool_bwd', True)
                and hh % 8 == 0 and ww % 32 == 0 and c in (32, 64)):
            amax = self._z(self.n, hh // 2, ww // 2, c, dtype=torch.uint8)
            self.amax_of[t.id] = amax
            self.fwd.append(lambda st: check(lib.satcv_bn_relu_pool_amax(
                y.data_ptr(), _fp(a['scale']), _fp(a['shift']), act_ptr, act_ld, pooled.data_ptr(), amax.data_ptr(),
                st_ptr, ld, self.n, hh, ww, c, f, dt, st)))
            return TRef([(act, c)], self.n, hh, ww) if actslot is None else None
        self.fwd.append(lambda st: check(lib.satcv_bn_relu_pool(
            y.data_ptr(), _fp(a['scale']), _fp(a['shift']), act_ptr, act_ld, pooled.data_ptr() if pooled is not None else None,
            st_ptr, ld, self.n, hh, ww, c, f, dt, st)))
        return TRef([(act, c)], self.n, hh, ww) if actslot is None else None

    def _build(self):
        rt, m, n = self.rt, self.rt.model, self.n
        T, dt, es = rt.tdtype, rt.dtype, rt.esize
        training = self.training
        consumers = defaultdict(list)
        for node in m.nodes:
            for t in node.inputs:
                consumers[t.id].append(node)
        vals, acts, ctx = {}, {}, {}
        sinks, cat_stats = {}, {}
        order = {id(nd): i for i, nd in enumerate(m.nodes)}
        fused_join = {}
        folded_plain = {}
        for node in m.nodes:
            if node.op == 'concat_bn_relu':
                a, b = node.inputs
# ... 1047 lines not shown
```

satellite_computervision_amd/model_tools.py:

```python
import ctypes as C
import json
import os
import time
from collections import defaultdict
from fractions import Fraction

import numpy as np
import torch

from . import engine as E
from . import ops
from ._lib import lib, check, F32, BF16

_DEFAULT_DTYPE = 'bfloat16'
_RNG = np.random.default_rng(0)
_UIDS = defaultdict(int)


def set_compute_dtype(name):
    global _DEFAULT_DTYPE
    assert name in ('bfloat16', 'float32')
    _DEFAULT_DTYPE = name


# ... 636 lines not shown
            s['done'] = torch.cuda.Event()
            s['done'].record(cs)
        s['multi'] = isinstance(b[0], (list, tuple))
        s['rest'] = tuple(b[2:])

    cur = 0
    upload(first, slots[0])
    while True:
        s = slots[cur]
        main.wait_event(s['done'])
        yield ((s['x'] if s['multi'] else s['x'][0]), s['y']) + s['rest']
        s['free'] = torch.cuda.Event()
        s['free'].record(main)
        try:
            nb = next(it)
        except StopIteration:
            return
        if not is_host_pair(nb):
            yield nb
            yield from it
            return
        cur ^= 1
        upload(nb, slots[cur])


class Model:

    def __init__(self, inputs, outputs, name='model', dtype=None):
        self.inputs = list(inputs) if isinstance(inputs, (list, tuple)) else [inputs]
        self.outputs = list(outputs) if isinstance(outputs, (list, tuple)) else [outputs]
        self._single_output = not isinstance(outputs, (list, tuple))
        self.name = name
        self.nodes = E.topo_nodes(self.outputs)
        seen, self.layers, self.param_specs = set(), [], []
        for node in self.nodes:
            lay = node.layer
            subs = [lay] if lay is not None else []
            if node.op == 'cba':
                subs = [l for l in (lay, node.attrs['owner'].bn_layer) if l is not None]
            for l in subs:
                if id(l) not in seen:
                    seen.add(id(l))
                    self.layers.append(l)
                    self.param_specs += l.specs
        self.compute_dtype = dtype or _DEFAULT_DTYPE
        self.bn_bessel = True
        self.fuse_head_bn_bwd = os.environ.get('SATCV_FUSE_HEAD_BN_BWD', '1') != '0'
        self.fuse_dgrad_bn_bwd = os.environ.get('SATCV_FUSE_DGRAD_BN_BWD', '1') != '0'
        self.wgrad_side_stream = os.environ.get('SATCV_WGRAD_STREAM', '1') != '0'
        self.fuse_pool_bn_sums = os.environ.get('SATCV_FUSE_POOL_BN_SUMS', '1') != '0'
        self.fuse_head_grad = os.environ.get('SATCV_FUSE_HEAD_GRAD', '1') != '0'
        self.fuse_pool_bwd = os.environ.get('SATCV_FUSE_POOL_BWD', '1') != '0'
        self.fuse_thin_bwd = os.environ.get('SATCV_FUSE_THIN_BWD', '1') != '0'
        self.sync_bn = os.environ.get('SATCV_SYNC_BN', '0') == '1'
        self._rt = None
        self.optimizer, self._loss, self._metrics = None, None, []
        self.metrics_names = []
        self.stop_training = False
        self._builder = None
        self.output_names = [t.name for t in self.outputs]

    @property
    def runtime(self):
        if self._rt is None:
            self._rt = E.Runtime(self, BF16 if self.compute_dtype == 'bfloat16' else F32)
            if self.optimizer is not None:
                self.optimizer._rt = self._rt
                self._rt.adam_state[0:1].fill_(self.optimizer._lr)
        return self._rt

    def count_params(self):
        return sum(p.size for p in self.param_specs)

    def get_layer(self, name):
        for l in self.layers:
            if l.name == name:
                return l
        raise ValueError(f'No such layer: {name}')

    def get_weights_dict(self):
        rt = self.runtime
        torch.cuda.synchronize()
        return {p.name: rt.get_param(p.name).detach().cpu().numpy().copy() for p in self.param_specs}

    def get_weights(self):
        w = self.get_weights_dict()
        return [w[ps.name] for ps in self.param_specs]

    def set_weights(self, weights):
        weights = list(weights)
        if len(weights) != len(self.param_specs):
            raise ValueError(f'You called `set_weights(weights)` with a weight list of length {len(weights)}, but the model was expecting '
                             f'{len(self.param_specs)} weights.')
        self.set_weights_dict({ps.name: np.asarray(v) for ps, v in zip(self.param_specs, weights)})

    def set_weights_dict(self, d, skip_mismatch=False):
        rt = self.runtime
        for k, v in d.items():
            if k.endswith('/moving_variance'):
                k = k[:-len('moving_variance')] + 'moving_var'
            if k not in rt.specs:
                if skip_mismatch:
                    continue
                raise KeyError(k)
            if tuple(np.shape(v)) != rt.specs[k].shape:
                if skip_mismatch:
# ... 668 lines not shown
```

satellite_computervision_amd/ops.py:

```python
import ctypes as C
import torch

from . import _lib
from ._lib import lib, check, ConvDesc, WgradDesc, BnBwdDesc, HeadDesc, F32, BF16, FP8, FP8X, STAT_ROWS

TORCH_DTYPE = {F32: torch.float32, BF16: torch.bfloat16, FP8: torch.float8_e4m3fn, FP8X: torch.float8_e4m3fn}
DTYPE_CODE = {torch.float32: F32, torch.bfloat16: BF16, torch.float8_e4m3fn: FP8}


def rup(a, b):
    return (a + b - 1) // b * b


def stream_ptr():
    return C.c_void_p(torch.cuda.current_stream().cuda_stream)


def ptr(t):
    if t is None:
        return None
    assert t.is_cuda, 'satcv ops need device tensors (no CPU fallback)'
    return C.c_void_p(t.data_ptr())


def new_stats(c, device):
    return torch.zeros(STAT_ROWS, 2, c, dtype=torch.float64, device=device)


def ingest_nhwc(x_f32, cpad, dtype):
    n, h, w, c = x_f32.shape
    x_f32 = x_f32.contiguous()
    out = torch.empty(n, h, w, cpad, dtype=TORCH_DTYPE[dtype], device=x_f32.device)
    check(lib.satcv_ingest_nhwc(ptr(x_f32), ptr(out), n * h * w, c, cpad, dtype, stream_ptr()))
    return out


def ingest_chw(planes, scale, cpad, dtype):
    n, c, h, w = planes.shape
    kind = {torch.uint8: 0, torch.int16: 1, torch.uint16: 1, torch.float32: 2}[planes.dtype]
    out = torch.empty(n, h, w, cpad, dtype=TORCH_DTYPE[dtype], device=planes.device)
    check(lib.satcv_ingest_chw(ptr(planes.contiguous()), kind, float(scale), ptr(out), n, c, h, w, cpad, dtype, stream_ptr()))
    return out


def packed_sizes(kh, kw, cin, cout, cin_pad, transposed):
    taps = kh * kw
    if not transposed:
        nf, nd = rup(cout, 32), rup(cin, 32)
        return taps * cin_pad * nf, taps * rup(cout, 16) * nd, nf, nd
    nf, nd = rup(taps * cout, 32), rup(cin, 32)
    return cin_pad * nf, rup(taps * cout, 16) * nd, nf, nd


def pack_weights(kernel_f32, cin_pad, dtype, transposed=False, want_dgrad=True, out_fwd=None, out_dgrad=None):
    if transposed:
        kh, kw, cout, cin = kernel_f32.shape
    else:
        kh, kw, cin, cout = kernel_f32.shape
    ef, ed, _, _ = packed_sizes(kh, kw, cin, cout, cin_pad, transposed)
    td = TORCH_DTYPE[dtype]
    fwd = out_fwd if out_fwd is not None else torch.empty(ef, dtype=td, device=kernel_f32.device)
    dg = out_dgrad if out_dgrad is not None else (torch.empty(ed, dtype=td, device=kernel_f32.device) if want_dgrad else None)
    check(lib.satcv_pack_weights(ptr(kernel_f32.contiguous()), ptr(fwd), ptr(dg), kh, kw, cin, cout, cin_pad,
                                 1 if transposed else 0, dtype, stream_ptr()))
    return fwd, dg


def make_conv_desc(*, x0, c0, w, y, ldy, n, h, w_, cout, cout_pad, dtype, x1=None, c1=0, in_scale=None, in_shift=None,
                   in_relu=0, bias=None, stats=None, stats_ld=0, kh=3, kw=3, dil=1, mode_in=0, mode_out=0, f=1,
                   cstat=None, out_relu=0, accumulate=0, stride=1, hin=0, win=0, out_scale=None, pool_y=None, pool_ld=0, pool_f=0, bst=None, tile_policy=0, pair=None):
    d = ConvDesc()
    d.tile_policy = int(tile_policy)
    if pair:
        d.pair_n, d.pair_c0, d.pair_c1 = (int(v) for v in pair)
    d.x0, d.x1, d.c0, d.c1 = x0, x1, c0, c1
    d.in_scale, d.in_shift, d.in_relu = in_scale, in_shift, int(in_relu)
    d.w, d.bias, d.y, d.ldy = w, bias, y, ldy
    d.stats, d.stats_ld = stats, stats_ld
    d.n, d.h, d.w_ = n, h, w_
    d.cout, d.cout_pad = cout, cout_pad
    d.kh, d.kw, d.dil = kh, kw, dil
    d.mode_in, d.mode_out, d.f = mode_in, mode_out, f
    d.cstat = cstat if cstat is not None else cout
    d.out_relu, d.dtype, d.accumulate = int(out_relu), dtype, int(accumulate)
    d.stride, d.hin, d.win, d.out_scale = stride, hin, win, out_scale
    d.pool_y, d.pool_ld, d.pool_f = pool_y, pool_ld, pool_f
    if bst:
        d.bst_y, d.bst_ld, d.bst_y1, d.bst_ld1, d.bst_split = bst['y'], bst['ld'], bst.get('y1'), bst.get('ld1', 0), bst.get('split', 0)
        d.bst_scale, d.bst_shift, d.bst_mean, d.bst_rstd, d.bst_relu = bst['scale'], bst['shift'], bst['mean'], bst['rstd'], int(bst.get('relu', 1))
    return d


def _p(t):
    return t.data_ptr() if t is not None else None


def conv2d(x, w_packed, cout, *, kh=3, kw=3, dil=1, bias=None, x1=None, in_scale=None, in_shift=None, in_relu=False,
           stats=None, out=None, out_relu=False, stride=1, bst=None, out_scale=None, pool_y=None, pool_f=0):
    n, hin, win, c0 = x.shape
    h, w_ = ((hin - 1) // stride + 1, (win - 1) // stride + 1) if stride > 1 else (hin, win)
    dtype = DTYPE_CODE[x.dtype]
    c1 = x1.shape[-1] if x1 is not None else 0
    cpad = rup(cout, 32)
    y = out if out is not None else torch.empty(n, h, w_, rup(cout, 16), dtype=x.dtype, device=x.device)
    d = make_conv_desc(x0=_p(x), c0=c0, x1=_p(x1), c1=c1, w=_p(w_packed), y=_p(y), ldy=y.shape[-1], n=n, h=h, w_=w_,
                       cout=cout, cout_pad=cpad, dtype=dtype, in_scale=_p(in_scale), in_shift=_p(in_shift),
                       in_relu=in_relu, bias=_p(bias), stats=_p(stats), stats_ld=stats.shape[-1] if stats is not None else 0,
                       kh=kh, kw=kw, dil=dil, out_relu=out_relu, stride=stride, hin=hin if stride > 1 else 0, win=win if stride > 1 else 0,
                       out_scale=_p(out_scale), pool_y=_p(pool_y), pool_ld=pool_y.shape[-1] if pool_y is not None else 0, pool_f=pool_f,
                       bst={k: (_p(v) if torch.is_tensor(v) else v) for k, v in bst.items()} if bst else None)
    if bst and lib.satcv_conv2d_igemm_pipelined(C.byref(d)) != 1:
        raise ValueError('conv2d: this shape cannot carry the fused BatchNorm-backward reduce (bst); run satcv_bn_bwd_reduce separately')
    check(lib.satcv_conv2d_igemm(C.byref(d), stream_ptr()))
    return y


def conv2d_transpose(x, w_packed, cout, f, *, bias=None, in_scale=None, in_shift=None, in_relu=False, stats=None, out=None,
                     out_scale=None, out_relu=False):
    n, h, w_, c0 = x.shape
    dtype = DTYPE_CODE[x.dtype]
    y = out if out is not None else torch.empty(n, h * f, w_ * f, rup(cout, 16), dtype=x.dtype, device=x.device)
    d = make_conv_desc(x0=_p(x), c0=c0, w=_p(w_packed), y=_p(y), ldy=y.shape[-1], n=n, h=h, w_=w_, cout=f * f * cout,
                       cout_pad=rup(f * f * cout, 32), dtype=dtype, in_scale=_p(in_scale), in_shift=_p(in_shift),
                       in_relu=in_relu, bias=_p(bias), stats=_p(stats), stats_ld=stats.shape[-1] if stats is not None else 0,
                       kh=1, kw=1, dil=1, mode_out=1, f=f, cstat=cout, out_scale=_p(out_scale), out_relu=out_relu)
    check(lib.satcv_conv2d_igemm(C.byref(d), stream_ptr()))
    return y


def conv2d_dgrad(dy, w_dgrad, cin, *, kh=3, kw=3, dil=1, out=None, accumulate=False):
    n, h, w_, cy = dy.shape
    dtype = DTYPE_CODE[dy.dtype]
    dx = out if out is not None else torch.empty(n, h, w_, rup(cin, 16), dtype=dy.dtype, device=dy.device)
    d = make_conv_desc(x0=_p(dy), c0=cy, w=_p(w_dgrad), y=_p(dx), ldy=dx.shape[-1], n=n, h=h, w_=w_, cout=cin,
                       cout_pad=rup(cin, 32), dtype=dtype, kh=kh, kw=kw, dil=dil, accumulate=accumulate)
    check(lib.satcv_conv2d_igemm(C.byref(d), stream_ptr()))
    return dx


def conv2d_transpose_dgrad(dy, w_dgrad, cin, cout, f, *, out=None, stats=None, bst=None):
    n, hf, wf, cy = dy.shape
    h, w_ = hf // f, wf // f
    dtype = DTYPE_CODE[dy.dtype]
    assert cy == cout, 'dy channel stride must equal cout'
    dx = out if out is not None else torch.empty(n, h, w_, rup(cin, 16), dtype=dy.dtype, device=dy.device)
    d = make_conv_desc(x0=_p(dy), c0=cy, w=_p(w_dgrad), y=_p(dx), ldy=dx.shape[-1], n=n, h=h, w_=w_, cout=cin,
                       cout_pad=rup(cin, 32), dtype=dtype, kh=1, kw=1, dil=1, mode_in=1, f=f,
                       stats=_p(stats), stats_ld=stats.shape[-1] if stats is not None else 0,
                       bst={k: (_p(v) if torch.is_tensor(v) else v) for k, v in bst.items()} if bst else None)
    check(lib.satcv_conv2d_igemm(C.byref(d), stream_ptr()))
    return dx


def make_wgrad_desc(*, x0, c0, dy, lddy, dw, cin, cout, n, h, w_, dtype, x1=None, c1=0, in_scale=None, in_shift=None,
                    in_relu=0, kh=3, kw=3, dil=1, mode_dy=0, f=1, transposed=0, workspace=None, workspace_bytes=0, accumulate=0, whole_chip=0, defer_reduce=0):
    d = WgradDesc()
    d.x0, d.x1, d.c0, d.c1 = x0, x1, c0, c1
    d.in_scale, d.in_shift, d.in_relu = in_scale, in_shift, int(in_relu)
    d.dy, d.lddy, d.dw, d.cin, d.cout = dy, lddy, dw, cin, cout
    d.n, d.h, d.w_, d.kh, d.kw, d.dil = n, h, w_, kh, kw, dil
    d.mode_dy, d.f, d.transposed = mode_dy, f, transposed
    d.workspace, d.workspace_bytes, d.dtype, d.accumulate = workspace, workspace_bytes, dtype, int(accumulate)
    d.whole_chip = int(whole_chip)
    d.defer_reduce = int(defer_reduce)
    return d


def make_bwdf_desc(*, g, yraw, ldg, bn_scale, bn_shift, bn_mean, bn_rstd, bn_coef, x0, c0, w_dgrad, dx, lddx, dw, cin, cout, n, h, w_, dtype,
                   linear=0, x1=None, c1=0, in_scale=None, in_shift=None, in_relu=0, kh=3, kw=3, dil=1, workspace=None, workspace_bytes=0,
                   accumulate=0, bst_sums=None, bst_sums_ld=0, bst_mean=None, bst_rstd=None, bst_act_form=0, dpool=None, lddp=0, amax=None,
                   hg_dlogits=None, hg_w=None, hg_ncls=0):
    from ._lib import BwdfDesc
    d = BwdfDesc()
    d.g, d.yraw, d.ldg = g, yraw, ldg
    d.bn_scale, d.bn_shift, d.bn_mean, d.bn_rstd, d.bn_coef, d.linear = bn_scale, bn_shift, bn_mean, bn_rstd, bn_coef, int(linear)
    d.x0, d.x1, d.c0, d.c1 = x0, x1, c0, c1
    d.in_scale, d.in_shift, d.in_relu = in_scale, in_shift, int(in_relu)
    d.w_dgrad, d.dx, d.lddx, d.dw, d.cin, d.cout = w_dgrad, dx, lddx, dw, cin, cout
    d.n, d.h, d.w_, d.kh, d.kw, d.dil = n, h, w_, kh, kw, dil
    d.workspace, d.workspace_bytes, d.dtype, d.accumulate = workspace, workspace_bytes, dtype, int(accumulate)
    d.bst_sums, d.bst_sums_ld, d.bst_mean, d.bst_rstd, d.bst_act_form = bst_sums, bst_sums_ld, bst_mean, bst_rstd, int(bst_act_form)
    d.dpool, d.lddp, d.amax = dpool, lddp, amax
    d.hg_dlogits, d.hg_w, d.hg_ncls = hg_dlogits, hg_w, int(hg_ncls)
    return d


def conv_bwd_fused(g, yraw, scale, shift, mean, rstd, coef, x, w_dgrad, cin, cout, *, x1=None, in_scale=None, in_shift=None, in_relu=False,
                   linear=False, accumulate_into=None, bst=None, dpool=None, amax=None, want_dx=True, head=None):
    n, h, w_, c0 = x.shape
    c1 = x1.shape[-1] if x1 is not None else 0
    dx = torch.empty(n, h, w_, c0 + c1, dtype=x.dtype, device=x.device) if want_dx else None
    dw = accumulate_into if accumulate_into is not None else torch.empty(3, 3, cin, cout, dtype=torch.float32, device=x.device)
    d = make_bwdf_desc(g=_p(g), yraw=_p(yraw), ldg=g.shape[-1] if g is not None else yraw.shape[-1], bn_scale=_p(scale), bn_shift=_p(shift), bn_mean=_p(mean), bn_rstd=_p(rstd),
                       bn_coef=_p(coef), x0=_p(x), c0=c0, x1=_p(x1), c1=c1, in_scale=_p(in_scale), in_shift=_p(in_shift), in_relu=in_relu,
                       w_dgrad=_p(w_dgrad), dx=_p(dx), lddx=c0 + c1, dw=_p(dw), cin=cin, cout=cout, n=n, h=h, w_=w_, dtype=DTYPE_CODE[x.dtype],
                       linear=linear, accumulate=accumulate_into is not None, dpool=_p(dpool), lddp=dpool.shape[-1] if dpool is not None else 0,
                       amax=_p(amax), **(dict(hg_dlogits=_p(head[0]), hg_w=_p(head[1]), hg_ncls=head[0].shape[-1]) if head else {}),
                       **(dict(bst_sums=_p(bst['sums']), bst_sums_ld=bst['sums'].shape[-1], bst_mean=_p(bst.get('mean')), bst_rstd=_p(bst.get('rstd')),
                               bst_act_form=bst.get('act_form', 0)) if bst else {}))
    nb = lib.satcv_conv2d_bwd_fused_workspace(C.byref(d))
    if nb < 0:
        return None
    ws = torch.empty(max(nb // 4, 1), dtype=torch.float32, device=x.device)
    d.workspace, d.workspace_bytes = ws.data_ptr(), nb
    check(lib.satcv_conv2d_bwd_fused(C.byref(d), stream_ptr()))
    return dx, dw


def conv2d_wgrad(x, dy, cin, cout, *, kh=3, kw=3, dil=1, x1=None, in_scale=None, in_shift=None, in_relu=False,
                 transposed_f=0, dw=None):
    n, h, w_, c0 = x.shape
    dtype = DTYPE_CODE[x.dtype]
    c1 = x1.shape[-1] if x1 is not None else 0
    f = transposed_f
    if dw is None:
        shape = (f, f, cout, cin) if f else (kh, kw, cin, cout)
        dw = torch.empty(shape, dtype=torch.float32, device=x.device)
    d = make_wgrad_desc(x0=_p(x), c0=c0, x1=_p(x1), c1=c1, dy=_p(dy), lddy=dy.shape[-1], dw=_p(dw), cin=cin, cout=cout,
                        n=n, h=h, w_=w_, dtype=dtype, in_scale=_p(in_scale), in_shift=_p(in_shift), in_relu=in_relu,
                        kh=1 if f else kh, kw=1 if f else kw, dil=dil, mode_dy=1 if f else 0, f=f if f else 1,
                        transposed=1 if f else 0)
    nbytes = lib.satcv_conv2d_wgrad_workspace(C.byref(d))
    if nbytes < 0:
        raise _lib.SatcvError(lib.satcv_last_error().decode())
    ws = torch.empty(max(nbytes // 4, 1), dtype=torch.float32, device=x.device)
    d.workspace, d.workspace_bytes = ws.data_ptr(), nbytes
    check(lib.satcv_conv2d_wgrad(C.byref(d), stream_ptr()))
    return dw


def bn_finalize_train(stats, count, gamma, beta, moving_mean, moving_var, eps=1e-3, momentum=0.99, updates=1, bessel=False):
    c = gamma.numel()
    dev = gamma.device
    scale, shift, mean, rstd = (torch.empty(c, dtype=torch.float32, device=dev) for _ in range(4))
    check(lib.satcv_bn_finalize_train(ptr(stats), stats.shape[-1], c, float(count), ptr(gamma), ptr(beta), eps, momentum,
                                      updates, int(bessel), ptr(moving_mean), ptr(moving_var), ptr(scale), ptr(shift),
                                      ptr(mean), ptr(rstd), stream_ptr()))
    return scale, shift, mean, rstd


def bn_affine_infer(gamma, beta, moving_mean, moving_var, eps=1e-3):
    c = gamma.numel()
    scale = torch.empty(c, dtype=torch.float32, device=gamma.device)
    shift = torch.empty_like(scale)
    check(lib.satcv_bn_affine_infer(ptr(gamma), ptr(beta), ptr(moving_mean), ptr(moving_var), eps, c, ptr(scale), ptr(shift), stream_ptr()))
    return scale, shift


def bn_relu_pool(yraw, scale, shift, f, want_act=True, want_pool=True, stats=None):
    n, h, w_, c = yraw.shape
    act = torch.empty_like(yraw) if want_act else None
    pooled = torch.empty(n, h // f, w_ // f, c, dtype=yraw.dtype, device=yraw.device) if want_pool else None
    check(lib.satcv_bn_relu_pool(ptr(yraw), ptr(scale), ptr(shift), ptr(act), 0, ptr(pooled), ptr(stats),
                                 stats.shape[-1] if stats is not None else 0, n, h, w_, c, f, DTYPE_CODE[yraw.dtype], stream_ptr()))
    return act, pooled


def bn_relu_pool_amax(yraw, scale, shift, f):
    n, h, w_, c = yraw.shape
    act = torch.empty_like(yraw)
    pooled = torch.empty(n, h // f, w_ // f, c, dtype=yraw.dtype, device=yraw.device)
    amax = torch.empty(n, h // f, w_ // f, c, dtype=torch.uint8, device=yraw.device)
    check(lib.satcv_bn_relu_pool_amax(ptr(yraw), ptr(scale), ptr(shift), ptr(act), 0, ptr(pooled), ptr(amax), None, 0, n, h, w_, c, f,
                                      DTYPE_CODE[yraw.dtype], stream_ptr()))
    return act, pooled, amax


def make_bnbwd_desc(*, yraw, ldy, scale, shift, mean, rstd, n, h, w_, c, dtype, da=None, ldda=0, dpool=None, lddp=0, f=1,
                    sums=None, sums_ld=0, coef=None, dy=None, lddy_out=0, dbias=None, linear=0, yraw1=None, ldy1=0, dy1=None, lddy1=0,
                    c_split=0, sk_sums=None, sk_sums_ld=0):
    d = BnBwdDesc()
    d.sk_sums, d.sk_sums_ld = sk_sums, sk_sums_ld
    d.linear = linear
    d.yraw1, d.ldy1, d.dy1, d.lddy1, d.c_split = yraw1, ldy1, dy1, lddy1, c_split
    d.da, d.ldda, d.dpool, d.lddp, d.f = da, ldda, dpool, lddp, f
    d.yraw, d.ldy = yraw, ldy
    d.scale, d.shift, d.mean, d.rstd = scale, shift, mean, rstd
    d.sums, d.sums_ld, d.coef = sums, sums_ld, coef
    d.dy, d.lddy_out, d.dbias = dy, lddy_out, dbias
    d.n, d.h, d.w_, d.c, d.dtype = n, h, w_, c, dtype
    return d


# ... 153 lines not shown
```

Measured before the change: 8372 tiles/s.

## Fuse BatchNorm finalize into the producing conv kernel via last-block ticket

Adds a device-side BN finalize job descriptor that conv kernels run in a tail: each workgroup takes an atomic ticket, and the last one to finish reduces the replicated statistics rows and writes scale/shift/mean/rstd and the moving averages. This removes the separate bn_finalize_train launch after each forward conv, cutting launch count and inter-kernel gaps. The cost is an extra global atomic and barrier per workgroup, a serial finalize in one block, and a host fallback launch for kernel variants that cannot carry the tail.

```diff
diff --git a/include/satcv.h b/include/satcv.h
--- a/include/satcv.h
+++ b/include/satcv.h
@@ -31,6 +31,19 @@
 int64_t satcv_pack_job_items(const satcv_pack_job* job);
 int satcv_pack_weights_batched(const satcv_pack_job* jobs_dev, const int64_t* prefix_dev, int32_t njobs, int64_t total_items, int32_t dtype,
                                void* stream);
+
+typedef struct satcv_bn_fin_job {
+  int32_t kind, c;
+  satcv_stat_t* rows; satcv_stat_t* act_rows;
+  int32_t rows_ld, act_rows_ld;
+  float count, eps, momentum;
+  int32_t updates, bessel, accumulate;
+  const float* gamma; const float* beta;
+  float* moving_mean; float* moving_var;
+  float* scale; float* shift; float* mean; float* rstd;
+  float* dgamma; float* dbeta; float* coef;
+  uint32_t* counter;
+} satcv_bn_fin_job;
 
 typedef struct satcv_conv_desc {
   const void* x0;
@@ -61,6 +74,7 @@
   void* pool_y; int32_t pool_ld, pool_f;
   const void* bst_y; const void* bst_y1; int32_t bst_ld, bst_ld1, bst_split;
   const float* bst_scale; const float* bst_shift; const float* bst_mean; const float* bst_rstd; int32_t bst_relu;
+  const satcv_bn_fin_job* fin;
   int32_t tile_policy;
   int32_t pair_n, pair_c0, pair_c1;
 } satcv_conv_desc;
diff --git a/satellite_computervision_amd/_lib.py b/satellite_computervision_amd/_lib.py
--- a/satellite_computervision_amd/_lib.py
+++ b/satellite_computervision_amd/_lib.py
@@ -25,8 +25,16 @@
                 ('cstat', c_i32), ('out_relu', c_i32), ('dtype', c_i32), ('accumulate', c_i32),
                 ('stride', c_i32), ('hin', c_i32), ('win', c_i32), ('out_scale', c_vp), ('pool_y', c_vp), ('pool_ld', c_i32), ('pool_f', c_i32),
                 ('bst_y', c_vp), ('bst_y1', c_vp), ('bst_ld', c_i32), ('bst_ld1', c_i32), ('bst_split', c_i32),
-                ('bst_scale', c_vp), ('bst_shift', c_vp), ('bst_mean', c_vp), ('bst_rstd', c_vp), ('bst_relu', c_i32), ('tile_policy', c_i32),
+                ('bst_scale', c_vp), ('bst_shift', c_vp), ('bst_mean', c_vp), ('bst_rstd', c_vp), ('bst_relu', c_i32), ('fin', c_vp), ('tile_policy', c_i32),
                 ('pair_n', c_i32), ('pair_c0', c_i32), ('pair_c1', c_i32)]
+
+
+class BnFinJob(C.Structure):
+    _fields_ = [('kind', c_i32), ('c', c_i32), ('rows', c_vp), ('act_rows', c_vp), ('rows_ld', c_i32), ('act_rows_ld', c_i32),
+                ('count', c_f32), ('eps', c_f32), ('momentum', c_f32), ('updates', c_i32), ('bessel', c_i32), ('accumulate', c_i32),
+                ('gamma', c_vp), ('beta', c_vp), ('moving_mean', c_vp), ('moving_var', c_vp),
+                ('scale', c_vp), ('shift', c_vp), ('mean', c_vp), ('rstd', c_vp),
+                ('dgamma', c_vp), ('dbeta', c_vp), ('coef', c_vp), ('counter', c_vp)]
 
 
 class PackJob(C.Structure):
diff --git a/satellite_computervision_amd/csrc/common.hpp b/satellite_computervision_amd/csrc/common.hpp
--- a/satellite_computervision_amd/csrc/common.hpp
+++ b/satellite_computervision_amd/csrc/common.hpp
@@ -275,3 +275,91 @@
 __device__ __forceinline__ void dma_wait_all() { asm volatile("s_waitcnt vmcnt(0)" ::: "memory"); }
 
 #define SATCV_STAT_REPL 32
+
+enum { SATCV_FIN_FWD = 0, SATCV_FIN_BWD = 1, SATCV_FIN_BWD_ACT = 2 };
+template <bool COH>
+__device__ __forceinline__ double bn_fin_take(satcv_stat_t* p) {
+  if constexpr (COH) {
+    static_assert(sizeof(satcv_stat_t) == 8, "rows are exchanged as 64-bit words");
+    return __builtin_bit_cast(double, __hip_atomic_exchange(reinterpret_cast<unsigned long long*>(p), 0ull, __ATOMIC_RELAXED, __HIP_MEMORY_SCOPE_AGENT));
+  } else {
+    const double v = *p; *p = 0.0; return v;
+  }
+}
+template <bool COH>
+__device__ __forceinline__ void bn_fin_channel(const satcv_bn_fin_job& j, int ch, int r) {
+  static_assert(SATCV_STAT_ROWS == 32, "one lane per replica row");
+  const int c = j.c;
+  if (j.kind == SATCV_FIN_FWD) {
+    double s1 = 0.0, s2 = 0.0;
+    float gam = 0.f, bet = 0.f, mm0 = 0.f, mv0 = 0.f;
+    float* mm = j.moving_mean; float* mv = j.moving_var;
+    if (ch < c) {
+      satcv_stat_t* row = j.rows + (size_t)r * 2 * j.rows_ld;
+      s1 = bn_fin_take<COH>(row + ch); s2 = bn_fin_take<COH>(row + j.rows_ld + ch);
+      if (r == 0) { gam = j.gamma[ch]; bet = j.beta[ch]; if (mm) { mm0 = mm[ch]; mv0 = mv[ch]; } }
+    }
+#pragma unroll
+    for (int o = 16; o > 0; o >>= 1) { s1 += __shfl_xor(s1, o, 64); s2 += __shfl_xor(s2, o, 64); }
+    if (ch >= c || r != 0) return;
+    const float count = j.count;
+    const double mean_d = s1 / (double)count;
+    const float mean = (float)mean_d;
+    float var = (float)(s2 / (double)count - mean_d * mean_d);
+    var = fmaxf(var, 0.f);
+    const float rstd = rsqrtf(var + j.eps);
+    const float sc = gam * rstd;
+    j.scale[ch] = sc; j.shift[ch] = bet - mean * sc;
+    j.mean[ch] = mean; j.rstd[ch] = rstd;
+    if (mm) {
+      const float momentum = j.momentum;
+      const float vv = j.bessel ? var * (count / fmaxf(count - 1.f, 1.f)) : var;
+      float a = mm0, b = mv0;
+      for (int u = 0; u < j.updates; ++u) { a = a * momentum + mean * (1.f - momentum); b = b * momentum + vv * (1.f - momentum); }
+      mm[ch] = a; mv[ch] = b;
+    }
+    return;
+  }
+  const bool act = j.kind == SATCV_FIN_BWD_ACT;
+  double d1 = 0.0, d2 = 0.0, a1 = 0.0, a2 = 0.0;
+  if (ch < c) {
+    if (j.rows) { satcv_stat_t* row = j.rows + (size_t)r * 2 * j.rows_ld; d1 = bn_fin_take<COH>(row + ch); d2 = bn_fin_take<COH>(row + j.rows_ld + ch); }
+    if (act) { satcv_stat_t* arow = j.act_rows + (size_t)r * 2 * j.act_rows_ld; a1 = bn_fin_take<COH>(arow + ch); a2 = bn_fin_take<COH>(arow + j.act_rows_ld + ch); }
+  }
+#pragma unroll
+  for (int o = 16; o > 0; o >>= 1) { d1 += __shfl_xor(d1, o, 64); d2 += __shfl_xor(d2, o, 64); }
+  if (act) {
+#pragma unroll
+    for (int o = 16; o > 0; o >>= 1) { a1 += __shfl_xor(a1, o, 64); a2 += __shfl_xor(a2, o, 64); }
+  }
+  if (ch >= c || r != 0) return;
+  float s1, s2;
+  if (act) {
+    const double sc = (double)j.scale[ch], sh = (double)j.shift[ch], mu = (double)j.mean[ch], rs = (double)j.rstd[ch];
+    const double a2x = sc != 0.0 ? (a2 - (sh + sc * mu) * a1) * (rs / sc) : 0.0;
+    s1 = (float)(d1 + a1); s2 = (float)(d2 + a2x);
+  } else {
+    s1 = (float)d1; s2 = (float)d2;
+  }
+  if (j.dbeta) j.dbeta[ch] = j.accumulate ? j.dbeta[ch] + s1 : s1;
+  if (j.dgamma) j.dgamma[ch] = j.accumulate ? j.dgamma[ch] + s2 : s2;
+  j.coef[ch] = s1 / j.count; j.coef[c + ch] = s2 / j.count;
+}
+
+__device__ __forceinline__ void bn_fin_tail(const satcv_bn_fin_job* job, unsigned* flag, int tid, int nthreads) {
+  if (!job) return;
+  asm volatile("s_waitcnt vmcnt(0)" ::: "memory");
+  __syncthreads();
+  if (tid == 0) {
+    const unsigned nwg = gridDim.x * gridDim.y * gridDim.z;
+    const unsigned ticket = __hip_atomic_fetch_add(job->counter, 1u, __ATOMIC_RELAXED, __HIP_MEMORY_SCOPE_AGENT);
+    *flag = ticket == nwg - 1 ? 1u : 0u;
+  }
+  __syncthreads();
+  if (*flag == 0u) return;
+  const satcv_bn_fin_job j = *job;
+  const int per = nthreads >> 5;
+  for (int c0 = 0; c0 < j.c; c0 += per) bn_fin_channel<true>(j, c0 + (tid >> 5), tid & 31);
+  if (tid == 0) __hip_atomic_store(j.counter, 0u, __ATOMIC_RELAXED, __HIP_MEMORY_SCOPE_AGENT);
+}
+int satcv_bn_fin_fallback(const satcv_bn_fin_job* job_dev, hipStream_t st);
diff --git a/satellite_computervision_amd/csrc/conv_igemm.hip b/satellite_computervision_amd/csrc/conv_igemm.hip
--- a/satellite_computervision_amd/csrc/conv_igemm.hip
+++ b/satellite_computervision_amd/csrc/conv_igemm.hip
@@ -302,6 +302,8 @@
   a.bst_scale = d->bst_scale; a.bst_shift = d->bst_shift; a.bst_mean = d->bst_mean; a.bst_rstd = d->bst_rstd; a.bst_relu = d->bst_relu;
   a.tile_policy = d->tile_policy;
   a.pair_n = d->pair_n; a.pair_c0 = d->pair_c0; a.pair_c1 = d->pair_c1;
+  SATCV_CHECK(!d->fin || (d->stats && !d->bst_y), "igemm: a finalize job needs the forward statistics rows it finalizes");
+  a.fin = d->fin; a.fin_done = 0;
   if (d->pair_n || d->pair_c0 || d->pair_c1) {
     const int epv = d->dtype == SATCV_F32 ? 4 : (d->dtype == SATCV_BF16 ? 8 : 16);
     SATCV_CHECK(d->pair_n > 0 && d->n == 2 * d->pair_n, "igemm: pair store needs n == 2 * pair_n (n=%d pair_n=%d)", d->n, d->pair_n);
@@ -366,6 +368,7 @@
   else if (d->dtype == SATCV_BF16) rc = launch_t<bf16>(a, st);
   else if (d->dtype == SATCV_F32) rc = launch_t<float>(a, st);
   else { satcv_set_error("igemm: bad dtype %d", d->dtype); rc = SATCV_ERR_INVALID; }
+  if (rc == SATCV_OK && a.fin && !a.fin_done) rc = satcv_bn_fin_fallback(a.fin, st);
   satcv_prof_end(d->kh * d->kw > 1 ? 0 : 1, st);
   return rc;
 }
diff --git a/satellite_computervision_amd/csrc/conv_igemm_fast.hip b/satellite_computervision_amd/csrc/conv_igemm_fast.hip
--- a/satellite_computervision_amd/csrc/conv_igemm_fast.hip
+++ b/satellite_computervision_amd/csrc/conv_igemm_fast.hip
@@ -516,6 +516,7 @@
       return;
     } else
     igemm_epilogue<T, TW, WM, WN, MT, NT, ABL(1), !DYN, true, M16, !DYN && !std::is_same<T, float>::value>(a, acc, n0, y0, x0, nbase, smem_raw);
+    if constexpr (!SK && !DYN && std::is_same<T, bf16>::value && MT * NT >= 4) bn_fin_tail(a.fin, reinterpret_cast<unsigned*>(smem_raw), tid, NTHREADS);
 #ifdef SATCV_STAMP
     {
       unsigned long long k4;
@@ -706,6 +707,7 @@
   hipError_t e = hipGetLastError();
   if (e != hipSuccess) { satcv_set_error("igemm_fast launch: %s", hipGetErrorString(e)); return SATCV_ERR_HIP; }
   if (a.ksplit > 1) return igemm_splitk_finish<T>(a, st);
+  a.fin_done = !SK && !dyn && std::is_same<T, bf16>::value && MT * NT >= 4;
   return SATCV_OK;
 }
 
diff --git a/satellite_computervision_amd/csrc/conv_igemm_m16.hip b/satellite_computervision_amd/csrc/conv_igemm_m16.hip
--- a/satellite_computervision_amd/csrc/conv_igemm_m16.hip
+++ b/satellite_computervision_amd/csrc/conv_igemm_m16.hip
@@ -204,6 +204,7 @@
     return;
   }
   igemm_epilogue<T, TW, WM, WN, MT, NT, false, true, true, true>(a, acc, n0, y0, x0, nbase, smem_raw);
+  bn_fin_tail(a.fin, reinterpret_cast<unsigned*>(smem_raw), threadIdx.x, WM * WN * 64);
 }
 
 template <int TW>
@@ -382,6 +383,7 @@
     interval(std::integral_constant<int, 2>{}, k + 2);
   }
   igemm_epilogue<T, TW, WM, WN, MT, NT, false, true, true, true>(a, acc, n0, y0, x0, nbase, smem_raw);
+  bn_fin_tail(a.fin, reinterpret_cast<unsigned*>(smem_raw), threadIdx.x, WM * WN * 64);
 }
 
 template <int TW>
@@ -416,6 +418,7 @@
   auto kern = roles ? igemm_m16_kernel<TW> : igemm_m16sym_kernel<TW>;
   { const int rc = satcv_ensure_dynamic_lds(reinterpret_cast<const void*>(kern), lds); if (rc) return rc; }
   hipLaunchKernelGGL(kern, dim3((unsigned)blocks), dim3(roles ? 768 : 512), lds, st, a);
+  a.fin_done = 1;
   hipError_t e = hipGetLastError();
   if (e != hipSuccess) { satcv_set_error("igemm_m16 launch: %s", hipGetErrorString(e)); return SATCV_ERR_HIP; }
   return SATCV_OK;
diff --git a/satellite_computervision_amd/csrc/conv_igemm_m16p.hip b/satellite_computervision_amd/csrc/conv_igemm_m16p.hip
--- a/satellite_computervision_amd/csrc/conv_igemm_m16p.hip
+++ b/satellite_computervision_amd/csrc/conv_igemm_m16p.hip
@@ -69,7 +69,10 @@
     m_lo = rr * per + (rr < extra ? rr : extra);
     ntl = per + (rr < extra ? 1 : 0);
   }
-  if (ntl <= 0) return;
+  if (ntl <= 0) {
+    if constexpr (!BST) { if (wave < 8) bn_fin_tail(a.fin, reinterpret_cast<unsigned*>(smem_raw), tid, 512); }
+    return;
+  }
   for (int i = tid; i < BN; i += 768) ldsB[i] = a.bias ? a.bias[nbase + i] : 0.f;
   const bool xaff = !BST && a.in_scale != nullptr;
   if (xaff) {
@@ -481,6 +484,7 @@
       atomicAdd(rowp + a.stats_ld + nbase + wave * 16 + l16, (satcv_stat_t)s2);
     }
   }
+  if constexpr (!BST) bn_fin_tail(a.fin, reinterpret_cast<unsigned*>(smem_raw), tid, 512);
 }
 
 template <int BN>
@@ -529,6 +533,7 @@
   auto kern = a.bst_y ? igemm_m16p_kernel<true, BN> : igemm_m16p_kernel<false, BN>;
   { const int rc = satcv_ensure_dynamic_lds(reinterpret_cast<const void*>(kern), lds); if (rc) return rc; }
   hipLaunchKernelGGL(kern, dim3((unsigned)(ranges * a.n_tiles)), dim3(768), lds, st, a, (int)m_total);
+  a.fin_done = a.bst_y ? 0 : 1;
   ++g_m16p_launches;
   hipError_t e = hipGetLastError();
   if (e != hipSuccess) { satcv_set_error("igemm_m16p launch: %s", hipGetErrorString(e)); return SATCV_ERR_HIP; }
diff --git a/satellite_computervision_amd/csrc/conv_igemm_ws.hip b/satellite_computervision_amd/csrc/conv_igemm_ws.hip
--- a/satellite_computervision_amd/csrc/conv_igemm_ws.hip
+++ b/satellite_computervision_amd/csrc/conv_igemm_ws.hip
@@ -13,6 +13,9 @@
 #define STAMP(t) do { __builtin_amdgcn_sched_barrier(0); asm volatile("s_memtime %0\n\ts_waitcnt lgkmcnt(0)" : "=s"(t) :: "memory"); __builtin_amdgcn_sched_barrier(0); } while (0)
 #define STAMP_V(t) do { __builtin_amdgcn_sched_barrier(0); asm volatile("s_waitcnt vmcnt(0)\n\ts_memtime %0\n\ts_waitcnt lgkmcnt(0)" : "=s"(t) :: "memory"); __builtin_amdgcn_sched_barrier(0); } while (0)
 #endif
+
+template <typename T, int CIN, int WPS, int DIL>
+constexpr bool ws_fin_v = std::is_same<T, bf16>::value && DIL == 1 && !(CIN == 32 && WPS == 3);
 
 template <typename T, int CIN, int NT, int WPS, int WN = 1, int DIL = 1>
 __global__ __launch_bounds__(256 * WN, WPS) void igemm_ws_kernel(const IgemmArgs a, const int total_tiles) {
@@ -187,6 +190,7 @@
     atomicAdd(rowp + tid, (satcv_stat_t)carry[0]);
     atomicAdd(rowp + a.stats_ld + tid, (satcv_stat_t)carry[1]);
   }
+  if constexpr (ws_fin_v<T, CIN, WPS, DIL>) bn_fin_tail(a.fin, reinterpret_cast<unsigned*>(smem_raw), tid, NTHREADS);
 #ifdef SATCV_STAMP
   if (blockIdx.x < 8 && lane == 0)
     for (int i = 0; i < 8; ++i) g_stamp_ws[blockIdx.x][wave][i] = z[i] / (unsigned long long)max(t_hi - t_lo, 1);
@@ -225,6 +229,7 @@
   long long grid = (long long)ncu * per_cu;
   if (grid > total) grid = total;
   hipLaunchKernelGGL(kern, dim3((unsigned)grid), dim3(256 * WN), LDS, st, a, (int)total);
+  a.fin_done = ws_fin_v<T, CIN, WPS, DIL>;
   ++g_ws_launches;
   hipError_t e = hipGetLastError();
   if (e != hipSuccess) { satcv_set_error("igemm_ws launch: %s", hipGetErrorString(e)); return SATCV_ERR_HIP; }
diff --git a/satellite_computervision_amd/csrc/conv_thin_roles.hip b/satellite_computervision_amd/csrc/conv_thin_roles.hip
--- a/satellite_computervision_amd/csrc/conv_thin_roles.hip
+++ b/satellite_computervision_amd/csrc/conv_thin_roles.hip
@@ -192,6 +192,7 @@
         atomicAdd(rowp + a.stats_ld + sid, (satcv_stat_t)t2);
       }
     }
+    bn_fin_tail(a.fin, reinterpret_cast<unsigned*>(smem_raw), sid, NS);
     return;
   }
 
@@ -290,6 +291,7 @@
   long long grid = ncu;
   if (grid > total) grid = total;
   hipLaunchKernelGGL(kern, dim3((unsigned)grid), dim3(768), G::LDS, st, a, (int)total);
+  a.fin_done = 1;
   ++g_ws_launches; ++g_tr_launches;
   hipError_t e = hipGetLastError();
   if (e != hipSuccess) { satcv_set_error("igemm_tr launch: %s", hipGetErrorString(e)); return SATCV_ERR_HIP; }
diff --git a/satellite_computervision_amd/csrc/conv_transpose_thin.hip b/satellite_computervision_amd/csrc/conv_transpose_thin.hip
--- a/satellite_computervision_amd/csrc/conv_transpose_thin.hip
+++ b/satellite_computervision_amd/csrc/conv_transpose_thin.hip
@@ -9,6 +9,7 @@
   satcv_stat_t* stats; int stats_ld;
   int h, w_;
   int total_strips;
+  const satcv_bn_fin_job* fin;
 };
 
 __device__ __forceinline__ unsigned pk_bf16(float a, float b) {
@@ -181,6 +182,7 @@
       atomicAdd(rowp + tid, (satcv_stat_t)t1);
       atomicAdd(rowp + a.stats_ld + tid, (satcv_stat_t)t2);
     }
+    bn_fin_tail(a.fin, reinterpret_cast<unsigned*>(tab), tid, NTHREADS);
   }
 }
 
@@ -421,7 +423,7 @@
   return SATCV_ERR_UNSUPPORTED;
 }
 
-int convt_thin_launch(const IgemmArgs& a, int dtype, hipStream_t st) {
+int convt_thin_launch(IgemmArgs& a, int dtype, hipStream_t st) {
   static const bool on = [] { const char* e = getenv("SATCV_CONVT_THIN"); return !e || atoi(e) != 0; }();
   if (!on || dtype != SATCV_BF16 || a.pair_n) return SATCV_ERR_UNSUPPORTED;
   if (a.kh != 1 || a.kw != 1 || a.mode_out != 1 || a.mode_in != 0 || a.f != 2 || a.x1 || a.stride != 1) return SATCV_ERR_UNSUPPORTED;
@@ -436,6 +438,8 @@
   ca.x = a.x0; ca.in_scale = a.in_scale; ca.in_shift = a.in_shift; ca.in_relu = a.in_relu;
   ca.w = a.w; ca.bias = a.bias; ca.out_scale = a.out_scale; ca.out_relu = a.out_relu; ca.y = a.y; ca.ldy = a.ldy; ca.stats = a.stats; ca.stats_ld = a.stats_ld;
   ca.h = a.h; ca.w_ = a.w_; ca.total_strips = (int)strips;
+  ca.fin = a.fin;
+  a.fin_done = 1;
   static const int wps = [] { const char* e = getenv("SATCV_CONVT_WPS"); return e ? atoi(e) : 3; }();
   if (cin == 64 && cout_t == 32) {
     if (wps == 2) return convt_thin_cfg<64, 32, 4, 2>(ca, st);
@@ -444,5 +448,6 @@
   if (cin == 128 && cout_t == 64) return convt_thin_cfg<128, 64, 8, 2>(ca, st);
   static const bool mid = [] { const char* e = getenv("SATCV_CONVT_MID"); return !e || atoi(e) != 0; }();
   if (cin == 256 && cout_t == 128 && mid) return convt_thin_cfg<256, 128, 8, 2, 4>(ca, st);
+  a.fin_done = 0;
   return SATCV_ERR_UNSUPPORTED;
 }
diff --git a/satellite_computervision_amd/csrc/elementwise.hip b/satellite_computervision_amd/csrc/elementwise.hip
--- a/satellite_computervision_amd/csrc/elementwise.hip
+++ b/satellite_computervision_amd/csrc/elementwise.hip
@@ -202,33 +202,20 @@
 __global__ void bn_finalize_train_kernel(satcv_stat_t* stats, int ld, int c, float count, const float* gamma, const float* beta,
                                          float eps, float momentum, int updates, int bessel, float* mm, float* mv,
                                          float* scale, float* shift, float* mean_o, float* rstd_o) {
-  static_assert(SATCV_STAT_ROWS == 32, "one lane per replica row");
-  const int ch = blockIdx.x * (blockDim.x / 32) + threadIdx.x / 32, r = threadIdx.x & 31;
-  double s1 = 0.0, s2 = 0.0;
-  float gam = 0.f, bet = 0.f, mm0 = 0.f, mv0 = 0.f;
-  if (ch < c) {
-    satcv_stat_t* row = stats + (size_t)r * 2 * ld;
-    s1 = row[ch]; s2 = row[ld + ch];
-    if (r == 0) { gam = gamma[ch]; bet = beta[ch]; if (mm) { mm0 = mm[ch]; mv0 = mv[ch]; } }
-    row[ch] = 0.0; row[ld + ch] = 0.0;
-  }
-#pragma unroll
-  for (int o = 16; o > 0; o >>= 1) { s1 += __shfl_xor(s1, o, 64); s2 += __shfl_xor(s2, o, 64); }
-  if (ch >= c || r != 0) return;
-  const double mean_d = s1 / (double)count;
-  const float mean = (float)mean_d;
-  float var = (float)(s2 / (double)count - mean_d * mean_d);
-  var = fmaxf(var, 0.f);
-  const float rstd = rsqrtf(var + eps);
-  const float sc = gam * rstd;
-  scale[ch] = sc; shift[ch] = bet - mean * sc;
-  mean_o[ch] = mean; rstd_o[ch] = rstd;
-  if (mm) {
-    const float vv = bessel ? var * (count / fmaxf(count - 1.f, 1.f)) : var;
-    float a = mm0, b = mv0;
-    for (int u = 0; u < updates; ++u) { a = a * momentum + mean * (1.f - momentum); b = b * momentum + vv * (1.f - momentum); }
-    mm[ch] = a; mv[ch] = b;
-  }
+  satcv_bn_fin_job j = {};
+  j.kind = SATCV_FIN_FWD; j.c = c; j.rows = stats; j.rows_ld = ld; j.count = count; j.eps = eps; j.momentum = momentum;
+  j.updates = updates; j.bessel = bessel; j.gamma = gamma; j.beta = beta; j.moving_mean = mm; j.moving_var = mv;
+  j.scale = scale; j.shift = shift; j.mean = mean_o; j.rstd = rstd_o;
+  bn_fin_channel<false>(j, blockIdx.x * (blockDim.x / 32) + threadIdx.x / 32, threadIdx.x & 31);
+}
+__global__ __launch_bounds__(256) void bn_fin_job_kernel(const satcv_bn_fin_job* job) {
+  const satcv_bn_fin_job j = *job;
+  for (int c0 = blockIdx.x * 8; c0 < j.c; c0 += gridDim.x * 8) bn_fin_channel<false>(j, c0 + threadIdx.x / 32, threadIdx.x & 31);
+}
+int satcv_bn_fin_fallback(const satcv_bn_fin_job* job_dev, hipStream_t st) {
+  hipLaunchKernelGGL(bn_fin_job_kernel, dim3(32), dim3(256), 0, st, job_dev);
+  LAUNCH_OK("bn_fin_job");
+  return SATCV_OK;
 }
 extern "C" int satcv_bn_finalize_train(satcv_stat_t* stats, int32_t stats_ld, int32_t c, float count, const float* gamma, const float* beta,
                                        float eps, float momentum, int32_t updates, int32_t bessel, float* moving_mean, float* moving_var,
@@ -727,41 +714,17 @@
   return SATCV_OK;
 }
 __global__ void bn_bwd_finalize_kernel(satcv_stat_t* sums, int ld, int c, float count, float* dgamma, float* dbeta, float* coef, int accumulate) {
-  const int ch = blockIdx.x * (blockDim.x / 32) + threadIdx.x / 32, r = threadIdx.x & 31;
-  double d1 = 0.0, d2 = 0.0;
-  if (ch < c) {
-    satcv_stat_t* row = sums + (size_t)r * 2 * ld;
-    d1 = row[ch]; d2 = row[ld + ch];
-    row[ch] = 0.0; row[ld + ch] = 0.0;
-  }
-#pragma unroll
-  for (int o = 16; o > 0; o >>= 1) { d1 += __shfl_xor(d1, o, 64); d2 += __shfl_xor(d2, o, 64); }
-  if (ch >= c || r != 0) return;
-  const float s1 = (float)d1, s2 = (float)d2;
-  if (dbeta) dbeta[ch] = accumulate ? dbeta[ch] + s1 : s1;
-  if (dgamma) dgamma[ch] = accumulate ? dgamma[ch] + s2 : s2;
-  coef[ch] = s1 / count; coef[c + ch] = s2 / count;
+  satcv_bn_fin_job j = {};
+  j.kind = SATCV_FIN_BWD; j.c = c; j.rows = sums; j.rows_ld = ld; j.count = count; j.dgamma = dgamma; j.dbeta = dbeta; j.coef = coef; j.accumulate = accumulate;
+  bn_fin_channel<false>(j, blockIdx.x * (blockDim.x / 32) + threadIdx.x / 32, threadIdx.x & 31);
 }
 __global__ void bn_bwd_finalize2_kernel(satcv_stat_t* sums, int ld, satcv_stat_t* asums, int ald, int c, float count, const float* scale, const float* shift,
                                         const float* mean, const float* rstd, float* dgamma, float* dbeta, float* coef, int accumulate) {
-  const int ch = blockIdx.x * (blockDim.x / 32) + threadIdx.x / 32, r = threadIdx.x & 31;
-  double d1 = 0.0, d2 = 0.0, a1 = 0.0, a2 = 0.0;
-  if (ch < c) {
-    if (sums) { satcv_stat_t* row = sums + (size_t)r * 2 * ld; d1 = row[ch]; d2 = row[ld + ch]; row[ch] = 0.0; row[ld + ch] = 0.0; }
-    satcv_stat_t* arow = asums + (size_t)r * 2 * ald;
-    a1 = arow[ch]; a2 = arow[ald + ch]; arow[ch] = 0.0; arow[ald + ch] = 0.0;
-  }
-#pragma unroll
-  for (int o = 16; o > 0; o >>= 1) {
-    d1 += __shfl_xor(d1, o, 64); d2 += __shfl_xor(d2, o, 64); a1 += __shfl_xor(a1, o, 64); a2 += __shfl_xor(a2, o, 64);
-  }
-  if (ch >= c || r != 0) return;
-  const double sc = (double)scale[ch], sh = (double)shift[ch], mu = (double)mean[ch], rs = (double)rstd[ch];
-  const double a2x = sc != 0.0 ? (a2 - (sh + sc * mu) * a1) * (rs / sc) : 0.0;
-  const float s1 = (float)(d1 + a1), s2 = (float)(d2 + a2x);
-  if (dbeta) dbeta[ch] = accumulate ? dbeta[ch] + s1 : s1;
-  if (dgamma) dgamma[ch] = accumulate ? dgamma[ch] + s2 : s2;
-  coef[ch] = s1 / count; coef[c + ch] = s2 / count;
+  satcv_bn_fin_job j = {};
+  j.kind = SATCV_FIN_BWD_ACT; j.c = c; j.rows = sums; j.rows_ld = ld; j.act_rows = asums; j.act_rows_ld = ald; j.count = count;
+  j.scale = const_cast<float*>(scale); j.shift = const_cast<float*>(shift); j.mean = const_cast<float*>(mean); j.rstd = const_cast<float*>(rstd);
+  j.dgamma = dgamma; j.dbeta = dbeta; j.coef = coef; j.accumulate = accumulate;
+  bn_fin_channel<false>(j, blockIdx.x * (blockDim.x / 32) + threadIdx.x / 32, threadIdx.x & 31);
 }
 extern "C" int satcv_bn_bwd_finalize2(satcv_stat_t* sums, int32_t sums_ld, satcv_stat_t* act_sums, int32_t act_sums_ld, int32_t c, float count,
                                       const float* scale, const float* shift, const float* mean, const float* rstd, float* dgamma, float* dbeta,
diff --git a/satellite_computervision_amd/csrc/igemm_common.hpp b/satellite_computervision_amd/csrc/igemm_common.hpp
--- a/satellite_computervision_amd/csrc/igemm_common.hpp
+++ b/satellite_computervision_amd/csrc/igemm_common.hpp
@@ -27,6 +27,8 @@
   int ksplit; float* kslab;
   int tile_policy;
   int pair_n, pair_c0, pair_c1;
+  const satcv_bn_fin_job* fin;
+  int fin_done;
 };
 
 template <typename T>
@@ -490,5 +492,5 @@
 int igemm_m16p_launch(IgemmArgs& a, int dtype, hipStream_t st, bool dry);
 int igemm_ws_launch(IgemmArgs& a, int dtype, hipStream_t st, bool dry_run);
 int igemm_tr_launch(IgemmArgs& a, int dtype, hipStream_t st, bool dry);
-int convt_thin_launch(const IgemmArgs& a, int dtype, hipStream_t st);
+int convt_thin_launch(IgemmArgs& a, int dtype, hipStream_t st);
 int convt_thin_dgrad_launch(const IgemmArgs& a, int dtype, hipStream_t st);
diff --git a/satellite_computervision_amd/engine.py b/satellite_computervision_amd/engine.py
--- a/satellite_computervision_amd/engine.py
+++ b/satellite_computervision_amd/engine.py
@@ -281,6 +281,7 @@
         d = ops.make_conv_desc(**kw)
         self.keep.append(d)
         fn = lambda st, d=d: check(lib.satcv_conv2d_igemm(C.byref(d), st))
+        fn.desc = d
         k, cin, cout = kw.get('kh', 1) * kw.get('kw', 1), kw.get('c0', 0) + (kw.get('c1', 0) or 0), kw['cout']
         px = kw['n'] * kw['h'] * kw['w_']
         fn.label = (f"conv_{role} k{kw.get('kh', 1)} d{kw.get('dil', 1)} n{kw['n']} {kw['h']}x{kw['w_']} {kw.get('c0', 0)}+{kw.get('c1', 0) or 0}->{cout}"
@@ -312,6 +313,18 @@
                     _fp(stats, off), ld, c, float(count), g, b, BN_EPS, BN_MOMENTUM, updates, bessel, None, None,
                     _fp(ts), _fp(tt), _fp(a['mean'], aoff), _fp(a['rstd'], aoff), st)))
                 self.fwd.append(lambda st: check(lib.satcv_bn_affine_infer(g, b, mm, mv, BN_EPS, c, _fp(a['scale'], aoff), _fp(a['shift'], aoff), st)))
+                return a
+            prod = self.fwd[-1] if self.fwd else None
+            pd = getattr(prod, 'desc', None)
+            lo = stats.data_ptr()
+            if (getattr(rt.model, 'fuse_bn_finalize', True) and not self.sync_bn and pd is not None and pd.stats and not pd.fin and not pd.bst_y
+                    and lo <= pd.stats < lo + stats.numel() * stats.element_size()):
+                job = ops.make_fin_job(0, c, float(count), stats.device, rows=_fp(stats, off), rows_ld=ld, gamma=g, beta=b, eps=BN_EPS,
+                                       momentum=BN_MOMENTUM, updates=updates, bessel=bessel, moving_mean=mm, moving_var=mv,
+                                       scale=_fp(a['scale'], aoff), shift=_fp(a['shift'], aoff), mean=_fp(a['mean'], aoff), rstd=_fp(a['rstd'], aoff))
+                self.keep.append(job)
+                pd.fin = job.data_ptr()
+                prod.label = getattr(prod, 'label', '') + ' +bnfin'
                 return a
             self.fwd.append(lambda st: check(lib.satcv_bn_finalize_train(
                 _fp(stats, off), ld, c, float(count), g, b, BN_EPS, BN_MOMENTUM, updates, bessel, mm, mv,
diff --git a/satellite_computervision_amd/model_tools.py b/satellite_computervision_amd/model_tools.py
--- a/satellite_computervision_amd/model_tools.py
+++ b/satellite_computervision_amd/model_tools.py
@@ -712,6 +712,7 @@
         self.fuse_head_grad = os.environ.get('SATCV_FUSE_HEAD_GRAD', '1') != '0'
         self.fuse_pool_bwd = os.environ.get('SATCV_FUSE_POOL_BWD', '1') != '0'
         self.fuse_thin_bwd = os.environ.get('SATCV_FUSE_THIN_BWD', '1') != '0'
+        self.fuse_bn_finalize = True
         self.sync_bn = os.environ.get('SATCV_SYNC_BN', '0') == '1'
         self._rt = None
         self.optimizer, self._loss, self._metrics = None, None, []
diff --git a/satellite_computervision_amd/ops.py b/satellite_computervision_amd/ops.py
--- a/satellite_computervision_amd/ops.py
+++ b/satellite_computervision_amd/ops.py
@@ -68,8 +68,9 @@
 
 def make_conv_desc(*, x0, c0, w, y, ldy, n, h, w_, cout, cout_pad, dtype, x1=None, c1=0, in_scale=None, in_shift=None,
                    in_relu=0, bias=None, stats=None, stats_ld=0, kh=3, kw=3, dil=1, mode_in=0, mode_out=0, f=1,
-                   cstat=None, out_relu=0, accumulate=0, stride=1, hin=0, win=0, out_scale=None, pool_y=None, pool_ld=0, pool_f=0, bst=None, tile_policy=0, pair=None):
+                   cstat=None, out_relu=0, accumulate=0, stride=1, hin=0, win=0, out_scale=None, pool_y=None, pool_ld=0, pool_f=0, bst=None, tile_policy=0, pair=None, fin=None):
     d = ConvDesc()
+    d.fin = fin
     d.tile_policy = int(tile_policy)
     if pair:
         d.pair_n, d.pair_c0, d.pair_c1 = (int(v) for v in pair)
@@ -96,7 +97,7 @@
 
 
 def conv2d(x, w_packed, cout, *, kh=3, kw=3, dil=1, bias=None, x1=None, in_scale=None, in_shift=None, in_relu=False,
-           stats=None, out=None, out_relu=False, stride=1, bst=None, out_scale=None, pool_y=None, pool_f=0):
+           stats=None, out=None, out_relu=False, stride=1, bst=None, out_scale=None, pool_y=None, pool_f=0, fin=None):
     n, hin, win, c0 = x.shape
     h, w_ = ((hin - 1) // stride + 1, (win - 1) // stride + 1) if stride > 1 else (hin, win)
     dtype = DTYPE_CODE[x.dtype]
@@ -108,7 +109,7 @@
                        in_relu=in_relu, bias=_p(bias), stats=_p(stats), stats_ld=stats.shape[-1] if stats is not None else 0,
                        kh=kh, kw=kw, dil=dil, out_relu=out_relu, stride=stride, hin=hin if stride > 1 else 0, win=win if stride > 1 else 0,
                        out_scale=_p(out_scale), pool_y=_p(pool_y), pool_ld=pool_y.shape[-1] if pool_y is not None else 0, pool_f=pool_f,
-                       bst={k: (_p(v) if torch.is_tensor(v) else v) for k, v in bst.items()} if bst else None)
+                       bst={k: (_p(v) if torch.is_tensor(v) else v) for k, v in bst.items()} if bst else None, fin=_p(fin))
     if bst and lib.satcv_conv2d_igemm_pipelined(C.byref(d)) != 1:
         raise ValueError('conv2d: this shape cannot carry the fused BatchNorm-backward reduce (bst); run satcv_bn_bwd_reduce separately')
     check(lib.satcv_conv2d_igemm(C.byref(d), stream_ptr()))
@@ -116,14 +117,14 @@
 
 
 def conv2d_transpose(x, w_packed, cout, f, *, bias=None, in_scale=None, in_shift=None, in_relu=False, stats=None, out=None,
-                     out_scale=None, out_relu=False):
+                     out_scale=None, out_relu=False, fin=None):
     n, h, w_, c0 = x.shape
     dtype = DTYPE_CODE[x.dtype]
     y = out if out is not None else torch.empty(n, h * f, w_ * f, rup(cout, 16), dtype=x.dtype, device=x.device)
     d = make_conv_desc(x0=_p(x), c0=c0, w=_p(w_packed), y=_p(y), ldy=y.shape[-1], n=n, h=h, w_=w_, cout=f * f * cout,
                        cout_pad=rup(f * f * cout, 32), dtype=dtype, in_scale=_p(in_scale), in_shift=_p(in_shift),
                        in_relu=in_relu, bias=_p(bias), stats=_p(stats), stats_ld=stats.shape[-1] if stats is not None else 0,
-                       kh=1, kw=1, dil=1, mode_out=1, f=f, cstat=cout, out_scale=_p(out_scale), out_relu=out_relu)
+                       kh=1, kw=1, dil=1, mode_out=1, f=f, cstat=cout, out_scale=_p(out_scale), out_relu=out_relu, fin=_p(fin))
     check(lib.satcv_conv2d_igemm(C.byref(d), stream_ptr()))
     return y
 
@@ -229,6 +230,25 @@
     return dw
 
 
+def make_fin_job(kind, c, count, device, *, rows=None, rows_ld=0, act_rows=None, act_rows_ld=0, gamma=None, beta=None, eps=1e-3, momentum=0.99,
+                 updates=1, bessel=False, moving_mean=None, moving_var=None, scale=None, shift=None, mean=None, rstd=None,
+                 dgamma=None, dbeta=None, coef=None, accumulate=0):
+    j = _lib.BnFinJob()
+    j.kind, j.c, j.count = int(kind), int(c), float(count)
+    j.rows, j.rows_ld, j.act_rows, j.act_rows_ld = rows, int(rows_ld), act_rows, int(act_rows_ld)
+    j.gamma, j.beta, j.eps, j.momentum, j.updates, j.bessel = gamma, beta, eps, momentum, int(updates), int(bool(bessel))
+    j.moving_mean, j.moving_var = moving_mean, moving_var
+    j.scale, j.shift, j.mean, j.rstd = scale, shift, mean, rstd
+    j.dgamma, j.dbeta, j.coef, j.accumulate = dgamma, dbeta, coef, int(accumulate)
+    size = (C.sizeof(j) + 15) // 16 * 16
+    buf = torch.zeros(size + 16, dtype=torch.uint8, device=device)
+    j.counter = buf.data_ptr() + size
+    host = torch.zeros(size + 16, dtype=torch.uint8)
+    C.memmove(host.data_ptr(), C.addressof(j), C.sizeof(j))
+    buf.copy_(host)
+    return buf
+
+
 def bn_finalize_train(stats, count, gamma, beta, moving_mean, moving_var, eps=1e-3, momentum=0.99, updates=1, bessel=False):
     c = gamma.numel()
     dev = gamma.device
```

After: 7370 tiles/s. 12.0% lower.
